# asbschmidt/CUDASW4

Measured on AMD Instinct MI355X. Metric: GCUPS, higher is better.
Workload: dtype f16x2; 1 GPU; peak: allqueries.fasta (20 queries, 41752 residues) vs pseudo DB 1000000 x 512, half2 kernel configuration, blosum62, gop -11 gex -1, top 10, C++ host driver; db_subjects=1000000, db_residues=512000000, queries=20, kernel=half2, queries_in_flight=1, tail_overlaps=10, numa_node_rank0=0, numa_bound=True, resident=True, residency=resident, cached_chars=512000000, parallelism=db-shard x1 (one DB sharded), one top-K gather per step + host merge

## Files before the change

cudasw4_amd/csrc/sw_api.hip:

```cpp
#include <hip/hip_runtime.h>
#include <hipcub/hipcub.hpp>

#include <algorithm>
#include <cstdio>
#include <cmath>
#include <cstdlib>
#include <cstring>
#include <ctime>
#include <string>
#include <vector>

#include "../../include/cudasw4_amd.h"
#include "../../include/cudasw4_amd_engine.h"
#include "sw_internal.hpp"
#include "sw_launch.hpp"
#include "sw_rows_pipeline.hpp"

namespace {

thread_local std::string g_last_error = "";

int fail(int code, const std::string& msg) {
    g_last_error = msg;
    return code;
}

#define SW_HIP(expr)                                                                              \
    do {                                                                                          \
        hipError_t e__ = (expr);                                                                  \
        if (e__ != hipSuccess)                                                                    \
            return fail(SW_ERR_HIP, std::string(#expr) + ": " + hipGetErrorString(e__));          \
    } while (0)

const swk::KindLaunch* kind_launch(int kind) {
    switch (kind) {
        case SW_KIND_F16X2: return &swk::launch_f16x2();
        case SW_KIND_I16X2: return &swk::launch_i16x2();
        case SW_KIND_I32: return &swk::launch_i32();
        case SW_KIND_F32: return &swk::launch_f32();
    }
    return nullptr;
}

bool kind_packed(int kind) { return kind == SW_KIND_F16X2 || kind == SW_KIND_I16X2; }

struct QueryPlan {
    int rows = 0;
    int nstripes = 0;
    int lanes = 16;
};

QueryPlan plan_query(int kind, int32_t qlen, int lanes) {
    const swk::KindLaunch* kl = kind_launch(kind);
    QueryPlan pl;
    pl.lanes = lanes;
    if (!kl || qlen <= 0) return pl;
    const int maxrows = swk::max_rows(kind, lanes);
    const int maxrows_multi = (kind == SW_KIND_F32 && lanes <= 16) ? std::min(maxrows, swk::kMaxRowsScalarMulti) : maxrows;
    double two_wave_penalty = 1.05;
    if (const char* e = getenv("CUDASW4_AMD_TWO_WAVE_PENALTY")) two_wave_penalty = std::max(1.0, atof(e));
    const bool has_three_wave_multi = kl->packed && lanes <= 16 && swk::kWaves3MaxRowsPackedMulti > maxrows / 2;
    double best = 1e300;
    auto consider = [&](int ns) {
        const int64_t per_lane = (qlen + (int64_t)lanes * ns - 1) / ((int64_t)lanes * ns);
        int r = (int)((per_lane + swk::kRowsGranule - 1) / swk::kRowsGranule * swk::kRowsGranule);
        r = std::max(r, swk::kRowsGranule);
        if (r > (ns > 1 ? maxrows_multi : maxrows)) return;
        if (ns > 1 && 2 * r <= maxrows) return;
        double cost = ns * (r + (ns > 1 ? 3.0 : 1.2));
        if (has_three_wave_multi && ns > 1 && r > swk::kWaves3MaxRowsPackedMulti) cost *= two_wave_penalty;
        if (cost < best - 1e-9) { best = cost; pl.rows = r; pl.nstripes = ns; }
    };
    if (qlen <= (int64_t)lanes * maxrows) consider(1);
    const int64_t stripe_multi = (int64_t)lanes * maxrows_multi;
    const int ns_m = std::max<int>(2, (int)((qlen + stripe_multi - 1) / stripe_multi));
    int ns_hi = ns_m + 2;
    if (has_three_wave_multi) {
        const int64_t stripe3 = (int64_t)lanes * swk::kWaves3MaxRowsPackedMulti;
        ns_hi = std::max<int>(ns_hi, (int)((qlen + stripe3 - 1) / stripe3) + 1);
    }
    for (int ns = ns_m; ns <= ns_hi; ns++) consider(ns);
    return pl;
}

struct Profile {
    unsigned char* dev = nullptr;
    size_t capacity = 0;
    bool valid = false;
    QueryPlan plan;
    int shift = 0;
    hipEvent_t ready = nullptr;
};

}

constexpr uint32_t kWorkSlots = 4096;
#ifndef SW_LANES8_MAX_QUERY_PACKED
#define SW_LANES8_MAX_QUERY_PACKED 256
#endif
#ifndef SW_LANES4_MAX_QUERY_PACKED
#define SW_LANES4_MAX_QUERY_PACKED 96
#endif
#ifndef SW_LANES4_MAX_QUERY_SCALAR
#define SW_LANES4_MAX_QUERY_SCALAR 128
#endif
#ifndef SW_LANES4_MAX_SUBJECT
#define SW_LANES4_MAX_SUBJECT 1280
#endif
#ifndef SW_LANES4_MIN_BATCHES_PER_CU
#define SW_LANES4_MIN_BATCHES_PER_CU 12
#endif
#ifndef SW_LANES8_MAX_SUBJECT
#define SW_LANES8_MAX_SUBJECT 192
#endif
#ifndef SW_LANES8_MAX_QUERY_SCALAR
#define SW_LANES8_MAX_QUERY_SCALAR 256
#endif

struct sw_ctx {
    int device = 0;
    int num_cus = 0;
    int8_t* d_matrix = nullptr;
    int dim = swk::kLetters;
    uint32_t* d_zeros = nullptr;
    uint32_t* d_work = nullptr;
    uint32_t work_next = 0;
    uint32_t work_zeroed = 0;
    uint32_t* start_signal = nullptr;
    uint32_t* dry_signal = nullptr;
    int32_t* dirty_counter = nullptr;
    uint32_t dry_value = 0;
    int grid_reserve = 0;
    int grid_mult = 4;
    int grid_cap = 0;
    bool have_matrix = false;
    int8_t* d_query = nullptr;
    size_t query_capacity = 0;
    static constexpr int kQuerySlots = 4;
    int8_t* h_query[kQuerySlots] = {};
    size_t h_query_capacity[kQuerySlots] = {};
    hipEvent_t query_copied[kQuerySlots] = {};
    bool query_slot_used[kQuerySlots] = {};
    int query_next = 0;
    int32_t qlen = 0;
    bool have_query = false;
    Profile profiles[4][4][2];
    bool use_offs = true;
    int64_t long16_min = -1;
    int64_t long16_min_default = -1;
    int matrix_max = 1;
    bool i32_native = false;
    int32_t lanes4_max_subject = -1;
    int32_t lanes4_max_q = -1;
    int32_t lanes8_max_q = -1;
    bool check_bounds = false;
    uint32_t pipe_spin_limit = 1u << 20;
    int32_t pipe_drop_stage = -1;
    int32_t pipe_cpl = 0;
    int32_t stream_slots = 4;
    int32_t stream_jump = 0;
    int32_t stream_cols_max = 4096;
    int32_t stream_multi_cols_max = 1536;
    int32_t stream_multi_max_subject = -1;
    int32_t pipe_quorum = 0;
    int32_t pipe_slot = 0;
};

namespace {

int max_grid(const sw_ctx* ctx) {
    const int g = std::max(1, ctx->num_cus) * ctx->grid_mult;
    return ctx->grid_cap > 0 ? std::min(g, ctx->grid_cap) : g;
}

int rescore_lanes(int32_t max_subject_len) { return max_subject_len > 1280 ? 64 : 16; }

int shape_index(int lanes) { return lanes == 64 ? 1 : lanes == 8 ? 2 : lanes == 4 ? 3 : 0; }

int effective_kind_of(const sw_ctx* ctx, int kind, int32_t max_subject_len) {
    if (kind != SW_KIND_I32 || ctx->i32_native || !ctx->have_query) return kind;
    const int64_t bound = (int64_t)std::min(ctx->qlen, max_subject_len) * std::max(1, ctx->matrix_max) + ((int64_t)1 << 22) + 4096;
    return bound < ((int64_t)1 << 24) ? SW_KIND_F32 : SW_KIND_I32;
}

int lanes_for_partition_any(const sw_ctx* ctx, int kind, int part_id, int32_t n, int32_t max_subject_len);
int lanes_for_partition(const sw_ctx* ctx, int kind, int part_id, int32_t n, int32_t max_subject_len) {
    const int lanes = lanes_for_partition_any(ctx, kind, part_id, n, max_subject_len);
    return (lanes == 16 && kind_packed(kind) && max_subject_len >= 0xffff) ? 64 : lanes;
}
int lanes_for_partition_any(const sw_ctx* ctx, int kind, int part_id, int32_t n, int32_t max_subject_len) {
    if (part_id < SW_NUM_LENGTH_PARTITIONS - 2) {
        if (!ctx->have_query) return 16;
        const int32_t limit4 = ctx->lanes4_max_q >= 0 ? ctx->lanes4_max_q : kind_packed(kind) ? SW_LANES4_MAX_QUERY_PACKED : SW_LANES4_MAX_QUERY_SCALAR;
        const int64_t batches4 = (int64_t)n / (64 * (kind_packed(kind) ? 2 : 1));
        const bool enough4 = ctx->lanes4_max_q >= 0 || batches4 >= (int64_t)SW_LANES4_MIN_BATCHES_PER_CU * std::max(1, ctx->num_cus);
        const int32_t lmax4 = ctx->lanes4_max_subject >= 0 ? ctx->lanes4_max_subject : SW_LANES4_MAX_SUBJECT;
        if (ctx->qlen <= 4 * swk::max_rows(kind, 4) && ctx->qlen <= limit4 && enough4 && max_subject_len <= lmax4) return 4;
        const bool fits8 = ctx->qlen <= 8 * swk::max_rows(kind, 8);
        const int32_t limit = ctx->lanes8_max_q >= 0 ? ctx->lanes8_max_q : kind_packed(kind) ? SW_LANES8_MAX_QUERY_PACKED : SW_LANES8_MAX_QUERY_SCALAR;
        if (fits8 && ctx->qlen <= limit) return 8;
        return 16;
    }
    const int64_t fills_gpu_twice = (int64_t)2 * std::max(1, ctx->num_cus) * 4 * 32;
    if (part_id == SW_NUM_LENGTH_PARTITIONS - 2) return n >= (ctx->long16_min >= 0 ? ctx->long16_min : 512) ? 16 : 64;
    return n >= fills_gpu_twice ? 16 : 64;
}


int ensure_profile(sw_ctx* ctx, int kind, int lanes, bool offs, int shift, hipStream_t stream) {
    Profile& pr = ctx->profiles[kind][shape_index(lanes)][offs];
    if (pr.valid && pr.shift != shift) pr.valid = false;
    if (pr.valid) {
        SW_HIP(hipStreamWaitEvent(stream, pr.ready, 0));
        return SW_OK;
    }
    const swk::KindLaunch* kl = kind_launch(kind);
    const QueryPlan pl = plan_query(kind, ctx->qlen, lanes);
    const size_t bytes = kl->tile_bytes(pl.rows, lanes) * (size_t)pl.nstripes;
    if (bytes == 0) return fail(SW_ERR_INVALID, "no kernel compiled for this query plan");
    if (bytes > pr.capacity) {
        const size_t cap = std::max<size_t>(std::max(bytes, 2 * pr.capacity), size_t(2) << 20);
        if (pr.dev) SW_HIP(hipFree(pr.dev));
        pr.dev = nullptr;
        pr.capacity = 0;
        SW_HIP(hipMalloc(&pr.dev, cap));
        pr.capacity = cap;
    }
    SW_HIP(kl->profile(pl.rows, lanes, ctx->d_query, ctx->qlen, ctx->d_matrix, ctx->dim, pl.nstripes, pr.dev, shift, stream));
    pr.shift = shift;
    if (!pr.ready) SW_HIP(hipEventCreateWithFlags(&pr.ready, hipEventDisableTiming));
    SW_HIP(hipEventRecord(pr.ready, stream));
    pr.plan = pl;
    pr.valid = true;
    return SW_OK;
}

int32_t border_capacity(int32_t max_len, int lanes) {
    const int64_t steps = ((int64_t)max_len + lanes - 1 + 3) / 4 * 4;
    return (int32_t)((steps + 15) / 16 * 16 + 16);
}
size_t border_bytes_per_wg(int32_t lcap, int lanes) {
    if (lanes == 4) return 0;
    const size_t region = lanes == 16 ? swk::border_region_words<16>(lcap) : lanes == 8 ? swk::border_region_words<8>(lcap) : swk::border_region_words<64>(lcap);
    return (size_t)(swk::kThreads / lanes) * region * sizeof(uint32_t);
}

__global__ void max_length_kernel(const int32_t* lengths, const int32_t* positions, const int32_t* count_ptr, int32_t first_pos,
                                  int32_t n, int32_t* out) {
    const int32_t cnt = count_ptr ? min(*count_ptr, n) : n;
    int32_t m = 0;
    for (int32_t i = blockIdx.x * blockDim.x + threadIdx.x; i < cnt; i += gridDim.x * blockDim.x)
        m = max(m, lengths[positions ? positions[i] : first_pos + i]);
    if (m > 0) atomicMax(out, m);
}

struct StreamPlan { int slots = 0, cols = 0, room = 0, base = 0, jump = 0; };
StreamPlan stream_plan(const sw_ctx* ctx, int kind, int lanes, int a, const QueryPlan& pl, int32_t max_subject_len) {
    StreamPlan sp;
    if (!kind_packed(kind) || lanes != 16 || a < 0) return sp;
    const bool multi = pl.nstripes > 1;
    const int P = swk::frame_classes(true, pl.rows, lanes, multi);
    sp.base = kind == SW_KIND_F16X2 ? -2016 : 0;
    const int top = kind == SW_KIND_F16X2 ? 1024 : 12400;
    sp.jump = ctx->stream_jump > 0 ? ctx->stream_jump : (kind == SW_KIND_F16X2 ? 512 : 2048);
    sp.room = top - sp.base - a * (2 * lanes + 4 + P);
    sp.cols = a > 0 ? std::min(sp.room / a, ctx->stream_cols_max) : ctx->stream_cols_max;
    sp.slots = std::max(1, std::min(ctx->stream_slots, swk::kStreamMaxSlots));
    if (sp.room < 4 * lanes * a || sp.cols < 4 * lanes) sp.slots = 1;
    if (multi) {
        const int32_t limit = ctx->stream_multi_max_subject >= 0 ? ctx->stream_multi_max_subject : (kind == SW_KIND_F16X2 ? 320 : 192);
        if (max_subject_len > limit) sp.slots = 1;
        sp.cols = std::min(sp.cols, ctx->stream_multi_cols_max);
    }
    return sp;
}

bool offs_possible(const sw_ctx* ctx, int kind, int lanes, int32_t max_subject_len, int gop, int gex, int ovf_check, int64_t* K_out) {
    const int a = -gex;
    const int64_t room = kind == SW_KIND_F16X2 ? 1536 : kind == SW_KIND_I16X2 ? 12500 : (int64_t)1 << 22;
    int64_t K = 1 << 21;
    while (K >= 4 * lanes && (int64_t)a * (K + 3 * lanes + 16) > room) K >>= 1;
    if (kind == SW_KIND_I16X2) K = std::min<int64_t>(K, std::max<int64_t>(2048, 4 * lanes));
    if (!kind_packed(kind) && max_subject_len + 3 * lanes + 16 > K) K = 0;
    if (K_out) *K_out = K;
    return ctx->use_offs && K >= 4 * lanes && (!kind_packed(kind) || (ovf_check && a >= 0)) && gop - gex >= -1000;
}
int packed_fallback_kind(int kind) { return kind == SW_KIND_F16X2 ? SW_KIND_F32 : SW_KIND_I32; }

constexpr uint32_t kWorkZeroBlock = 64;
hipError_t take_work_slot(sw_ctx* ctx, hipStream_t stream, uint32_t** out) {
    uint32_t* w = ctx->d_work + 2 * (ctx->work_next++ % kWorkSlots);
    *out = w;
    if (ctx->work_zeroed > 0) { ctx->work_zeroed--; return hipSuccess; }
    return hipMemsetAsync(w, 0, 2 * sizeof(uint32_t), stream);
}

struct ListMode {
    int32_t* claim = nullptr;
    int service_workgroups = 0;
    const uint32_t* done_flag = nullptr;
    uint32_t done_value = 0;
};

int scan_common(sw_ctx* ctx, int kind, int lanes, const int8_t* chars, const uint64_t* offsets, const int32_t* lengths,
                const int32_t* positions, const int32_t* count_ptr, int32_t first_pos, int32_t n,
                int32_t max_subject_len, int gop, int gex, float* scores, int32_t* ids, int64_t id_offset,
                int32_t* ovf_pos, int32_t* ovf_count, int ovf_check, void* temp, size_t temp_bytes,
                hipStream_t stream, int32_t* stat_count = nullptr, int32_t stat_limit = 0, const ListMode& list = ListMode()) {
    if (!ctx) return fail(SW_ERR_INVALID, "null context");
    uint32_t* const start_signal = ctx->start_signal;
    ctx->start_signal = nullptr;
    uint32_t* const dry_signal = ctx->dry_signal;
    ctx->dry_signal = nullptr;
    const swk::KindLaunch* kl = kind_launch(kind);
    if (!kl) return fail(SW_ERR_INVALID, "unknown kind");
    if (n < 0 || max_subject_len < 0) return fail(SW_ERR_INVALID, "negative count or length");
    if (max_subject_len > SW_MAX_SUBJECT_LEN)
        return fail(SW_ERR_INVALID, "max_subject_len " + std::to_string(max_subject_len) + ": pass the longest subject of the range (lengths[last]), not the partition's nominal boundary");
    if (gop > 0 || gex > 0) return fail(SW_ERR_INVALID, "gap scores must be <= 0");
    if (kind_packed(kind) && (gop < -1000 || gex < -1000)) return fail(SW_ERR_INVALID, "gap score out of range for a 16-bit kind");
    if (!ctx->have_matrix) return fail(SW_ERR_NO_MATRIX, "sw_set_matrix has not been called");
    if (!ctx->have_query) return fail(SW_ERR_NO_QUERY, "sw_set_query has not been called");
    if (n == 0) return SW_OK;
    if (!chars || !offsets || !lengths || !scores || !ids) return fail(SW_ERR_INVALID, "null buffer");
    if (ovf_check && kind_packed(kind) && (!ovf_pos || !ovf_count)) return fail(SW_ERR_INVALID, "overflow check without overflow buffers");
    SW_HIP(hipSetDevice(ctx->device));
    if (ctx->check_bounds) {
        int32_t* slot = reinterpret_cast<int32_t*>(ctx->d_zeros + 64);
        int32_t longest = 0;
        SW_HIP(hipMemsetAsync(slot, 0, sizeof(int32_t), stream));
        hipLaunchKernelGGL(max_length_kernel, dim3(std::min(1024, (n + 255) / 256)), dim3(256), 0, stream, lengths, positions, count_ptr, first_pos, n, slot);
        SW_HIP(hipGetLastError());
        SW_HIP(hipMemcpyAsync(&longest, slot, sizeof(int32_t), hipMemcpyDeviceToHost, stream));
        SW_HIP(hipStreamSynchronize(stream));
        if (longest > max_subject_len)
            return fail(SW_ERR_INVALID, "max_subject_len " + std::to_string(max_subject_len) + " under-reports: a subject of the range has " +
                                            std::to_string(longest) + " residues");
    }
    const int a = -gex;
    int64_t K = 0;
    const bool offs = offs_possible(ctx, kind, lanes, max_subject_len, gop, gex, ovf_check, &K);
    if (kind_packed(kind) && !offs) return fail(SW_ERR_INVALID, "internal: a packed launch without the column-offset recurrence (packed_fallback_kind)");
    int rc = ensure_profile(ctx, kind, lanes, offs, offs ? a : 0, stream);
    if (rc != SW_OK) return rc;
    const Profile& prof = ctx->profiles[kind][shape_index(lanes)][offs];
    const QueryPlan pl = prof.plan;
    const bool multi = pl.nstripes > 1;

    const int subj_per_batch = (swk::kThreads / lanes) * (kind_packed(kind) ? 2 : 1);
    const int nbatches = (n + subj_per_batch - 1) / subj_per_batch;
    int grid = std::min(nbatches, max_grid(ctx));
    if (list.service_workgroups > 0) grid = std::min(grid, list.service_workgroups);

    swk::ScanParams p{};
    p.claim = list.claim;
    p.service = list.service_workgroups > 0 ? 1 : 0;
    p.done_flag = list.done_flag;
    p.done_value = list.done_value;
    p.chars = chars; p.offsets = offsets; p.lengths = lengths;
    p.positions = positions; p.count_ptr = count_ptr;
    p.first_pos = first_pos; p.n = n;
    p.profile = prof.dev; p.nstripes = pl.nstripes;
    switch (kind) {
        case SW_KIND_F16X2: p.gop = swk::Arith<swk::F16X2>::encode_gap(gop); p.gex = swk::Arith<swk::F16X2>::encode_gap(gex); break;
        case SW_KIND_I16X2: p.gop = swk::Arith<swk::I16X2>::encode_gap(gop); p.gex = swk::Arith<swk::I16X2>::encode_gap(gex); break;
        case SW_KIND_I32: p.gop = swk::Arith<swk::I32>::encode_gap(gop); p.gex = swk::Arith<swk::I32>::encode_gap(gex); break;
        default: p.gop = swk::Arith<swk::F32>::encode_gap(gop); p.gex = swk::Arith<swk::F32>::encode_gap(gex); break;
    }
    if (offs) {
        const int g = gop - gex;
        switch (kind) {
            case SW_KIND_F16X2: p.gop = swk::Arith<swk::F16X2>::encode_gap(g); break;
            case SW_KIND_I16X2: p.gop = swk::Arith<swk::I16X2>::encode_gap(g); break;
            case SW_KIND_I32: p.gop = swk::Arith<swk::I32>::encode_gap(g); break;
            default: p.gop = swk::Arith<swk::F32>::encode_gap(g); break;
        }
        p.gex_mag = a;
        {
            const int P = swk::frame_classes(kl->packed, pl.rows, lanes, multi);
            const int wrap = -a * P, wrap_last = -a * ((pl.rows - 1) % P + 1);
            switch (kind) {
                case SW_KIND_F16X2: p.wrap_class = swk::Arith<swk::F16X2>::encode_gap(wrap); p.wrap_last = swk::Arith<swk::F16X2>::encode_gap(wrap_last); break;
                case SW_KIND_I16X2: p.wrap_class = swk::Arith<swk::I16X2>::encode_gap(wrap); p.wrap_last = swk::Arith<swk::I16X2>::encode_gap(wrap_last); break;
                case SW_KIND_I32: p.wrap_class = swk::Arith<swk::I32>::encode_gap(wrap); p.wrap_last = swk::Arith<swk::I32>::encode_gap(wrap_last); break;
                default: p.wrap_class = swk::Arith<swk::F32>::encode_gap(wrap); p.wrap_last = swk::Arith<swk::F32>::encode_gap(wrap_last); break;
            }
        }
        p.renorm_quads = (int32_t)(K / 4);
        const int lower = -(int)((int64_t)a * K);
        switch (kind) {
            case SW_KIND_F16X2: p.renorm_word = swk::Arith<swk::F16X2>::encode_gap(lower); break;
            case SW_KIND_I16X2: p.renorm_word = swk::Arith<swk::I16X2>::encode_gap(lower); break;
            case SW_KIND_I32: p.renorm_word = swk::Arith<swk::I32>::encode_gap(lower); break;
            default: p.renorm_word = swk::Arith<swk::F32>::encode_gap(lower); break;
        }
    }
    const StreamPlan sp = stream_plan(ctx, kind, lanes, a, pl, max_subject_len);
    if (sp.slots >= 1) {
        p.stream_slots = sp.slots; p.stream_cols = sp.cols; p.stream_room = sp.room; p.level_base = sp.base;
        p.jump = sp.jump; p.jump_limit = sp.jump - 4;
        p.jump_word = kind == SW_KIND_F16X2 ? swk::Arith<swk::F16X2>::pos_word(sp.jump) : swk::Arith<swk::I16X2>::pos_word(sp.jump);
    }
    p.scores = scores; p.ids = ids; p.id_offset = id_offset;
    p.ovf_pos = ovf_pos; p.ovf_count = ovf_count; p.ovf_check = (ovf_check && kind_packed(kind)) ? 1 : 0;
    p.scratch = nullptr; p.lcap = 0; p.zeros = ctx->d_zeros + kind * 16;
    p.stat_count = stat_count; p.stat_limit = stat_limit;
    if (multi) {
        p.lcap = border_capacity(max_subject_len, lanes);
        if (p.stream_slots > 1) {
            int cols = p.stream_cols;
            while (cols > max_subject_len && (size_t)grid * border_bytes_per_wg(border_capacity(cols, lanes), lanes) > temp_bytes) cols = cols * 3 / 4;
            p.stream_cols = cols;
            p.lcap = border_capacity(std::max(max_subject_len, cols), lanes);
        }
        const size_t per_wg = border_bytes_per_wg(p.lcap, lanes);
        if (!temp || temp_bytes < per_wg) return fail(SW_ERR_TEMP, "temp buffer too small for a multi-stripe query");
        grid = (int)std::min<size_t>((size_t)grid, temp_bytes / per_wg);
        p.scratch = static_cast<uint32_t*>(temp);
    }
    SW_HIP(take_work_slot(ctx, stream, &p.work_counter));
    p.start_signal = start_signal;
    p.start_quorum = (uint32_t)std::min(grid, 64);
    p.dry_signal = dry_signal;
    if (!stat_count && !positions && p.stream_slots > 1 && lanes == 16 && kind_packed(kind)) { p.stat_count = ctx->dirty_counter; p.stat_limit = INT32_MAX; }
    p.dry_value = ctx->dry_value;
    const int reserve = (list.service_workgroups > 0 || list.claim) ? 0 : ctx->grid_reserve;
    SW_HIP(kl->scan(pl.rows, lanes, multi, offs, grid, reserve, stream, p));
    return SW_OK;
}

}

namespace {
#define SW_REP8(OP) OP(0) OP(1) OP(2) OP(3) OP(4) OP(5) OP(6) OP(7)
#define SW_OP_PK_MAX3(i) asm volatile("v_pk_maximum3_f16 %0, %0, %1, %2" : "+v"(a[i]) : "v"(b), "v"(c));
#define SW_OP_ADD_F32(i) asm volatile("v_add_f32 %0, %0, %1" : "+v"(a[i]) : "v"(b));
#define SW_OP_MAX3_F32(i) asm volatile("v_max3_f32 %0, %0, %1, %2" : "+v"(a[i]) : "v"(b), "v"(c));
#define SW_OP_ADD_U32(i) asm volatile("v_add_u32 %0, %0, %1" : "+v"(a[i]) : "v"(b));
#define SW_OP_MAX3_I32(i) asm volatile("v_max3_i32 %0, %0, %1, %2" : "+v"(a[i]) : "v"(b), "v"(c));
#define SW_OP_PK_FMA(i) asm volatile("v_pk_fma_f16 %0, %1, %2, %0 op_sel:[0,1,0] op_sel_hi:[1,0,1]" : "+v"(a[i]) : "v"(b), "v"(c));
#define SW_OP_PK_ADD(i) asm volatile("v_pk_add_f16 %0, %0, %1" : "+v"(a[i]) : "v"(b));
#define SW_OP_DPP(i) asm volatile("v_mov_b32_dpp %0, %1 row_shr:1 row_mask:0xf bank_mask:0xf" : "+v"(a[i]) : "v"(b));
#define SW_OP_PERM(i) asm volatile("v_perm_b32 %0, %0, %1, %2" : "+v"(a[i]) : "v"(b), "v"(c));
template <int MIX>
__global__ void __launch_bounds__(256) valu_rate_kernel(unsigned* out, unsigned long long* clocks, unsigned seed, int iters) {
    unsigned a[8];
    unsigned b = seed + threadIdx.x, c = seed * 3u + 1u;
    for (int i = 0; i < 8; i++) a[i] = seed + i + threadIdx.x;
    if constexpr (MIX == 4) {
        asm volatile("v_mov_b32 v0, %0\nv_mov_b32 v1, %0\nv_mov_b32 v2, %0\nv_mov_b32 v3, %0\nv_mov_b32 v4, %0\nv_mov_b32 v5, %0\nv_mov_b32 v6, %0\nv_mov_b32 v7, %0\n"
                     "v_mov_b32 v8, %1\nv_mov_b32 v9, %1\nv_mov_b32 v10, %1\nv_mov_b32 v11, %1\nv_mov_b32 v12, %2\nv_mov_b32 v13, %2\nv_mov_b32 v14, %2\nv_mov_b32 v15, %2\n"
                     :: "v"(a[0]), "v"(b), "v"(c) : "v0", "v1", "v2", "v3", "v4", "v5", "v6", "v7", "v8", "v9", "v10", "v11", "v12", "v13", "v14", "v15");
    }
    const unsigned long long t0 = clock64(), w0 = wall_clock64();
    for (int it = 0; it < iters; it++) {
        if constexpr (MIX == 0) { SW_REP8(SW_OP_PK_MAX3) SW_REP8(SW_OP_PK_MAX3) SW_REP8(SW_OP_PK_MAX3) SW_REP8(SW_OP_PK_MAX3) }
        if constexpr (MIX == 1) { SW_REP8(SW_OP_ADD_F32) SW_REP8(SW_OP_MAX3_F32) SW_REP8(SW_OP_ADD_F32) SW_OP_MAX3_F32(0) SW_OP_MAX3_F32(1) SW_OP_MAX3_F32(2) SW_OP_MAX3_F32(3) SW_OP_MAX3_F32(4) SW_OP_MAX3_F32(5) SW_OP_ADD_F32(6) SW_OP_ADD_F32(7) }
        if constexpr (MIX == 3) {
            SW_REP8(SW_OP_PK_MAX3) SW_OP_PK_FMA(0) SW_OP_PK_FMA(1) SW_OP_PK_ADD(2) SW_OP_PK_ADD(3) SW_OP_DPP(4) SW_OP_PK_FMA(5) SW_OP_PK_ADD(6) SW_OP_ADD_U32(7)
            SW_REP8(SW_OP_PK_MAX3) SW_OP_PK_FMA(0) SW_OP_PK_FMA(1) SW_OP_PK_ADD(2) SW_OP_PK_ADD(3) SW_OP_DPP(4) SW_OP_PK_FMA(5) SW_OP_PK_ADD(6) SW_OP_PERM(7)
            SW_REP8(SW_OP_PK_MAX3) SW_OP_PK_FMA(0) SW_OP_PK_FMA(1) SW_OP_PK_ADD(2) SW_OP_PK_ADD(3) SW_OP_DPP(4) SW_OP_PK_ADD(5) SW_OP_PK_ADD(6) SW_OP_ADD_U32(7)
            SW_REP8(SW_OP_PK_MAX3) SW_OP_PK_FMA(0) SW_OP_PK_FMA(1) SW_OP_PK_ADD(2) SW_OP_PK_ADD(3) SW_OP_PK_MAX3(4) SW_OP_PK_MAX3(5) SW_OP_PK_MAX3(6) SW_OP_PK_ADD(7)
        }
        if constexpr (MIX == 4) {
#define SW_B4_MAX3(i, j, k) "v_pk_maximum3_f16 v" #i ", v" #i ", v" #j ", v" #k "\n"
#define SW_B4_FMA(i, j, k) "v_pk_fma_f16 v" #i ", v" #j ", v" #k ", v" #i " op_sel:[0,1,0] op_sel_hi:[1,0,1]\n"
#define SW_B4_ADD(i, j) "v_pk_add_f16 v" #i ", v" #i ", v" #j "\n"
#define SW_B4_DPP(i, j) "v_mov_b32_dpp v" #i ", v" #j " row_shr:1 row_mask:0xf bank_mask:0xf\n"
#define SW_B4_ADDU(i, j) "v_add_u32 v" #i ", v" #i ", v" #j "\n"
#define SW_B4_ROW8 SW_B4_MAX3(0, 9, 14) SW_B4_MAX3(1, 10, 15) SW_B4_MAX3(2, 11, 12) SW_B4_MAX3(3, 8, 13) SW_B4_MAX3(4, 9, 14) SW_B4_MAX3(5, 10, 15) SW_B4_MAX3(6, 11, 12) SW_B4_MAX3(7, 8, 13)
            asm volatile(
                SW_B4_ROW8 SW_B4_FMA(0, 9, 14) SW_B4_FMA(1, 10, 15) SW_B4_ADD(2, 11) SW_B4_ADD(3, 8) SW_B4_DPP(4, 9) SW_B4_FMA(5, 10, 15) SW_B4_ADD(6, 11) SW_B4_ADDU(7, 8)
                SW_B4_ROW8 SW_B4_FMA(0, 9, 14) SW_B4_FMA(1, 10, 15) SW_B4_ADD(2, 11) SW_B4_ADD(3, 8) SW_B4_DPP(4, 9) SW_B4_FMA(5, 10, 15) SW_B4_ADD(6, 11) SW_B4_MAX3(7, 8, 13)
                SW_B4_ROW8 SW_B4_FMA(0, 9, 14) SW_B4_FMA(1, 10, 15) SW_B4_ADD(2, 11) SW_B4_ADD(3, 8) SW_B4_DPP(4, 9) SW_B4_ADD(5, 10) SW_B4_ADD(6, 11) SW_B4_ADDU(7, 8)
                SW_B4_ROW8 SW_B4_FMA(0, 9, 14) SW_B4_FMA(1, 10, 15) SW_B4_ADD(2, 11) SW_B4_ADD(3, 8) SW_B4_MAX3(4, 9, 14) SW_B4_MAX3(5, 10, 15) SW_B4_MAX3(6, 11, 12) SW_B4_ADD(7, 8)
                ::: "v0", "v1", "v2", "v3", "v4", "v5", "v6", "v7", "v8", "v9", "v10", "v11", "v12", "v13", "v14", "v15");
        }
        if constexpr (MIX == 2) { SW_REP8(SW_OP_MAX3_I32) SW_REP8(SW_OP_ADD_U32) SW_REP8(SW_OP_MAX3_I32) SW_OP_ADD_U32(0) SW_OP_ADD_U32(1) SW_OP_ADD_U32(2) SW_OP_ADD_U32(3) SW_OP_MAX3_I32(4) SW_OP_MAX3_I32(5) SW_OP_MAX3_I32(6) SW_OP_MAX3_I32(7) }
    }
    const unsigned long long t1 = clock64(), w1 = wall_clock64();
    if constexpr (MIX == 4) asm volatile("v_mov_b32 %0, v0\nv_xor_b32 %0, %0, v7" : "=v"(a[0]) :: "v0", "v7");
    unsigned r = 0;
    for (int i = 0; i < 8; i++) r ^= a[i];
    out[blockIdx.x * blockDim.x + threadIdx.x] = r;
    if (threadIdx.x == 0) { clocks[2 * blockIdx.x] = t1 - t0; clocks[2 * blockIdx.x + 1] = w1 - w0; }
}
}

namespace swi {
int fail(int code, const std::string& msg) { return ::fail(code, msg); }
int32_t query_length(const sw_ctx* ctx) { return ctx && ctx->have_query ? ctx->qlen : 0; }
int device_of(const sw_ctx* ctx) { return ctx ? ctx->device : -1; }
int num_cus(const sw_ctx* ctx) { return ctx ? ctx->num_cus : 0; }
const int8_t* matrix(const sw_ctx* ctx, int* dim) {
    if (!ctx || !ctx->have_matrix) return nullptr;
    *dim = ctx->dim;
    return ctx->d_matrix;
}
}

extern "C" {

const char* sw_version(void) { return "cudasw4_amd 0.2 (gfx950)"; }

const char* sw_last_error(void) { return g_last_error.c_str(); }

int sw_device_count(void) {
    int n = 0;
    if (hipGetDeviceCount(&n) != hipSuccess) return 0;
    return n;
}

int sw_ctx_create(int device, sw_ctx** out) {
    if (!out) return fail(SW_ERR_INVALID, "null out pointer");
    *out = nullptr;
    int n = 0;
    if (hipGetDeviceCount(&n) != hipSuccess || n <= 0) return fail(SW_ERR_NO_DEVICE, "no HIP device available (this library has no CPU path)");
    if (device < 0 || device >= n) return fail(SW_ERR_INVALID, "device index out of range");
    SW_HIP(hipSetDevice(device));
    hipDeviceProp_t prop;
    SW_HIP(hipGetDeviceProperties(&prop, device));
    sw_ctx* ctx = new sw_ctx;
    ctx->device = device;
    ctx->num_cus = prop.multiProcessorCount;
    if (const char* e = getenv("CUDASW4_AMD_GRID_CAP")) ctx->grid_cap = std::max(0, atoi(e));
    if (const char* e = getenv("CUDASW4_AMD_NO_OFFS")) ctx->use_offs = !(e[0] == '1');
    if (const char* e = getenv("CUDASW4_AMD_I32_NATIVE")) ctx->i32_native = e[0] == '1';
    if (const char* e = getenv("CUDASW4_AMD_LANES8_MAX_Q")) ctx->lanes8_max_q = atoi(e);
    if (const char* e = getenv("CUDASW4_AMD_LANES4_MAX_Q")) ctx->lanes4_max_q = atoi(e);
    if (const char* e = getenv("CUDASW4_AMD_LANES4_MAX_SUBJECT")) ctx->lanes4_max_subject = atoi(e);
    if (const char* e = getenv("CUDASW4_AMD_CHECK_BOUNDS")) ctx->check_bounds = e[0] == '1';
    if (const char* e = getenv("CUDASW4_AMD_PIPE_SPIN_LIMIT")) ctx->pipe_spin_limit = (uint32_t)std::max(1ll, atoll(e));
    if (const char* e = getenv("CUDASW4_AMD_PIPE_TEST_DROP_STAGE")) ctx->pipe_drop_stage = atoi(e);
    if (const char* e = getenv("CUDASW4_AMD_PIPE_CPL")) ctx->pipe_cpl = atoi(e);
    if (const char* e = getenv("CUDASW4_AMD_STREAM")) ctx->stream_slots = std::max(0, std::min(swk::kStreamMaxSlots, atoi(e)));
    hipError_t e = hipMalloc(&ctx->d_matrix, 26 * swk::kLetters);
    if (e == hipSuccess) e = hipMalloc(&ctx->d_zeros, 256 + 64);
    if (e == hipSuccess) e = hipMalloc(&ctx->d_work, 2 * kWorkSlots * sizeof(uint32_t));
    if (e == hipSuccess) {
        uint32_t z[64] = {};
        for (int i = 0; i < 16; i++) z[SW_KIND_I16X2 * 16 + i] = swk::Arith<swk::I16X2>::kZero;
        e = hipMemcpy(ctx->d_zeros, z, sizeof(z), hipMemcpyHostToDevice);
    }
    for (int kind = 0; kind < 4 && e == hipSuccess; kind++) e = kind_launch(kind)->warm(nullptr);
    if (e == hipSuccess) e = hipStreamSynchronize(nullptr);
    if (e != hipSuccess) { delete ctx; return fail(SW_ERR_HIP, std::string("context set-up: ") + hipGetErrorString(e)); }
    *out = ctx;
    return SW_OK;
}

int sw_ctx_destroy(sw_ctx* ctx) {
    if (!ctx) return SW_OK;
    (void)hipSetDevice(ctx->device);
    if (ctx->d_matrix) (void)hipFree(ctx->d_matrix);
    if (ctx->d_zeros) (void)hipFree(ctx->d_zeros);
    if (ctx->d_work) (void)hipFree(ctx->d_work);
    if (ctx->d_query) (void)hipFree(ctx->d_query);
    for (int i = 0; i < sw_ctx::kQuerySlots; i++) {
        if (ctx->h_query[i]) (void)hipHostFree(ctx->h_query[i]);
        if (ctx->query_copied[i]) (void)hipEventDestroy(ctx->query_copied[i]);
    }
    for (auto& row : ctx->profiles)
        for (auto& shape : row)
            for (auto& pr : shape) {
                if (pr.dev) (void)hipFree(pr.dev);
                if (pr.ready) (void)hipEventDestroy(pr.ready);
            }
    delete ctx;
    return SW_OK;
}

int sw_set_matrix(sw_ctx* ctx, const int8_t* matrix_host, int dim) {
    if (!ctx || !matrix_host) return fail(SW_ERR_INVALID, "null argument");
    if (dim != 21 && dim != 25) return fail(SW_ERR_INVALID, "substitution matrices are 21 x 21 (20 amino acids + other) or 25 x 25 (types.hpp:205-396)");
    constexpr int kX = 23;
    int8_t m[26 * swk::kLetters];
    auto subject_col = [&](int j) { return (dim == 25 && j == swk::kPadLetter) ? kX : j; };
    for (int i = 0; i <= dim; i++) {
        const int qi = i < dim ? i : (dim == 25 ? kX : swk::kPadLetter);
        for (int j = 0; j < swk::kLetters; j++) m[i * swk::kLetters + j] = matrix_host[qi * dim + subject_col(j)];
    }
    for (int i = 0; i <= dim; i++)
        if (m[i * swk::kLetters + swk::kPadLetter] >= 0) return fail(SW_ERR_INVALID, "scores against the padding letter must be negative");
    for (int j = 0; j < swk::kLetters; j++)
        if (m[dim * swk::kLetters + j] >= 0) return fail(SW_ERR_INVALID, "scores against the padding letter must be negative");
    SW_HIP(hipSetDevice(ctx->device));
    SW_HIP(hipMemcpy(ctx->d_matrix, m, (size_t)(dim + 1) * swk::kLetters, hipMemcpyHostToDevice));
    ctx->matrix_max = 1;
    for (int i = 0; i < dim * dim; i++) ctx->matrix_max = std::max(ctx->matrix_max, (int)matrix_host[i]);
    if (ctx->have_query && dim < ctx->dim) ctx->have_query = false;
    ctx->dim = dim;
    ctx->have_matrix = true;
    for (auto& row : ctx->profiles)
        for (auto& shape : row)
            for (auto& pr : shape) pr.valid = false;
    return SW_OK;
}

int sw_set_query(sw_ctx* ctx, const int8_t* query_codes_host, int32_t qlen, void* stream) {
    if (!ctx || !query_codes_host) return fail(SW_ERR_INVALID, "null argument");
    if (qlen <= 0) return fail(SW_ERR_INVALID, "query length must be positive");
    for (int32_t i = 0; i < qlen; i++)
        if (query_codes_host[i] < 0 || query_codes_host[i] >= ctx->dim) return fail(SW_ERR_INVALID, "query code out of range for the installed matrix");
    SW_HIP(hipSetDevice(ctx->device));
    if ((size_t)qlen > ctx->query_capacity) {
        if (ctx->d_query) SW_HIP(hipFree(ctx->d_query));
        ctx->d_query = nullptr;
        ctx->query_capacity = 0;
        const size_t cap = std::max<size_t>(((size_t)qlen + 4095) / 4096 * 4096 * 2, size_t(1) << 16);
        SW_HIP(hipMalloc(&ctx->d_query, cap));
        ctx->query_capacity = cap;
    }
    hipStream_t s = static_cast<hipStream_t>(stream);
    const int slot = ctx->query_next;
    ctx->query_next = (ctx->query_next + 1) % sw_ctx::kQuerySlots;
    if (ctx->query_slot_used[slot]) SW_HIP(hipEventSynchronize(ctx->query_copied[slot]));
    if ((size_t)qlen > ctx->h_query_capacity[slot]) {
        if (ctx->h_query[slot]) SW_HIP(hipHostFree(ctx->h_query[slot]));
        ctx->h_query[slot] = nullptr;
        ctx->h_query_capacity[slot] = 0;
        const size_t cap = std::max<size_t>(((size_t)qlen + 4095) / 4096 * 4096 * 2, size_t(1) << 16);
        SW_HIP(hipHostMalloc(&ctx->h_query[slot], cap));
        ctx->h_query_capacity[slot] = cap;
    }
    if (!ctx->query_copied[slot]) SW_HIP(hipEventCreateWithFlags(&ctx->query_copied[slot], hipEventDisableTiming));
    memcpy(ctx->h_query[slot], query_codes_host, (size_t)qlen);
    SW_HIP(hipMemcpyAsync(ctx->d_query, ctx->h_query[slot], qlen, hipMemcpyHostToDevice, s));
    ctx->work_next = (ctx->work_next + kWorkZeroBlock - 1) / kWorkZeroBlock * kWorkZeroBlock;
    SW_HIP(hipMemsetAsync(ctx->d_work + 2 * (ctx->work_next % kWorkSlots), 0, 2 * kWorkZeroBlock * sizeof(uint32_t), s));
    ctx->work_zeroed = kWorkZeroBlock;
    SW_HIP(hipEventRecord(ctx->query_copied[slot], s));
    ctx->query_slot_used[slot] = true;
    ctx->qlen = qlen;
    ctx->have_query = true;
    for (auto& row : ctx->profiles)
        for (auto& shape : row)
            for (auto& pr : shape) pr.valid = false;
    return SW_OK;
}

namespace {
__global__ void __launch_bounds__(256) check_codes_kernel(const int8_t* __restrict__ chars, size_t n, int32_t* bad) {
    const size_t stride = (size_t)gridDim.x * blockDim.x * 16;
    unsigned m = 0;
    const size_t head = (16 - ((size_t)chars & 15)) & 15;
    const size_t tid = (size_t)blockIdx.x * blockDim.x + threadIdx.x;
    if (tid < head && tid < n) m |= (unsigned char)chars[tid] > 20 ? 1u : 0u;
    const size_t body = n > head ? (n - head) / 16 * 16 : 0;
    for (size_t i = tid * 16; i < body; i += stride) {
        const uint4 v = *reinterpret_cast<const uint4*>(chars + head + i);
        const unsigned w[4] = {v.x, v.y, v.z, v.w};
#pragma unroll
        for (int k = 0; k < 4; k++) {
            m |= w[k] & 0xE0E0E0E0u;
            m |= ((w[k] & 0x1F1F1F1Fu) + 0x0B0B0B0Bu) & 0x20202020u;
        }
    }
    const size_t tail0 = head + body;
    if (tail0 + tid < n && tid < 16) m |= (unsigned char)chars[tail0 + tid] > 20 ? 1u : 0u;
    if (m) atomicOr(bad, 1);
}
}

int sw_check_letter_codes(sw_ctx* ctx, const int8_t* chars, size_t n, int32_t* bad_flag, void* stream) {
    if (!ctx || !bad_flag) return fail(SW_ERR_INVALID, "null argument");
    if (n == 0) return SW_OK;
    if (!chars) return fail(SW_ERR_INVALID, "null buffer");
    SW_HIP(hipSetDevice(ctx->device));
    const size_t want = (n / 16 + 255) / 256 + 1;
    const int grid = (int)std::min<size_t>(want, (size_t)std::max(1, ctx->num_cus) * 16);
    hipLaunchKernelGGL(check_codes_kernel, dim3(grid), dim3(256), 0, static_cast<hipStream_t>(stream), chars, n, bad_flag);
    SW_HIP(hipGetLastError());
    return SW_OK;
}

int sw_set_start_signal(sw_ctx* ctx, uint32_t* signal) {
    if (!ctx) return fail(SW_ERR_INVALID, "null context");
    ctx->start_signal = signal;
    return SW_OK;
}


namespace {
int rows_common_checks(sw_ctx* ctx, const int8_t* chars, const uint64_t* offsets, const int32_t* lengths, int32_t first_pos, int32_t n,
                       int32_t max_subject_len, int gop, int gex, float* scores, int32_t* ids, bool dry_armed, hipStream_t stream,
                       const char* who) {
    if (dry_armed) return fail(SW_ERR_INVALID, std::string(who) + " never runs dry: sw_set_dry_signal applies to sw_scan_partition launches (the armed signal was cancelled)");
    if (n < 0 || max_subject_len < 0) return fail(SW_ERR_INVALID, "negative count or length");
    if (gop > 0 || gex > 0) return fail(SW_ERR_INVALID, "gap scores must be <= 0");
    if (gop > gex) return fail(SW_ERR_INVALID, std::string(who) + " needs gop <= gex (the prefix form of the horizontal gap)");
    if (gex < -10000 || gop < -100000) return fail(SW_ERR_INVALID, std::string("gap score out of range for ") + who);
    if (!ctx->have_matrix) return fail(SW_ERR_NO_MATRIX, "sw_set_matrix has not been called");
    if (!ctx->have_query) return fail(SW_ERR_NO_QUERY, "sw_set_query has not been called");
    if (n == 0) return SW_OK;
    if (!chars || !offsets || !lengths || !scores || !ids) return fail(SW_ERR_INVALID, "null buffer");
    SW_HIP(hipSetDevice(ctx->device));
    if (ctx->check_bounds) {
        int32_t* slot = reinterpret_cast<int32_t*>(ctx->d_zeros + 64);
        int32_t longest = 0;
        SW_HIP(hipMemsetAsync(slot, 0, sizeof(int32_t), stream));
        hipLaunchKernelGGL(max_length_kernel, dim3(std::min(1024, (n + 255) / 256)), dim3(256), 0, stream, lengths, nullptr, nullptr, first_pos, n, slot);
        SW_HIP(hipGetLastError());
        SW_HIP(hipMemcpyAsync(&longest, slot, sizeof(int32_t), hipMemcpyDeviceToHost, stream));
        SW_HIP(hipStreamSynchronize(stream));
        if (longest > max_subject_len)
            return fail(SW_ERR_INVALID, "max_subject_len " + std::to_string(max_subject_len) + " under-reports: a subject of the range has " +
                                            std::to_string(longest) + " residues");
    }
    return SW_OK;
}

int pipeline_cpl(const sw_ctx* ctx, int32_t n, int32_t max_subject_len) {
    if (ctx->pipe_cpl == 4 || ctx->pipe_cpl == 8 || ctx->pipe_cpl == 16) return ctx->pipe_cpl;
    static const double kRowUs16[3] = {0.27, 0.38, 0.57}, kHopUs16[3] = {3.6, 5.0, 8.0}, kRowUs8[3] = {0.32, 0.42, 0.61}, kHopUs8[3] = {2.4, 3.4, 5.3};
    const bool shortBatch = ctx->qlen <= swk::kPipeShortBatchMaxQuery;
    const double* kRowUs = shortBatch ? kRowUs8 : kRowUs16;
    const double* kHopUs = shortBatch ? kHopUs8 : kHopUs16;
    int best = 16;
    double bestT = 1e300;
    for (int k = 0; k < 3; k++) {
        const int cpl = 4 << k;
        const double stages = std::max(1.0, std::ceil((double)max_subject_len / (64.0 * cpl)));
        if (cpl < 16 && (double)std::max(n, 1) * stages > 768.0) continue;
        const double t = (double)std::max(ctx->qlen, 1) * kRowUs[k] + stages * kHopUs[k];
        if (t < bestT) { bestT = t; best = cpl; }
    }
    return best;
}
constexpr size_t kPipeCtrlBytes = 16;
int64_t pipeline_stages(int cpl, int32_t max_subject_len) { return std::max<int64_t>(1, ((int64_t)max_subject_len + 64 * cpl - 1) / (64 * cpl)); }
}


size_t sw_scan_rows_pipelined_temp_bytes(sw_ctx* ctx, int32_t n, int32_t max_subject_len) {
    if (!ctx || !ctx->have_query || n <= 0 || max_subject_len < 0) return 0;
    const int64_t tickets = (int64_t)n * pipeline_stages(pipeline_cpl(ctx, n, max_subject_len), max_subject_len);
    return kPipeCtrlBytes + (size_t)tickets * ((size_t)ctx->qlen + 1) * sizeof(unsigned long long);
}

namespace {
int launch_pipeline(sw_ctx* ctx, swk::PipelineParams& p, int cpl, int64_t stages, int64_t tickets, uint32_t* start_signal, void* xfer,
                    hipStream_t stream) {
    const size_t need = kPipeCtrlBytes + (size_t)tickets * ((size_t)ctx->qlen + 1) * sizeof(unsigned long long);
    p.query = ctx->d_query; p.qlen = ctx->qlen; p.matrix = ctx->d_matrix; p.dim = ctx->dim;
    p.ctrl = static_cast<uint32_t*>(xfer);
    p.xfer = reinterpret_cast<unsigned long long*>(static_cast<char*>(xfer) + kPipeCtrlBytes);
    p.start_signal = start_signal;
    const int slot_regs = ctx->pipe_slot > 0 ? ctx->pipe_slot : 128;
    const int64_t resident = (int64_t)std::max(1, ctx->num_cus) * 4 * std::max(1, std::min(8, 512 / slot_regs)) / 2;
    p.start_quorum = (uint32_t)std::max<int64_t>(1, std::min(tickets, ctx->pipe_quorum > 0 ? (int64_t)ctx->pipe_quorum : resident));
    p.max_stages = (int32_t)stages;
    p.spin_limit = ctx->pipe_spin_limit;
    p.test_drop_stage = ctx->pipe_drop_stage;
    SW_HIP(hipMemsetAsync(xfer, 0xFF, need, stream));
    const dim3 grid((unsigned)tickets), block(64);
    const int slot = ctx->pipe_slot;
#define SW_PIPE_LAUNCH_B(CPL, B)                                                                                            \
    do {                                                                                                                    \
        if (slot == 128) hipLaunchKernelGGL((swk::sw_rows_pipeline_kernel<CPL, 128, B>), grid, block, 0, stream, p);        \
        else if (slot == 168) hipLaunchKernelGGL((swk::sw_rows_pipeline_kernel<CPL, 168, B>), grid, block, 0, stream, p);   \
        else if (slot == 256) hipLaunchKernelGGL((swk::sw_rows_pipeline_kernel<CPL, 256, B>), grid, block, 0, stream, p);   \
        else hipLaunchKernelGGL((swk::sw_rows_pipeline_kernel<CPL, 0, B>), grid, block, 0, stream, p);                      \
    } while (0)
#define SW_PIPE_LAUNCH(CPL)                                                                                              \
    do {                                                                                                                 \
        if (ctx->qlen <= swk::kPipeShortBatchMaxQuery) SW_PIPE_LAUNCH_B(CPL, 8);                                         \
        else SW_PIPE_LAUNCH_B(CPL, 16);                                                                                  \
    } while (0)
    if (cpl == 4) SW_PIPE_LAUNCH(4);
    else if (cpl == 8) SW_PIPE_LAUNCH(8);
    else SW_PIPE_LAUNCH(16);
#undef SW_PIPE_LAUNCH_B
#undef SW_PIPE_LAUNCH
    SW_HIP(hipGetLastError());
    return SW_OK;
}

__global__ void __launch_bounds__(256) pipeline_pick_kernel(int32_t* list, const int32_t* count_ptr, int32_t max_count, const int32_t* lengths,
                                                            int32_t min_len, int32_t cap, int32_t* out_pos, int32_t* out_count) {
    __shared__ int k;
    if (threadIdx.x == 0) k = 0;
    __syncthreads();
    const int32_t cnt = min(*count_ptr, max_count);
    for (int32_t i = threadIdx.x; i < cnt; i += blockDim.x) {
        const int32_t v = __hip_atomic_load(list + i, __ATOMIC_RELAXED, __HIP_MEMORY_SCOPE_AGENT);
        if (v < 0 || lengths[v] < min_len) continue;
        const int slot = atomicAdd(&k, 1);
        if (slot >= cap) continue;
        if (atomicCAS(list + i, v, swk::kListTaken) == v) out_pos[slot] = v;
        else out_pos[slot] = -1;
    }
    __syncthreads();
    if (threadIdx.x == 0) *out_count = min(k, cap);
}
constexpr int32_t kPipeRescoreCap = 64;
size_t pipe_rescore_header_bytes() { return 256 + (size_t)kPipeRescoreCap * sizeof(int32_t); }
}

int sw_scan_rows_pipelined(sw_ctx* ctx, const int8_t* chars, const uint64_t* offsets, const int32_t* lengths, int32_t first_pos,
                           int32_t n, int32_t max_subject_len, int gop, int gex, float* scores, int32_t* ids, int64_t id_offset,
                           int32_t* fail_count, int32_t* over_limit_count, int32_t* over_limit_count2, int32_t packed_limit,
                           void* temp, size_t temp_bytes, void* stream_) {
    if (!ctx) return fail(SW_ERR_INVALID, "null context");
    uint32_t* const start_signal = ctx->start_signal;
    ctx->start_signal = nullptr;
    const bool dry_armed = ctx->dry_signal != nullptr;
    ctx->dry_signal = nullptr;
    hipStream_t stream = static_cast<hipStream_t>(stream_);
    if ((int64_t)max_subject_len * (int64_t)(-gex) >= ((int64_t)1 << 28)) return fail(SW_ERR_INVALID, "subject length x gap extension out of range for sw_scan_rows_pipelined");
    const int rc = rows_common_checks(ctx, chars, offsets, lengths, first_pos, n, max_subject_len, gop, gex, scores, ids, dry_armed, stream, "sw_scan_rows_pipelined");
    if (rc != SW_OK || n == 0) return rc;
    const int cpl = pipeline_cpl(ctx, n, max_subject_len);
    const int64_t stages = pipeline_stages(cpl, max_subject_len);
    const int64_t tickets = (int64_t)n * stages;
    if (tickets > (int64_t)1 << 24) return fail(SW_ERR_INVALID, "too many pipeline stages for one sw_scan_rows_pipelined launch");
    const size_t need = kPipeCtrlBytes + (size_t)tickets * ((size_t)ctx->qlen + 1) * sizeof(unsigned long long);
    if (!temp || temp_bytes < need) return fail(SW_ERR_TEMP, "temp buffer too small for sw_scan_rows_pipelined (sw_scan_rows_pipelined_temp_bytes)");
    swk::PipelineParams p{};
    p.chars = chars; p.offsets = offsets; p.lengths = lengths; p.first_pos = first_pos; p.n = n;
    p.gop = gop; p.gex = gex; p.scores = scores; p.ids = ids; p.id_offset = id_offset;
    p.fail_count = fail_count;
    p.stat_count = over_limit_count; p.stat_count2 = over_limit_count2; p.stat_limit = packed_limit;
    return launch_pipeline(ctx, p, cpl, stages, tickets, start_signal, temp, stream);
}

size_t sw_rescore_overflow_pipelined_temp_bytes(sw_ctx* ctx, int32_t max_subject_len) {
    if (!ctx || !ctx->have_query || max_subject_len < 0) return 0;
    const int64_t tickets = (int64_t)kPipeRescoreCap * pipeline_stages(pipeline_cpl(ctx, kPipeRescoreCap, max_subject_len), max_subject_len);
    return pipe_rescore_header_bytes() + kPipeCtrlBytes + (size_t)tickets * ((size_t)ctx->qlen + 1) * sizeof(unsigned long long);
}

int sw_rescore_overflow_pipelined(sw_ctx* ctx, int32_t* ovf_pos, const int32_t* ovf_count, int32_t max_count, const int8_t* chars,
                                  const uint64_t* offsets, const int32_t* lengths, int32_t max_subject_len, int32_t min_subject_len,
                                  int gop, int gex, float* scores, int32_t* ids, int64_t id_offset, int32_t* fail_count,
                                  int32_t packed_limit, int32_t* true_overflow_count, void* temp, size_t temp_bytes, void* stream_) {
    if (!ctx) return fail(SW_ERR_INVALID, "null context");
    ctx->start_signal = nullptr;
    const bool dry_armed = ctx->dry_signal != nullptr;
    ctx->dry_signal = nullptr;
    hipStream_t stream = static_cast<hipStream_t>(stream_);
    if (!ovf_pos || !ovf_count) return fail(SW_ERR_INVALID, "null overflow buffers");
    if (max_count <= 0) return SW_OK;
    if ((int64_t)max_subject_len * (int64_t)(-gex) >= ((int64_t)1 << 28)) return fail(SW_ERR_INVALID, "subject length x gap extension out of range for sw_rescore_overflow_pipelined");
    const int rc = rows_common_checks(ctx, chars, offsets, lengths, 0, 1, max_subject_len, gop, gex, scores, ids, dry_armed, stream, "sw_rescore_overflow_pipelined");
    if (rc != SW_OK) return rc;
    const int cpl = pipeline_cpl(ctx, kPipeRescoreCap, max_subject_len);
    const int64_t stages = pipeline_stages(cpl, max_subject_len);
    const int64_t tickets = (int64_t)kPipeRescoreCap * stages;
    const size_t need = sw_rescore_overflow_pipelined_temp_bytes(ctx, max_subject_len);
    if (!temp || temp_bytes < need) return fail(SW_ERR_TEMP, "temp buffer too small for sw_rescore_overflow_pipelined");
    int32_t* out_count = static_cast<int32_t*>(temp);
    int32_t* out_pos = reinterpret_cast<int32_t*>(static_cast<char*>(temp) + 256);
    hipLaunchKernelGGL(pipeline_pick_kernel, dim3(1), dim3(256), 0, stream, ovf_pos, ovf_count, max_count, lengths, std::max(min_subject_len, 1),
                       kPipeRescoreCap, out_pos, out_count);
    SW_HIP(hipGetLastError());
    swk::PipelineParams p{};
    p.chars = chars; p.offsets = offsets; p.lengths = lengths; p.first_pos = 0; p.n = kPipeRescoreCap;
    p.positions = out_pos; p.count_ptr = out_count;
    p.gop = gop; p.gex = gex; p.scores = scores; p.ids = ids; p.id_offset = id_offset;
    p.fail_count = fail_count;
    p.stat_count = true_overflow_count; p.stat_count2 = nullptr; p.stat_limit = packed_limit;
    return launch_pipeline(ctx, p, cpl, stages, tickets, nullptr, static_cast<char*>(temp) + pipe_rescore_header_bytes(), stream);
}

int sw_set_dirty_counter(sw_ctx* ctx, int32_t* counter) {
    if (!ctx) return fail(SW_ERR_INVALID, "null context");
    ctx->dirty_counter = counter;
    return SW_OK;
}

int sw_set_dry_signal(sw_ctx* ctx, uint32_t* signal, uint32_t value) {
    if (!ctx) return fail(SW_ERR_INVALID, "null context");
    ctx->dry_signal = signal;
    ctx->dry_value = value;
    return SW_OK;
}

int sw_set_long16_min(sw_ctx* ctx, int32_t subjects) {
    if (!ctx) return fail(SW_ERR_INVALID, "null context");
    ctx->long16_min = subjects < 0 ? ctx->long16_min_default : subjects;
    return SW_OK;
}

int sw_set_grid_reserve(sw_ctx* ctx, int32_t workgroups) {
    if (!ctx) return fail(SW_ERR_INVALID, "null context");
    if (workgroups < 0) return fail(SW_ERR_INVALID, "negative reserve");
    ctx->grid_reserve = workgroups;
    return SW_OK;
}

namespace {
__global__ void reduce_windows_kernel(const float* __restrict__ win_scores, const int32_t* __restrict__ win_first,
                                      const int32_t* __restrict__ real_pos, int32_t n_real, float* __restrict__ scores,
                                      int32_t* __restrict__ ids, int64_t id_offset) {
    const int32_t i = blockIdx.x * blockDim.x + threadIdx.x;
    if (i >= n_real) return;
    float m = -1.0f;
    for (int32_t w = win_first[i]; w < win_first[i + 1]; w++) m = fmaxf(m, win_scores[w]);
    const int32_t pos = real_pos[i];
    scores[pos] = m;
    ids[pos] = (int32_t)(id_offset + pos);
}
}

namespace {
__global__ void probe_wait_kernel(unsigned* flag, unsigned* saw, unsigned long long max_ticks) {
    const unsigned long long t0 = wall_clock64();
    unsigned v = 0;
    while ((v = __hip_atomic_load(flag, __ATOMIC_RELAXED, __HIP_MEMORY_SCOPE_AGENT)) == 0 && wall_clock64() - t0 < max_ticks)
        __builtin_amdgcn_s_sleep(8);
    *saw = v;
}
__global__ void probe_set_kernel(unsigned* flag) { __hip_atomic_store(flag, 1u, __ATOMIC_RELAXED, __HIP_MEMORY_SCOPE_AGENT); }
__global__ void probe_side_kernel(unsigned* signal, unsigned* flag, unsigned* saw, unsigned long long max_ticks) {
    __hip_atomic_fetch_add(signal, 1u, __ATOMIC_RELEASE, __HIP_MEMORY_SCOPE_SYSTEM);
    const unsigned long long t0 = wall_clock64();
    unsigned v = 0;
    while ((v = __hip_atomic_load(flag, __ATOMIC_RELAXED, __HIP_MEMORY_SCOPE_AGENT)) == 0 && wall_clock64() - t0 < max_ticks)
        __builtin_amdgcn_s_sleep(8);
    *saw = v;
}
}

int sw_probe_handshake(sw_ctx* ctx, void* side_stream, void* gated_stream, uint32_t* signal) {
    if (!ctx || !signal) return fail(SW_ERR_INVALID, "null argument");
    SW_HIP(hipSetDevice(ctx->device));
    hipStream_t side = static_cast<hipStream_t>(side_stream), gated = static_cast<hipStream_t>(gated_stream);
    unsigned* words = reinterpret_cast<unsigned*>(ctx->d_zeros + 72);
    SW_HIP(hipStreamSynchronize(side));
    SW_HIP(hipStreamSynchronize(gated));
    SW_HIP(hipMemsetAsync(words, 0, 2 * sizeof(unsigned), side));
    SW_HIP(hipStreamSynchronize(side));
    const uint32_t base = *reinterpret_cast<volatile uint32_t*>(signal);
    SW_HIP(hipStreamWaitValue32(gated, signal, base + 1u, hipStreamWaitValueGte, 0xffffffffu));
    hipLaunchKernelGGL(probe_set_kernel, dim3(1), dim3(1), 0, gated, words);
    hipLaunchKernelGGL(probe_side_kernel, dim3(1), dim3(1), 0, side, signal, words, words + 1, 1000000ull);
    SW_HIP(hipGetLastError());
    bool released = true;
    for (int i = 0;; i++) {
        const hipError_t q = hipStreamQuery(gated);
        if (q == hipSuccess) break;
        if (q != hipErrorNotReady) return fail(SW_ERR_HIP, std::string("hipStreamQuery: ") + hipGetErrorString(q));
        if (i >= 2000) {
            *reinterpret_cast<volatile uint32_t*>(signal) = base + 1u;
            released = false;
            break;
        }
        struct timespec ts = {0, 1000000};
        nanosleep(&ts, nullptr);
    }
    SW_HIP(hipStreamSynchronize(side));
    SW_HIP(hipStreamSynchronize(gated));
    unsigned saw = 0;
    SW_HIP(hipMemcpy(&saw, words + 1, sizeof(unsigned), hipMemcpyDeviceToHost));
    *reinterpret_cast<volatile uint32_t*>(signal) = base;
    return released && saw ? 1 : 0;
}

int sw_streams_run_concurrently(sw_ctx* ctx, void* stream_a, void* stream_b) {
    if (!ctx) return fail(SW_ERR_INVALID, "null context");
    SW_HIP(hipSetDevice(ctx->device));
    unsigned* words = reinterpret_cast<unsigned*>(ctx->d_zeros + 72);
    SW_HIP(hipMemsetAsync(words, 0, 2 * sizeof(unsigned), static_cast<hipStream_t>(stream_a)));
    SW_HIP(hipStreamSynchronize(static_cast<hipStream_t>(stream_a)));
    hipLaunchKernelGGL(probe_wait_kernel, dim3(1), dim3(1), 0, static_cast<hipStream_t>(stream_a), words, words + 1, 500000ull);
    hipLaunchKernelGGL(probe_set_kernel, dim3(1), dim3(1), 0, static_cast<hipStream_t>(stream_b), words);
    SW_HIP(hipGetLastError());
    unsigned saw = 0;
    SW_HIP(hipStreamSynchronize(static_cast<hipStream_t>(stream_b)));
    SW_HIP(hipMemcpyAsync(&saw, words + 1, sizeof(unsigned), hipMemcpyDeviceToHost, static_cast<hipStream_t>(stream_a)));
    SW_HIP(hipStreamSynchronize(static_cast<hipStream_t>(stream_a)));
    return saw ? 1 : 0;
}

int sw_measure_valu_rate(sw_ctx* ctx, int mix, int millis, double* lane_instr_per_s, double* shader_hz) {
    if (!ctx || mix < 0 || mix > 4) return fail(SW_ERR_INVALID, "null context or unknown instruction mix");
    SW_HIP(hipSetDevice(ctx->device));
    const int grid = std::max(1, ctx->num_cus) * 4;
    unsigned* out = nullptr;
    unsigned long long* clocks = nullptr;
    SW_HIP(hipMalloc(&out, (size_t)grid * 256 * sizeof(unsigned)));
    if (hipMalloc(&clocks, (size_t)grid * 2 * sizeof(unsigned long long)) != hipSuccess) { (void)hipFree(out); return fail(SW_ERR_HIP, "hipMalloc"); }
    hipEvent_t e0 = nullptr, e1 = nullptr;
    hipError_t err = hipEventCreate(&e0);
    if (err == hipSuccess) err = hipEventCreate(&e1);
    auto run = [&](int iters, float* ms) -> hipError_t {
        hipError_t e = hipEventRecord(e0, nullptr);
        if (e != hipSuccess) return e;
        if (mix == 0) hipLaunchKernelGGL(valu_rate_kernel<0>, dim3(grid), dim3(256), 0, nullptr, out, clocks, 7u, iters);
        else if (mix == 1) hipLaunchKernelGGL(valu_rate_kernel<1>, dim3(grid), dim3(256), 0, nullptr, out, clocks, 7u, iters);
        else if (mix == 2) hipLaunchKernelGGL(valu_rate_kernel<2>, dim3(grid), dim3(256), 0, nullptr, out, clocks, 7u, iters);
        else if (mix == 3) hipLaunchKernelGGL(valu_rate_kernel<3>, dim3(grid), dim3(256), 0, nullptr, out, clocks, 7u, iters);
        else hipLaunchKernelGGL(valu_rate_kernel<4>, dim3(grid), dim3(256), 0, nullptr, out, clocks, 7u, iters);
        e = hipGetLastError();
        if (e == hipSuccess) e = hipEventRecord(e1, nullptr);
        if (e == hipSuccess) e = hipEventSynchronize(e1);
        if (e == hipSuccess) e = hipEventElapsedTime(ms, e0, e1);
        return e;
    };
    float ms = 0.0f;
    int iters = 4096;
    if (err == hipSuccess) err = run(iters, &ms);
    if (err == hipSuccess && ms > 0.0f) {
        iters = (int)std::min(1.0e7, std::max(1024.0, iters * (double)std::max(millis, 1) / ms));
        err = run(iters, &ms);
    }
    double hz = 0.0;
    if (err == hipSuccess) {
        std::vector<unsigned long long> h((size_t)grid * 2);
        err = hipMemcpy(h.data(), clocks, h.size() * sizeof(unsigned long long), hipMemcpyDeviceToHost);
        double ticks = 0.0, wall = 0.0;
        for (int i = 0; i < grid; i++) { ticks += (double)h[2 * i]; wall += (double)h[2 * i + 1]; }
        if (wall > 0.0) hz = ticks / wall * 100.0e6;
    }
    if (e0) (void)hipEventDestroy(e0);
    if (e1) (void)hipEventDestroy(e1);
    (void)hipFree(out);
    (void)hipFree(clocks);
    if (err != hipSuccess) return fail(SW_ERR_HIP, std::string("sw_measure_valu_rate: ") + hipGetErrorString(err));
    if (lane_instr_per_s) *lane_instr_per_s = ms > 0.0f ? (double)grid * 256.0 * (mix >= 3 ? 64.0 : 32.0) * (double)iters / (ms * 1e-3) : 0.0;
    if (shader_hz) *shader_hz = hz;
    return SW_OK;
}

int32_t sw_window_overlap(sw_ctx* ctx, int gop, int gex) {
    if (!ctx || !ctx->have_query || !ctx->have_matrix) return -1;
    const int cost = std::min(-gop, -gex);
    if (cost <= 0) return -1;
    const int64_t span = (int64_t)ctx->qlen + (int64_t)ctx->qlen * std::max(1, ctx->matrix_max) / cost + 1;
    return span > 0x3fffffff ? -1 : (int32_t)span;
}

int sw_reduce_windows(sw_ctx* ctx, const float* win_scores, const int32_t* win_first, const int32_t* real_pos, int32_t n_real,
                      float* scores, int32_t* ids, int64_t id_offset, void* stream) {
    if (!ctx) return fail(SW_ERR_INVALID, "null context");
    if (n_real <= 0) return SW_OK;
    if (!win_scores || !win_first || !real_pos || !scores || !ids) return fail(SW_ERR_INVALID, "null buffer");
    SW_HIP(hipSetDevice(ctx->device));
    hipLaunchKernelGGL(reduce_windows_kernel, dim3((n_real + 255) / 256), dim3(256), 0, static_cast<hipStream_t>(stream), win_scores,
                       win_first, real_pos, n_real, scores, ids, id_offset);
    SW_HIP(hipGetLastError());
    return SW_OK;
}

int sw_plan_query(int kind, int32_t qlen, int32_t* rows_per_lane, int32_t* nstripes) {
    if (!kind_launch(kind) || qlen <= 0) return fail(SW_ERR_INVALID, "bad kind or query length");
    const QueryPlan pl = plan_query(kind, qlen, 16);
    if (rows_per_lane) *rows_per_lane = pl.rows;
    if (nstripes) *nstripes = pl.nstripes;
    return SW_OK;
}

int sw_plan_launch(sw_ctx* ctx, int kind, int part_id, int32_t n, int32_t max_subject_len, int32_t* effective_kind,
                   int32_t* rows_per_lane, int32_t* nstripes, int32_t* lanes) {
    if (!ctx || !kind_launch(kind)) return fail(SW_ERR_INVALID, "null context or unknown kind");
    if (!ctx->have_query) return fail(SW_ERR_NO_QUERY, "sw_set_query has not been called");
    if (part_id >= SW_NUM_LENGTH_PARTITIONS || max_subject_len < 0) return fail(SW_ERR_INVALID, "bad partition id or length");
    kind = effective_kind_of(ctx, kind, max_subject_len);
    const int ln = part_id < 0 ? rescore_lanes(max_subject_len) : lanes_for_partition(ctx, kind, part_id, n, max_subject_len);
    const QueryPlan pl = plan_query(kind, ctx->qlen, ln);
    if (effective_kind) *effective_kind = kind;
    if (rows_per_lane) *rows_per_lane = pl.rows;
    if (nstripes) *nstripes = pl.nstripes;
    if (lanes) *lanes = ln;
    return SW_OK;
}

int sw_launch_vgpr_slot(sw_ctx* ctx, int kind, int part_id, int32_t n, int32_t max_subject_len) {
    if (!ctx || !kind_launch(kind) || !ctx->have_query || part_id >= SW_NUM_LENGTH_PARTITIONS || max_subject_len < 0) return 0;
    kind = effective_kind_of(ctx, kind, max_subject_len);
    const int ln = part_id < 0 ? rescore_lanes(max_subject_len) : lanes_for_partition(ctx, kind, part_id, n, max_subject_len);
    const QueryPlan pl = plan_query(kind, ctx->qlen, ln);
    if (pl.rows <= 0) return 0;
    return swk::vgpr_slot_of(kind, pl.rows, ln, pl.nstripes > 1);
}

int sw_set_rows_pipeline_slot(sw_ctx* ctx, int vgprs) {
    if (!ctx) return fail(SW_ERR_INVALID, "null context");
    if (vgprs != 0 && vgprs != 128 && vgprs != 168 && vgprs != 256) return fail(SW_ERR_INVALID, "a register-file slot is 128, 168 or 256 VGPRs (0: as few as the stage needs)");
    ctx->pipe_slot = vgprs;
    return SW_OK;
}

static size_t scan_temp_bytes_of(sw_ctx* ctx, int kind, int part_id, int32_t n, int32_t max_subject_len);
size_t sw_scan_temp_bytes(sw_ctx* ctx, int kind, int part_id, int32_t n, int32_t max_subject_len) {
    if (!ctx || !ctx->have_query || !kind_launch(kind) || max_subject_len < 0 || n <= 0) return 0;
    if (kind_packed(kind) && part_id >= 0) {
        const int fb = packed_fallback_kind(kind);
        const size_t own = scan_temp_bytes_of(ctx, kind, part_id, n, max_subject_len);
        return std::max(own, scan_temp_bytes_of(ctx, effective_kind_of(ctx, fb, max_subject_len), part_id, n, max_subject_len));
    }
    return scan_temp_bytes_of(ctx, effective_kind_of(ctx, kind, max_subject_len), part_id, n, max_subject_len);
}

static size_t scan_temp_bytes_of(sw_ctx* ctx, int kind, int part_id, int32_t n, int32_t max_subject_len) {
    const int lanes = part_id < 0 ? rescore_lanes(max_subject_len) : lanes_for_partition(ctx, kind, part_id, n, max_subject_len);
    const QueryPlan pl = plan_query(kind, ctx->qlen, lanes);
    if (pl.nstripes <= 1) return 0;
    const int subj_per_batch = (swk::kThreads / lanes) * (kind_packed(kind) ? 2 : 1);
    const int64_t nbatches = ((int64_t)n + subj_per_batch - 1) / subj_per_batch;
    const int64_t grid = std::min<int64_t>(nbatches, max_grid(ctx));
    const StreamPlan sp = stream_plan(ctx, kind, lanes, 1, pl, max_subject_len);
    const int32_t cols = sp.slots > 1 ? std::max(max_subject_len, sp.cols) : max_subject_len;
    return (size_t)grid * border_bytes_per_wg(border_capacity(cols, lanes), lanes);
}

int sw_scan_partition(sw_ctx* ctx, int kind, int part_id, const int8_t* chars, const uint64_t* offsets,
                      const int32_t* lengths, int32_t first_pos, int32_t n, int32_t max_subject_len, int gop, int gex,
                      float* scores, int32_t* ids, int64_t id_offset, int32_t* ovf_pos, int32_t* ovf_count,
                      int ovf_check, void* temp, size_t temp_bytes, void* stream) {
    if (!ctx) return fail(SW_ERR_INVALID, "null context");
    if (part_id < 0 || part_id >= SW_NUM_LENGTH_PARTITIONS || !kind_launch(kind)) {
        ctx->start_signal = nullptr;
        ctx->dry_signal = nullptr;
        return fail(SW_ERR_INVALID, part_id < 0 || part_id >= SW_NUM_LENGTH_PARTITIONS ? "partition id out of range" : "unknown kind");
    }
    kind = effective_kind_of(ctx, kind, max_subject_len);
    int lanes = lanes_for_partition(ctx, kind, part_id, n, max_subject_len);
    if (kind_packed(kind) && !offs_possible(ctx, kind, lanes, max_subject_len, gop, gex, ovf_check, nullptr)) {
        kind = effective_kind_of(ctx, packed_fallback_kind(kind), max_subject_len);
        lanes = lanes_for_partition(ctx, kind, part_id, n, max_subject_len);
        ovf_pos = nullptr; ovf_count = nullptr; ovf_check = 0;
    }
    return scan_common(ctx, kind, lanes, chars, offsets, lengths, nullptr, nullptr, first_pos, n, max_subject_len, gop, gex,
                       scores, ids, id_offset, ovf_pos, ovf_count, ovf_check, temp, temp_bytes,
                       static_cast<hipStream_t>(stream));
}

int sw_rescore_overflow(sw_ctx* ctx, int kind, const int32_t* ovf_pos, const int32_t* ovf_count, int32_t max_count,
                        const int8_t* chars, const uint64_t* offsets, const int32_t* lengths, int32_t max_subject_len,
                        int gop, int gex, float* scores, int32_t* ids, int64_t id_offset, void* temp,
                        size_t temp_bytes, void* stream) {
    return sw_rescore_overflow_stat(ctx, kind, ovf_pos, ovf_count, max_count, chars, offsets, lengths, max_subject_len, gop, gex,
                                    scores, ids, id_offset, temp, temp_bytes, 0, nullptr, stream);
}

int sw_rescore_overflow_stat(sw_ctx* ctx, int kind, const int32_t* ovf_pos, const int32_t* ovf_count, int32_t max_count,
                             const int8_t* chars, const uint64_t* offsets, const int32_t* lengths, int32_t max_subject_len,
                             int gop, int gex, float* scores, int32_t* ids, int64_t id_offset, void* temp,
                             size_t temp_bytes, int32_t packed_limit, int32_t* true_overflow_count, void* stream) {
    if (!ctx) return fail(SW_ERR_INVALID, "null context");
    uint32_t* const start_signal = ctx->start_signal;
    uint32_t* const dry_signal = ctx->dry_signal;
    ctx->start_signal = nullptr;
    ctx->dry_signal = nullptr;
    if (kind != SW_KIND_I32 && kind != SW_KIND_F32) return fail(SW_ERR_INVALID, "overflow re-score needs a 32-bit kind");
    if (!ovf_pos || !ovf_count) return fail(SW_ERR_INVALID, "null overflow buffers");
    if (max_count <= 0) return SW_OK;
    ctx->start_signal = start_signal;
    ctx->dry_signal = dry_signal;
    kind = effective_kind_of(ctx, kind, max_subject_len);
    const int lanes = rescore_lanes(max_subject_len);
    return scan_common(ctx, kind, lanes, chars, offsets, lengths, ovf_pos, ovf_count, 0, max_count, max_subject_len, gop, gex,
                       scores, ids, id_offset, nullptr, nullptr, 0, temp, temp_bytes, static_cast<hipStream_t>(stream),
                       true_overflow_count, packed_limit);
}

size_t sw_rescore_service_temp_bytes(sw_ctx* ctx, int kind, int32_t max_subject_len, int workgroups) {
    if (!ctx || !ctx->have_query || !kind_launch(kind) || max_subject_len < 0 || workgroups <= 0) return 0;
    kind = effective_kind_of(ctx, kind, max_subject_len);
    const int lanes = rescore_lanes(max_subject_len);
    const QueryPlan pl = plan_query(kind, ctx->qlen, lanes);
    if (pl.nstripes <= 1) return 0;
    return (size_t)workgroups * border_bytes_per_wg(border_capacity(max_subject_len, lanes), lanes);
}

int sw_rescore_service(sw_ctx* ctx, int kind, int32_t* ovf_pos, const int32_t* ovf_count, int32_t max_count,
                       const int8_t* chars, const uint64_t* offsets, const int32_t* lengths, int32_t max_subject_len,
                       int gop, int gex, float* scores, int32_t* ids, int64_t id_offset, void* temp, size_t temp_bytes,
                       int32_t packed_limit, int32_t* true_overflow_count, const uint32_t* done_flag, uint32_t done_value,
                       int workgroups, void* stream) {
    if (!ctx) return fail(SW_ERR_INVALID, "null context");
    uint32_t* const start_signal = ctx->start_signal;
    uint32_t* const dry_signal = ctx->dry_signal;
    ctx->start_signal = nullptr;
    ctx->dry_signal = nullptr;
    if (kind != SW_KIND_I32 && kind != SW_KIND_F32) return fail(SW_ERR_INVALID, "overflow re-score needs a 32-bit kind");
    if (!ovf_pos || !ovf_count || !done_flag) return fail(SW_ERR_INVALID, "null overflow buffers or flag");
    if (max_count <= 0 || workgroups <= 0) return SW_OK;
    ctx->start_signal = start_signal;
    ctx->dry_signal = dry_signal;
    kind = effective_kind_of(ctx, kind, max_subject_len);
    ListMode lm;
    lm.claim = ovf_pos;
    lm.service_workgroups = workgroups;
    lm.done_flag = done_flag;
    lm.done_value = done_value;
    return scan_common(ctx, kind, rescore_lanes(max_subject_len), chars, offsets, lengths, ovf_pos, ovf_count, 0, max_count, max_subject_len,
                       gop, gex, scores, ids, id_offset, nullptr, nullptr, 0, temp, temp_bytes, static_cast<hipStream_t>(stream),
                       true_overflow_count, packed_limit, lm);
}

int sw_rescore_overflow_claim(sw_ctx* ctx, int kind, int32_t* ovf_pos, const int32_t* ovf_count, int32_t max_count,
                              const int8_t* chars, const uint64_t* offsets, const int32_t* lengths, int32_t max_subject_len,
                              int gop, int gex, float* scores, int32_t* ids, int64_t id_offset, void* temp, size_t temp_bytes,
                              int32_t packed_limit, int32_t* true_overflow_count, void* stream) {
    if (!ctx) return fail(SW_ERR_INVALID, "null context");
    uint32_t* const start_signal = ctx->start_signal;
    uint32_t* const dry_signal = ctx->dry_signal;
    ctx->start_signal = nullptr;
    ctx->dry_signal = nullptr;
    if (kind != SW_KIND_I32 && kind != SW_KIND_F32) return fail(SW_ERR_INVALID, "overflow re-score needs a 32-bit kind");
    if (!ovf_pos || !ovf_count) return fail(SW_ERR_INVALID, "null overflow buffers");
    if (max_count <= 0) return SW_OK;
    ctx->start_signal = start_signal;
    ctx->dry_signal = dry_signal;
    kind = effective_kind_of(ctx, kind, max_subject_len);
    ListMode lm;
    lm.claim = ovf_pos;
    return scan_common(ctx, kind, rescore_lanes(max_subject_len), chars, offsets, lengths, ovf_pos, ovf_count, 0, max_count, max_subject_len,
                       gop, gex, scores, ids, id_offset, nullptr, nullptr, 0, temp, temp_bytes, static_cast<hipStream_t>(stream),
                       true_overflow_count, packed_limit, lm);
}


namespace {
struct TopkLayout {
    size_t keys_off, vals_off, cub_off, total, cub_bytes;
};
TopkLayout topk_layout(int64_t n) {
    TopkLayout L{};
    size_t cub = 0;
    (void)hipcub::DeviceRadixSort::SortPairsDescending(nullptr, cub, (const float*)nullptr, (float*)nullptr,
                                                       (const int32_t*)nullptr, (int32_t*)nullptr, (int)std::max<int64_t>(n, 1));
    auto al = [](size_t x) { return (x + 255) / 256 * 256; };
    L.keys_off = 0;
    L.vals_off = al((size_t)n * sizeof(float));
    L.cub_off = L.vals_off + al((size_t)n * sizeof(int32_t));
    L.cub_bytes = cub;
    L.total = L.cub_off + al(cub);
    return L;
}
__global__ void topk_copy_kernel(const float* keys, const int32_t* vals, int64_t n, int k, float* out_s, int32_t* out_i) {
    const int i = blockIdx.x * blockDim.x + threadIdx.x;
    if (i < k) {
        out_s[i] = i < n ? keys[i] : -1.0f;
        out_i[i] = i < n ? vals[i] : -1;
    }
}

constexpr int kSelBins = 2048;
constexpr int kSelPasses = 6;
__constant__ const int kSelShift[kSelPasses] = {53, 42, 32, 21, 10, 0};
__constant__ const int kSelBits[kSelPasses] = {11, 11, 10, 11, 11, 10};

struct TopkState {
    unsigned long long prefix;
    unsigned long long decided;
    unsigned long long remaining;
    unsigned int skip_rest;
    unsigned int out_count;
    unsigned int blocks_done;
    unsigned int hist[kSelBins];
};

__device__ __forceinline__ unsigned long long topk_key(float score, unsigned int pos) {
    unsigned int u = __float_as_uint(score);
    u ^= (u >> 31) ? 0xffffffffu : 0x80000000u;
    return ((unsigned long long)u << 32) | (unsigned long long)(~pos);
}

__global__ void topk_init_kernel(TopkState* st, int k) {
    for (int i = threadIdx.x; i < kSelBins; i += blockDim.x) st->hist[i] = 0;
    if (threadIdx.x == 0) { st->prefix = 0; st->decided = 0; st->remaining = (unsigned long long)k; st->skip_rest = 0; st->out_count = 0; st->blocks_done = 0; }
}

__device__ void topk_pick(TopkState* st, int pass, unsigned int* h, unsigned long long* part) {
    const int nb = 1 << kSelBits[pass];
    for (int i = threadIdx.x; i < kSelBins; i += blockDim.x) { h[i] = i < nb ? __hip_atomic_load(&st->hist[i], __ATOMIC_RELAXED, __HIP_MEMORY_SCOPE_AGENT) : 0u; }
    __syncthreads();
    constexpr int per = kSelBins / 256;
    unsigned long long mine = 0;
    for (int j = 0; j < per; j++) { const int b = kSelBins - 1 - (threadIdx.x * per + j); mine += h[b]; }
    part[threadIdx.x] = mine;
    __syncthreads();
    if (threadIdx.x == 0) {
        unsigned long long need = st->remaining, above = 0;
        int t = 0;
        while (t < 255 && above + part[t] < need) { above += part[t]; t++; }
        int b = kSelBins - 1 - t * per;
        for (int j = 0; j < per - 1 && above + h[b] < need; j++) { above += h[b]; b--; }
        const int shift = kSelShift[pass];
        st->prefix |= (unsigned long long)b << shift;
        st->decided |= (unsigned long long)((1u << kSelBits[pass]) - 1u) << shift;
        st->remaining = need - above;
        if (st->remaining == h[b]) st->skip_rest = 1;
    }
    __syncthreads();
    for (int i = threadIdx.x; i < kSelBins; i += blockDim.x) st->hist[i] = 0;
}

__global__ void __launch_bounds__(256) topk_hist_kernel(const float* __restrict__ scores, int64_t n, TopkState* st, int pass) {
    if (st->skip_rest) return;
    __shared__ unsigned int h[kSelBins];
    for (int i = threadIdx.x; i < kSelBins; i += blockDim.x) h[i] = 0;
    __syncthreads();
    const unsigned long long prefix = st->prefix, decided = st->decided;
    const int shift = kSelShift[pass];
    const unsigned int mask = (1u << kSelBits[pass]) - 1u;
    const int wlane = threadIdx.x & 63;
    for (int64_t i0 = (int64_t)blockIdx.x * blockDim.x; i0 < n; i0 += (int64_t)gridDim.x * blockDim.x) {
        const int64_t i = i0 + threadIdx.x;
        bool act = false;
        unsigned int bin = 0;
        if (i < n) {
            const unsigned long long key = topk_key(scores[i], (unsigned int)i);
            act = (key & decided) == prefix;
            bin = (unsigned int)(key >> shift) & mask;
        }
        const unsigned long long m = __ballot(act);
        if (m == 0) continue;
        const unsigned int lb = (unsigned int)__shfl((int)bin, __ffsll((long long)m) - 1);
        const unsigned long long same = __ballot(act && bin == lb);
        if (act) {
            if (bin != lb) atomicAdd(&h[bin], 1u);
            else if (wlane == __ffsll((long long)same) - 1) atomicAdd(&h[lb], (unsigned int)__popcll(same));
        }
    }
    __syncthreads();
    for (int i = threadIdx.x; i < kSelBins; i += blockDim.x)
        if (h[i]) atomicAdd(&st->hist[i], h[i]);
    __shared__ unsigned long long part[256];
    __shared__ bool last;
    __threadfence();
    __syncthreads();
    if (threadIdx.x == 0) last = atomicAdd(&st->blocks_done, 1u) + 1u == gridDim.x;
    __syncthreads();
    if (!last) return;
    __threadfence();
    topk_pick(st, pass, h, part);
    if (threadIdx.x == 0) st->blocks_done = 0;
}

__global__ void __launch_bounds__(256) topk_compact_kernel(const float* __restrict__ scores, const int32_t* __restrict__ ids, int64_t n,
                                                           TopkState* st, int k, unsigned long long* out_keys, int32_t* out_ids) {
    const unsigned long long prefix = st->prefix, decided = st->decided;
    for (int64_t i = (int64_t)blockIdx.x * blockDim.x + threadIdx.x; i < n; i += (int64_t)gridDim.x * blockDim.x) {
        const unsigned long long key = topk_key(scores[i], (unsigned int)i);
        if ((key & decided) >= prefix) {
            const unsigned int slot = atomicAdd(&st->out_count, 1u);
            if (slot < (unsigned int)k) { out_keys[slot] = key; out_ids[slot] = ids[i]; }
        }
    }
}

__global__ void topk_emit_kernel(const unsigned long long* keys, const int32_t* vals, int k, float* out_s, int32_t* out_i) {
    const int i = blockIdx.x * blockDim.x + threadIdx.x;
    if (i < k) {
        unsigned int u = (unsigned int)(keys[i] >> 32);
        u ^= (u >> 31) ? 0x80000000u : 0xffffffffu;
        out_s[i] = __uint_as_float(u);
        out_i[i] = vals[i];
    }
}

__global__ void __launch_bounds__(256) topk_rank_emit_kernel(const unsigned long long* keys, const int32_t* vals, int k, float* out_s, int32_t* out_i) {
    __shared__ unsigned long long sk[1024];
    for (int i = threadIdx.x; i < k; i += blockDim.x) sk[i] = keys[i];
    __syncthreads();
    for (int i = threadIdx.x; i < k; i += blockDim.x) {
        const unsigned long long mine = sk[i];
        int rank = 0;
        for (int j = 0; j < k; j++) rank += sk[j] > mine ? 1 : 0;
        unsigned int u = (unsigned int)(mine >> 32);
        u ^= (u >> 31) ? 0x80000000u : 0xffffffffu;
        out_s[rank] = __uint_as_float(u);
        out_i[rank] = vals[i];
    }
}

constexpr int kSmallK = 32;
constexpr int kSmallChunk = 2048;
constexpr int kSmallMaxGrid = 1024;

__device__ __forceinline__ unsigned long long block_max_u64(unsigned long long v, unsigned long long* wmax) {
#pragma unroll
    for (int d = 32; d >= 1; d >>= 1) {
        const unsigned long long o = __shfl_xor(v, d);
        v = o > v ? o : v;
    }
    __syncthreads();
    if ((threadIdx.x & 63) == 0) wmax[threadIdx.x >> 6] = v;
    __syncthreads();
    unsigned long long m = wmax[0];
#pragma unroll
    for (int w = 1; w < 4; w++) m = wmax[w] > m ? wmax[w] : m;
    return m;
}

__device__ __forceinline__ void small_merge(unsigned long long (&key)[8], unsigned long long* best, unsigned long long* wmax, int k) {
    unsigned long long mine = 0;
#pragma unroll
    for (int e = 0; e < 8; e++) mine = key[e] > mine ? key[e] : mine;
    for (int round = 0; round < k; round++) {
        const unsigned long long m = block_max_u64(mine, wmax);
        if (m <= best[k - 1]) break;
        if (mine == m) {
            mine = 0;
#pragma unroll
            for (int e = 0; e < 8; e++) {
                if (key[e] == m) key[e] = 0;
                mine = key[e] > mine ? key[e] : mine;
            }
        }
        if (threadIdx.x == 0) {
            int i = k - 1;
            while (i > 0 && best[i - 1] < m) { best[i] = best[i - 1]; i--; }
            best[i] = m;
        }
        __syncthreads();
    }
}

__global__ void __launch_bounds__(256) topk_small_partial_kernel(const float* __restrict__ scores, int64_t n, int k, unsigned long long* out) {
    __shared__ unsigned long long best[kSmallK];
    __shared__ unsigned long long wmax[4];
    if (threadIdx.x < kSmallK) best[threadIdx.x] = 0;
    __syncthreads();
    const int64_t nchunks = (n + kSmallChunk - 1) / kSmallChunk;
    for (int64_t c = blockIdx.x; c < nchunks; c += gridDim.x) {
        unsigned long long key[8];
        const unsigned long long thr = best[k - 1];
        bool above = false;
#pragma unroll
        for (int e = 0; e < 8; e++) {
            const int64_t i = c * kSmallChunk + e * 256 + threadIdx.x;
            key[e] = i < n ? topk_key(scores[i], (unsigned int)i) : 0ull;
            above = above || key[e] > thr;
        }
        if (!__syncthreads_or(above)) continue;
        small_merge(key, best, wmax, k);
    }
    __syncthreads();
    if (threadIdx.x < k) out[(size_t)blockIdx.x * k + threadIdx.x] = best[threadIdx.x];
}

__global__ void __launch_bounds__(256) topk_small_final_kernel(const unsigned long long* __restrict__ cand, int ncand, const int32_t* __restrict__ ids,
                                                               int k, float* out_s, int32_t* out_i) {
    __shared__ unsigned long long best[kSmallK];
    __shared__ unsigned long long wmax[4];
    if (threadIdx.x < kSmallK) best[threadIdx.x] = 0;
    __syncthreads();
    for (int c0 = 0; c0 < ncand; c0 += kSmallChunk) {
        unsigned long long key[8];
#pragma unroll
        for (int e = 0; e < 8; e++) {
            const int i = c0 + e * 256 + threadIdx.x;
            key[e] = i < ncand ? cand[i] : 0ull;
        }
        small_merge(key, best, wmax, k);
    }
    __syncthreads();
    if (threadIdx.x < k) {
        const unsigned long long key = best[threadIdx.x];
        unsigned int u = (unsigned int)(key >> 32);
        u ^= (u >> 31) ? 0x80000000u : 0xffffffffu;
        out_s[threadIdx.x] = __uint_as_float(u);
        out_i[threadIdx.x] = ids[~(unsigned int)key];
    }
}

int small_grid(const sw_ctx* ctx, int64_t n) {
    const int64_t nchunks = (n + kSmallChunk - 1) / kSmallChunk;
    return (int)std::max<int64_t>(1, std::min<int64_t>(nchunks, std::min<int64_t>(kSmallMaxGrid, (int64_t)std::max(1, ctx->num_cus) * 4)));
}

struct SelectLayout {
    size_t state_off, keys_a, keys_b, vals_a, vals_b, cub_off, cub_bytes, total;
};
SelectLayout select_layout(int k) {
    SelectLayout L{};
    size_t cub = 0;
    (void)hipcub::DeviceRadixSort::SortPairsDescending(nullptr, cub, (const unsigned long long*)nullptr, (unsigned long long*)nullptr,
                                                       (const int32_t*)nullptr, (int32_t*)nullptr, std::max(k, 1));
    auto al = [](size_t x) { return (x + 255) / 256 * 256; };
    L.state_off = 0;
    L.keys_a = al(sizeof(TopkState));
    L.keys_b = L.keys_a + al((size_t)k * 8);
    L.vals_a = L.keys_b + al((size_t)k * 8);
    L.vals_b = L.vals_a + al((size_t)k * 4);
    L.cub_off = L.vals_b + al((size_t)k * 4);
    L.cub_bytes = cub;
    L.total = L.cub_off + al(cub);
    return L;
}

bool use_select(int64_t n, int k) {
    const char* force = getenv("CUDASW4_AMD_TOPK");
    if (k >= n) return false;
    if (force && force[0] == 's' && force[1] == 'o') return false;
    if (force && force[0] == 's' && force[1] == 'e') return true;
    return n >= (int64_t(1) << 17) && (int64_t)k * 8 <= n;
}
}

size_t sw_topk_temp_bytes(int64_t n, int k) {
    if (n <= 0 || k <= 0) return 0;
    return std::max(std::max(topk_layout(n).total, k < n ? select_layout(k).total : size_t(0)), (size_t)kSmallMaxGrid * kSmallK * sizeof(unsigned long long));
}

int sw_topk(sw_ctx* ctx, const float* scores, const int32_t* ids, int64_t n, int k, float* out_scores,
            int32_t* out_ids, void* temp, size_t temp_bytes, void* stream) {
    if (!ctx) return fail(SW_ERR_INVALID, "null context");
    if (k <= 0) return SW_OK;
    if (n < 0 || n > 0x7fffffffLL) return fail(SW_ERR_INVALID, "bad result count");
    if (!out_scores || !out_ids) return fail(SW_ERR_INVALID, "null output");
    SW_HIP(hipSetDevice(ctx->device));
    hipStream_t s = static_cast<hipStream_t>(stream);
    if (n > 0 && (!scores || !ids)) return fail(SW_ERR_INVALID, "null input");
    const char* force = getenv("CUDASW4_AMD_TOPK");
    if (n > k && k <= kSmallK && (!force || (force[0] == 's' && force[1] == 'm'))) {
        const int grid = small_grid(ctx, n);
        if (!temp || temp_bytes < (size_t)grid * k * sizeof(unsigned long long)) return fail(SW_ERR_TEMP, "temp buffer too small for top-K");
        unsigned long long* cand = static_cast<unsigned long long*>(temp);
        hipLaunchKernelGGL(topk_small_partial_kernel, dim3(grid), dim3(256), 0, s, scores, n, k, cand);
        hipLaunchKernelGGL(topk_small_final_kernel, dim3(1), dim3(256), 0, s, cand, grid * k, ids, k, out_scores, out_ids);
        SW_HIP(hipGetLastError());
        return SW_OK;
    }
    if (n > 0 && use_select(n, k)) {
        const SelectLayout L = select_layout(k);
        if (!temp || temp_bytes < L.total) return fail(SW_ERR_TEMP, "temp buffer too small for top-K");
        char* base = static_cast<char*>(temp);
        TopkState* st = reinterpret_cast<TopkState*>(base + L.state_off);
        auto* keys_a = reinterpret_cast<unsigned long long*>(base + L.keys_a);
        auto* keys_b = reinterpret_cast<unsigned long long*>(base + L.keys_b);
        auto* vals_a = reinterpret_cast<int32_t*>(base + L.vals_a);
        auto* vals_b = reinterpret_cast<int32_t*>(base + L.vals_b);
        const int grid = (int)std::min<int64_t>((n + 256 * 16 - 1) / (256 * 16), (int64_t)std::max(1, ctx->num_cus) * 8);
        hipLaunchKernelGGL(topk_init_kernel, dim3(1), dim3(256), 0, s, st, k);
        for (int pass = 0; pass < kSelPasses; pass++) {
            hipLaunchKernelGGL(topk_hist_kernel, dim3(grid), dim3(256), 0, s, scores, n, st, pass);
        }
        hipLaunchKernelGGL(topk_compact_kernel, dim3(grid), dim3(256), 0, s, scores, ids, n, st, k, keys_a, vals_a);
        SW_HIP(hipGetLastError());
        if (k <= 1024) {
            hipLaunchKernelGGL(topk_rank_emit_kernel, dim3(1), dim3(256), 0, s, keys_a, vals_a, k, out_scores, out_ids);
        } else {
            size_t cub = L.cub_bytes;
            SW_HIP(hipcub::DeviceRadixSort::SortPairsDescending(base + L.cub_off, cub, keys_a, keys_b, vals_a, vals_b, k, 0, 64, s));
            hipLaunchKernelGGL(topk_emit_kernel, dim3((k + 255) / 256), dim3(256), 0, s, keys_b, vals_b, k, out_scores, out_ids);
        }
        SW_HIP(hipGetLastError());
        return SW_OK;
    }
    float* keys = nullptr;
    int32_t* vals = nullptr;
    if (n > 0) {
        const TopkLayout L = topk_layout(n);
        if (!temp || temp_bytes < L.total) return fail(SW_ERR_TEMP, "temp buffer too small for top-K");
        char* base = static_cast<char*>(temp);
        keys = reinterpret_cast<float*>(base + L.keys_off);
        vals = reinterpret_cast<int32_t*>(base + L.vals_off);
        size_t cub = L.cub_bytes;
        SW_HIP(hipcub::DeviceRadixSort::SortPairsDescending(base + L.cub_off, cub, scores, keys, ids, vals, (int)n, 0, 32, s));
    }
    hipLaunchKernelGGL(topk_copy_kernel, dim3((k + 255) / 256), dim3(256), 0, s, keys, vals, n, k, out_scores, out_ids);
    SW_HIP(hipGetLastError());
    return SW_OK;
}

}
```

cudasw4_amd/csrc/sw_dp_kernel.hpp:

```cpp
#pragma once

#include <hip/hip_runtime.h>
#include <stdint.h>

#include <type_traits>

namespace swk {

typedef uint32_t u32;
typedef short s16x2 __attribute__((ext_vector_type(2)));
typedef unsigned short u16x2 __attribute__((ext_vector_type(2)));
typedef _Float16 f16x2 __attribute__((ext_vector_type(2)));

constexpr int kGroup = 16;
constexpr int kThreads = 256;
constexpr int kPadLetter = 20;
constexpr int kLetters = 21;

enum { F16X2 = 0, I16X2 = 1, I32 = 2, F32 = 3 };

constexpr int DPP_ROW_SHL1 = 0x101;
constexpr int DPP_ROW_SHR1 = 0x111;
constexpr int DPP_ROW_ROR1 = 0x121;
constexpr int DPP_QUAD_SHR1 = 0x90;
constexpr int DPP_WAVE_SHL1 = 0x130;
constexpr int DPP_WAVE_SHR1 = 0x138;

template <int LANES>
struct Shift {
    static_assert(LANES == 4 || LANES == 8 || LANES == 16 || LANES == 64, "group = a DPP quad, half a DPP row, a DPP row or the whole wave");
    static constexpr int kShr1 = LANES <= 16 ? DPP_ROW_SHR1 : DPP_WAVE_SHR1;
    static constexpr int kShl1 = LANES <= 16 ? DPP_ROW_SHL1 : DPP_WAVE_SHL1;
};

template <int CTRL, bool ZERO_FILL>
__device__ __forceinline__ u32 dpp(u32 old, u32 src) {
    return (u32)__builtin_amdgcn_update_dpp((int)old, (int)src, CTRL, 0xf, 0xf, ZERO_FILL);
}

template <int LANES, bool ZERO_FILL>
__device__ __forceinline__ u32 prev_lane(u32 headval, u32 src, bool head) {
    if constexpr (LANES == 8) {
        const u32 v = dpp<DPP_ROW_SHR1, false>(headval, src);
        return head ? headval : v;
    } else if constexpr (LANES == 4) {
        const u32 v = dpp<DPP_QUAD_SHR1, false>(headval, src);
        return head ? headval : v;
    } else {
        (void)head;
        return dpp<Shift<LANES>::kShr1, ZERO_FILL>(headval, src);
    }
}

#ifndef SWK_F32_WINDOW
#define SWK_F32_WINDOW 0
#endif
template <int KIND>
struct Arith;

template <>
struct Arith<I16X2> {
    static constexpr bool kPacked = true;
    static constexpr int kSubjects = 2;
    static constexpr int kLimit = 25000;
    static constexpr bool kWindow = true;
    static constexpr int kBias = 1024;
    static constexpr u32 kZero = (u32)kBias | ((u32)kBias << 16);
    static __host__ __device__ u32 encode_gap(int g) { u32 m = (u32)(-g) & 0xffffu; return m | (m << 16); }
    static __host__ __device__ u32 encode_score(int s) { return (u32)(uint16_t)(int16_t)s; }
    static __device__ __forceinline__ u32 add(u32 a, u32 b) {
        return __builtin_bit_cast(u32, (u16x2)(__builtin_bit_cast(u16x2, a) + __builtin_bit_cast(u16x2, b)));
    }
    static __device__ __forceinline__ u32 max3(u32 a, u32 b, u32 c) {
        return __builtin_bit_cast(u32, __builtin_elementwise_maximum(
            __builtin_elementwise_maximum(__builtin_bit_cast(f16x2, a), __builtin_bit_cast(f16x2, b)),
            __builtin_bit_cast(f16x2, c)));
    }
    static __device__ __forceinline__ u32 max2(u32 a, u32 b) {
        return __builtin_bit_cast(u32, __builtin_elementwise_maximum(__builtin_bit_cast(f16x2, a), __builtin_bit_cast(f16x2, b)));
    }
    static __device__ __forceinline__ u32 cell_h(u32 t, u32 e, u32 f) { return max3(t, e, f); }
    static __device__ __forceinline__ u32 gap(u32 a, u32 g) {
        return __builtin_bit_cast(u32, (u16x2)(__builtin_bit_cast(u16x2, a) - __builtin_bit_cast(u16x2, g)));
    }
    static __device__ __forceinline__ u32 gap_state(u32 ext, u32 open) { return max3(ext, open, kZero); }
    static __device__ __forceinline__ u32 fold2(u32 m, u32 a, u32 b) { return max3(m, a, b); }
    static __device__ __forceinline__ int score_lo(u32 v) { return (int)(v & 0xffffu) - kBias; }
    static __device__ __forceinline__ int score_hi(u32 v) { return (int)(v >> 16) - kBias; }
    static __host__ __device__ u32 zero_at(int a, int k) { u32 z = (u32)(kBias + a * k) & 0xffffu; return z | (z << 16); }
    static __host__ __device__ u32 pos_word(int a) { u32 m = (u32)a & 0xffffu; return m | (m << 16); }
    static __device__ __forceinline__ u32 level_word(int v) { const u32 z = (u32)(kBias + v) & 0xffffu; return z | (z << 16); }
    static __device__ __forceinline__ u32 true_of(u32 m, u32 z) { return gap(m, z); }
    static __device__ __forceinline__ u32 true_max(u32 a, u32 b) {
        return __builtin_bit_cast(u32, __builtin_elementwise_max(__builtin_bit_cast(u16x2, a), __builtin_bit_cast(u16x2, b)));
    }
    static __device__ __forceinline__ int true_lo(u32 v) { return (int)(v & 0xffffu); }
    static __device__ __forceinline__ int true_hi(u32 v) { return (int)(v >> 16); }
    static constexpr u32 kOne = 1u;
    static __device__ __forceinline__ u32 add_pair(u32 wa, u32 wb, u32 c) {
        u32 d;
        asm("v_pk_mad_u16 %0, %1, %2, %3 op_sel:[0,1,0] op_sel_hi:[1,0,1]" : "=v"(d) : "v"(wa), "v"(wb), "v"(c));
        return d;
    }
};

template <>
struct Arith<F16X2> {
    static constexpr bool kPacked = true;
    static constexpr int kSubjects = 2;
    static constexpr int kLimit = 2048;
    static constexpr bool kWindow = true;
    static constexpr u32 kZero = 0u;
    static __host__ __device__ u32 half_bits(int v) {
        if (v == 0) return 0;
        u32 sign = v < 0 ? 0x8000u : 0u;
        u32 a = (u32)(v < 0 ? -v : v);
        int e = 0;
        while ((a >> (e + 1)) != 0) e++;
        u32 mant = (a << (10 - e)) & 0x3ffu;
        return sign | ((u32)(e + 15) << 10) | mant;
    }
    static __host__ __device__ u32 encode_gap(int g) { u32 h = half_bits(g); return h | (h << 16); }
    static __host__ __device__ u32 encode_score(int s) { return half_bits(s); }
    static __device__ __forceinline__ u32 add(u32 a, u32 b) {
        return __builtin_bit_cast(u32, (f16x2)(__builtin_bit_cast(f16x2, a) + __builtin_bit_cast(f16x2, b)));
    }
    static __device__ __forceinline__ u32 max3(u32 a, u32 b, u32 c) {
        return __builtin_bit_cast(u32, __builtin_elementwise_maximum(
            __builtin_elementwise_maximum(__builtin_bit_cast(f16x2, a), __builtin_bit_cast(f16x2, b)),
            __builtin_bit_cast(f16x2, c)));
    }
    static __device__ __forceinline__ u32 max2(u32 a, u32 b) {
        return __builtin_bit_cast(u32, __builtin_elementwise_maximum(__builtin_bit_cast(f16x2, a), __builtin_bit_cast(f16x2, b)));
    }
    static __device__ __forceinline__ u32 cell_h(u32 t, u32 e, u32 f) { return max3(t, e, f); }
    static __device__ __forceinline__ u32 gap(u32 a, u32 g) { return add(a, g); }
    static __device__ __forceinline__ u32 gap_state(u32 ext, u32 open) { return max3(ext, open, 0u); }
    static __device__ __forceinline__ u32 fold2(u32 m, u32 a, u32 b) { return max3(m, a, b); }
    static __device__ __forceinline__ int score_lo(u32 v) { return (int)(float)__builtin_bit_cast(f16x2, v).x; }
    static __device__ __forceinline__ int score_hi(u32 v) { return (int)(float)__builtin_bit_cast(f16x2, v).y; }
    static __host__ __device__ u32 zero_at(int a, int k) { u32 h = half_bits(a * k); return h | (h << 16); }
    static __host__ __device__ u32 pos_word(int a) { u32 h = half_bits(a); return h | (h << 16); }
    static __device__ __forceinline__ u32 level_word(int v) {
        const u32 h = (u32)__builtin_bit_cast(unsigned short, (_Float16)(float)v);
        return h | (h << 16);
    }
    static __device__ __forceinline__ u32 true_of(u32 m, u32 z) {
        return __builtin_bit_cast(u32, (f16x2)(__builtin_bit_cast(f16x2, m) - __builtin_bit_cast(f16x2, z)));
    }
    static __device__ __forceinline__ u32 true_max(u32 a, u32 b) { return max2(a, b); }
    static __device__ __forceinline__ int true_lo(u32 v) { return score_lo(v); }
    static __device__ __forceinline__ int true_hi(u32 v) { return score_hi(v); }
    static constexpr u32 kOne = 0x3c00u;
    static __device__ __forceinline__ u32 add_pair(u32 wa, u32 wb, u32 c) {
        u32 d;
        asm("v_pk_fma_f16 %0, %1, %2, %3 op_sel:[0,1,0] op_sel_hi:[1,0,1]" : "=v"(d) : "v"(wa), "v"(wb), "v"(c));
        return d;
    }
};

template <>
struct Arith<I32> {
    static constexpr bool kPacked = false;
    static constexpr int kSubjects = 1;
    static constexpr int kLimit = 0x7fffffff;
    static constexpr bool kWindow = true;
    static constexpr u32 kZero = 0u;
    static __host__ __device__ u32 encode_gap(int g) { return (u32)g; }
    static __host__ __device__ u32 encode_score(int s) { return (u32)s; }
    static __device__ __forceinline__ u32 max3(u32 a, u32 b, u32 c) {
        u32 d;
        asm("v_max3_i32 %0, %1, %2, %3" : "=v"(d) : "v"(a), "v"(b), "v"(c));
        return d;
    }
    static __device__ __forceinline__ u32 max3_zero(u32 a, u32 b) {
        u32 d;
        asm("v_max3_i32 %0, %1, %2, 0" : "=v"(d) : "v"(a), "v"(b));
        return d;
    }
    static __device__ __forceinline__ u32 add(u32 a, u32 b) { return a + b; }
    static __device__ __forceinline__ u32 max2(u32 a, u32 b) { return (u32)((int)a > (int)b ? (int)a : (int)b); }
    static __device__ __forceinline__ u32 cell_h(u32 t, u32 e, u32 f) { return max3(t, e, f); }
    static __device__ __forceinline__ u32 gap(u32 a, u32 g) { return a + g; }
    static __device__ __forceinline__ u32 gap_state(u32 ext, u32 open) { return max3_zero(ext, open); }
    static __device__ __forceinline__ u32 fold2(u32 m, u32 a, u32 b) { return max3(m, a, b); }
    static __device__ __forceinline__ int score_lo(u32 v) { return (int)v; }
    static __device__ __forceinline__ int score_hi(u32) { return 0; }
    static __host__ __device__ u32 zero_at(int a, int k) { return (u32)(a * k); }
    static __host__ __device__ u32 pos_word(int a) { return (u32)a; }
    static __device__ __forceinline__ u32 true_of(u32 m, u32 z) { return m - z; }
    static __device__ __forceinline__ u32 true_max(u32 a, u32 b) { return max2(a, b); }
    static __device__ __forceinline__ int true_lo(u32 v) { return (int)v; }
    static __device__ __forceinline__ int true_hi(u32) { return 0; }
};

template <>
struct Arith<F32> {
    static constexpr bool kPacked = false;
    static constexpr int kSubjects = 1;
    static constexpr int kLimit = 0x7fffffff;
    static constexpr bool kWindow = SWK_F32_WINDOW != 0;
    static constexpr u32 kZero = 0u;
    static __host__ __device__ u32 encode_gap(int g) { return __builtin_bit_cast(u32, (float)g); }
    static __host__ __device__ u32 encode_score(int s) { return __builtin_bit_cast(u32, (float)s); }
    static __device__ __forceinline__ float f(u32 v) { return __builtin_bit_cast(float, v); }
    static __device__ __forceinline__ u32 u(float v) { return __builtin_bit_cast(u32, v); }
    static __device__ __forceinline__ u32 add(u32 a, u32 b) { return u(f(a) + f(b)); }
    static __device__ __forceinline__ u32 max2(u32 a, u32 b) { return u(__builtin_fmaxf(f(a), f(b))); }
    static __device__ __forceinline__ u32 max3(u32 a, u32 b, u32 c) { return u(__builtin_fmaxf(__builtin_fmaxf(f(a), f(b)), f(c))); }
    static __device__ __forceinline__ u32 cell_h(u32 t, u32 e, u32 ff) { return u(__builtin_fmaxf(__builtin_fmaxf(f(t), f(e)), f(ff))); }
    static __device__ __forceinline__ u32 gap(u32 a, u32 g) { return u(f(a) + f(g)); }
    static __device__ __forceinline__ u32 gap_state(u32 ext, u32 open) { return u(__builtin_fmaxf(__builtin_fmaxf(f(ext), f(open)), 0.0f)); }
    static __device__ __forceinline__ u32 fold2(u32 m, u32 a, u32 b) { return u(__builtin_fmaxf(__builtin_fmaxf(f(m), f(a)), f(b))); }
    static __device__ __forceinline__ int score_lo(u32 v) { return (int)f(v); }
    static __device__ __forceinline__ int score_hi(u32) { return 0; }
    static __host__ __device__ u32 zero_at(int a, int k) { return __builtin_bit_cast(u32, (float)(a * k)); }
    static __host__ __device__ u32 pos_word(int a) { return __builtin_bit_cast(u32, (float)a); }
    static __device__ __forceinline__ u32 true_of(u32 m, u32 z) { return u(f(m) - f(z)); }
    static __device__ __forceinline__ u32 true_max(u32 a, u32 b) { return max2(a, b); }
    static __device__ __forceinline__ int true_lo(u32 v) { return (int)f(v); }
    static __device__ __forceinline__ int true_hi(u32) { return 0; }
};

template <int NW>
struct Chunks {
    static constexpr int kRem = NW % 4;
    static constexpr int kWant3 = (4 - kRem) % 4;
    static constexpr bool kSplit = NW >= 3 * kWant3;
    static constexpr int kN3 = kSplit ? kWant3 : 1;
    static constexpr int kN4 = kSplit ? (NW - 3 * kWant3) / 4 : NW / 4;
    static constexpr int kCount = kN4 + kN3;
    static constexpr int first(int c) { return c < kN4 ? 4 * c : 4 * kN4 + 3 * (c - kN4); }
    static constexpr int words(int c) { return c < kN4 ? 4 : (kSplit ? 3 : kRem); }
    static constexpr int chunk_of(int w) { return w < 4 * kN4 ? w / 4 : kN4 + (w - 4 * kN4) / 3; }
    static constexpr bool starts_chunk(int w) { return first(chunk_of(w)) == w; }
    static constexpr bool lead_ok(int lead, int ahead, int slack) {
        for (int r = 0; r < NW; r++) {
            const int need = chunk_of(r + ahead < NW ? r + ahead : NW - 1);
            if (need >= lead && first(need - lead) + slack > r) return false;
        }
        return true;
    }
    static constexpr int lead_for(int ahead, int slack) {
        int lead = 1;
        while (lead < kCount && !lead_ok(lead, ahead, slack)) lead++;
        return lead;
    }
};

template <int KIND, int R, int LANES = kGroup>
struct Geometry {
    static constexpr bool kPacked = Arith<KIND>::kPacked;
    static constexpr bool kWide = kPacked && LANES <= 16;
    static constexpr int NW = (kPacked && !kWide) ? (R + 1) / 2 : R;
    using C = Chunks<NW>;
    static constexpr int NCH = C::kCount;
    static constexpr int kChunkRowBytes = (LANES <= 16 ? 16 : LANES) * 16;
    static constexpr int kRowBytes = NCH * kChunkRowBytes;
    static constexpr int kTileBytes = kLetters * kRowBytes;
    static constexpr int kStripeRows = LANES * R;
    static constexpr int kLetterShift = LANES <= 16 ? 8 : 10;
    static constexpr int kLetterUnits = kRowBytes >> kLetterShift;
    static_assert(kPadLetter * kLetterUnits < 256, "letter offset must fit a byte");
};

struct ScanParams {
    const int8_t* chars;
    const uint64_t* offsets;
    const int32_t* lengths;
    const int32_t* positions;
    const int32_t* count_ptr;
    int32_t first_pos;
    int32_t n;
    const unsigned char* profile;
    int32_t nstripes;
    u32 gop, gex;
    float* scores;
    int32_t* ids;
    int64_t id_offset;
    int32_t* ovf_pos;
    int32_t* ovf_count;
    int32_t ovf_check;
    u32* scratch;
    int32_t lcap;
    const u32* zeros;
    u32* work_counter;
    int32_t gex_mag;
    int32_t renorm_quads;
    u32 renorm_word;
    u32 wrap_class;
    u32 wrap_last;
    int32_t* stat_count;
    int32_t stat_limit;
    u32* start_signal;
    u32 start_quorum;
    int32_t* claim;
    int32_t service;
    const u32* done_flag;
    u32 done_value;
    u32* dry_signal;
    u32 dry_value;
    int32_t stream_slots;
    int32_t stream_cols;
    int32_t stream_room;
    int32_t level_base;
    int32_t jump;
    u32 jump_word;
    int32_t jump_limit;
};

constexpr int32_t kListEmpty = -1, kListTaken = -2;

typedef u32 u32x3 __attribute__((ext_vector_type(3)));

template <int NW, int CHUNK_ROW_BYTES>
__device__ __forceinline__ void lds_read_chunk(u32 (&dst)[NW], const unsigned char* p, int c) {
    using C = Chunks<NW>;
    const int w = C::first(c);
    if (c < C::kN4) {
        const uint4 v = *reinterpret_cast<const uint4*>(p + c * CHUNK_ROW_BYTES);
        dst[w + 0] = v.x; dst[w + 1] = v.y; dst[w + 2] = v.z; dst[w + 3] = v.w;
    } else if (c < C::kCount) {
        const u32x3 v = *reinterpret_cast<const u32x3*>(p + c * CHUNK_ROW_BYTES);
        if constexpr (C::kSplit) {
            dst[w + 0] = v.x; dst[w + 1] = v.y; dst[w + 2] = v.z;
        } else {
            u32 x = v.x;
            if constexpr (C::kRem == 1) asm("" : "+v"(x) : "v"(v.y), "v"(v.z));
            if constexpr (C::kRem == 2) asm("" : "+v"(x) : "v"(v.z));
            dst[w] = x;
            if constexpr (C::kRem == 2) dst[w + 1] = v.y;
        }
    }
}

template <int NW, int CHUNK_ROW_BYTES>
__device__ __forceinline__ void lds_read_words(u32 (&dst)[NW], const unsigned char* p) {
#pragma unroll
    for (int c = 0; c < Chunks<NW>::kCount; c++) lds_read_chunk<NW, CHUNK_ROW_BYTES>(dst, p, c);
}

#ifndef SWK_WAVES3_MAX_R
#define SWK_WAVES3_MAX_R 36
#endif
#ifndef SWK_WAVES3_MAX_R_MULTI
#define SWK_WAVES3_MAX_R_MULTI 32
#endif
#ifndef SWK_MULTI_SCALAR_LOOP
#define SWK_MULTI_SCALAR_LOOP 1
#endif
#ifndef SWK_WAVES4_MAX_R
#define SWK_WAVES4_MAX_R 22
#endif
#ifndef SWK_CLASSES_PACKED
#define SWK_CLASSES_PACKED 8
#endif
#ifndef SWK_CLASSES_PACKED_SMALL
#define SWK_CLASSES_PACKED_SMALL 4
#endif
#ifndef SWK_CLASSES_SCALAR
#define SWK_CLASSES_SCALAR 4
#endif
constexpr int frame_classes(bool packed, int R, int lanes, bool multi) {
    (void)lanes;
    const int want = packed ? ((R > SWK_WAVES3_MAX_R || (multi && R >= 25 && R > SWK_WAVES3_MAX_R_MULTI)) ? SWK_CLASSES_PACKED : SWK_CLASSES_PACKED_SMALL)
                            : SWK_CLASSES_SCALAR;
    int P = want;
    while (P > 1 && 2 * P > R) P--;
    return P;
}

template <int NW, int CHUNK_ROW_BYTES>
__device__ __forceinline__ void lds_read_chunk2(u32 (&da)[NW], u32 (&db)[NW], const unsigned char* pa, const unsigned char* pb, int c) {
    lds_read_chunk<NW, CHUNK_ROW_BYTES>(da, pa, c);
    lds_read_chunk<NW, CHUNK_ROW_BYTES>(db, pb, c);
    __builtin_amdgcn_sched_barrier(0);
}

template <int NW, int CHUNK_ROW_BYTES>
__device__ __forceinline__ void lds_read_words2(u32 (&da)[NW], u32 (&db)[NW], const unsigned char* pa, const unsigned char* pb) {
#pragma unroll
    for (int c = 0; c < Chunks<NW>::kCount; c++) lds_read_chunk2<NW, CHUNK_ROW_BYTES>(da, db, pa, pb, c);
}

template <int NW, int CHUNK_ROW_BYTES>
__device__ __forceinline__ void lds_read_chunk1(u32 (&da)[NW], const unsigned char* pa, int c) {
    lds_read_chunk<NW, CHUNK_ROW_BYTES>(da, pa, c);
    __builtin_amdgcn_sched_barrier(0);
}

template <int KIND, int R, int P = 1>
struct StripeState {
    u32 H[R];
    u32 E[R];
    u32 upH_prev;
    u32 Hlast;
    u32 Fout;
    u32 yA, yB;
    u32 maxv[P + 3];
    u32 Zc[P + 4];
};

template <int KIND, int R, int LANES, int BYTE, bool MULTI, bool OFFS = false, int P = 1, bool ZFILL = true>
__device__ __forceinline__ void dp_step(StripeState<KIND, R, P>& st, const unsigned char* tile,
                                        u32 lettersA, u32 lettersB, u32 gop, u32 gex, u32 inH, u32 inF,
                                        u32 apos = 0, bool first = false, u32 wrapP = 0, u32 wrapLast = 0, bool head = false,
                                        u32 laneStep = 0) {
    using A = Arith<KIND>;
    using G = Geometry<KIND, R, LANES>;
    const u32 step2 = LANES < 16 ? laneStep : 0x00100010u;
    const u32 step1 = LANES < 16 ? laneStep : 16u;
    constexpr u32 kSel = 0x0c0c000cu | ((u32)BYTE << 8);
    constexpr int kPostShift = G::kLetterShift - 8;

#ifndef SWK_PROG_SCALAR
#define SWK_PROG_SCALAR 1
#endif
    constexpr bool kProgScalar = SWK_PROG_SCALAR != 0;
    u32 wa[G::NW];
    u32 wb[G::NW];
    if constexpr (A::kPacked && LANES <= 16) {
        constexpr u32 kSel2 = ((u32)(4 + BYTE) << 24) | 0x000c000cu | ((u32)BYTE << 8);
        const u32 inj = __builtin_amdgcn_perm(lettersB, lettersA, kSel2);
        st.yA = prev_lane<LANES, false>(inj, st.yA, head) + step2;
        if constexpr (!OFFS) lds_read_words2<G::NW, G::kChunkRowBytes>(wa, wb, tile + (st.yA & 0xffffu), tile + (st.yA >> 16));
    } else {
        const u32 injA = __builtin_amdgcn_perm(0u, lettersA, kSel) << kPostShift;
        st.yA = prev_lane<LANES, false>(injA, st.yA, head) + step1;
        if constexpr (A::kPacked || !OFFS || !kProgScalar) lds_read_words<G::NW, G::kChunkRowBytes>(wa, tile + st.yA);
        if constexpr (A::kPacked) {
            const u32 injB = __builtin_amdgcn_perm(0u, lettersB, kSel) << kPostShift;
            st.yB = prev_lane<LANES, false>(injB, st.yB, head) + step1;
            lds_read_words<G::NW, G::kChunkRowBytes>(wb, tile + st.yB);
        }
    }

    if constexpr (OFFS) {
        constexpr int kLastClass = (R - 1) % P;
        constexpr int Q = A::kWindow ? BYTE : 0;
        u32 upH, F;
        if constexpr (MULTI) {
            (void)first;
            upH = prev_lane<LANES, false>(inH, st.Hlast, head);
            F = prev_lane<LANES, false>(inF, st.Fout, head);
        } else {
            const u32 bH = st.Zc[Q + kLastClass];
            upH = prev_lane<LANES, false>(bH, st.Hlast, head);
            if constexpr (ZFILL) F = prev_lane<LANES, true>(0u, st.Fout, head);
            else F = prev_lane<LANES, false>(st.Zc[Q], st.Fout, head);
        }
        u32 diag = st.upH_prev;
        st.upH_prev = upH;
        u32 m[P];
#pragma unroll
        for (int c = 0; c < P; c++) m[c] = A::kWindow ? st.maxv[Q + c] : A::add(st.maxv[c], apos);
        auto score = [&](int r) -> u32 {
            if constexpr (G::kWide) return 0u;
            else if constexpr (A::kPacked) return __builtin_amdgcn_perm(wb[r >> 1], wa[r >> 1], (r & 1) ? 0x07060302u : 0x05040100u);
            else return wa[r];
        };
        auto diag_term = [&](int, u32 d, u32 sc) -> u32 { return A::add(d, sc); };
#ifndef SWK_LOOKAHEAD
#define SWK_LOOKAHEAD 12
#endif
        constexpr int kAhead = G::kWide ? (SWK_LOOKAHEAD < R ? SWK_LOOKAHEAD : R) : 1;
        using CH = Chunks<G::NW>;
        constexpr int kChunksAll = CH::kCount;
        constexpr int kChunks0 = G::kWide ? CH::lead_for(kAhead, 4) : 1;
        static_assert(!G::kWide || kChunks0 >= kChunksAll || CH::lead_ok(kChunks0, kAhead, 4), "a score word would be used before its read is issued");
        const unsigned char* const pa = tile + (st.yA & 0xffffu);
        const unsigned char* const pb = tile + (st.yA >> 16);
        u32 tq[G::kWide ? R : 1];
        if constexpr (G::kWide) {
#pragma unroll
            for (int k = 0; k < kChunks0 && k < kChunksAll; k++) lds_read_chunk2<G::NW, G::kChunkRowBytes>(wa, wb, pa, pb, k);
#pragma unroll
            for (int r = 0; r < kAhead; r++) tq[r] = A::add_pair(wa[r], wb[r], r == 0 ? diag : st.H[r - 1]);
        }
        constexpr bool kProg1 = !A::kPacked && kProgScalar;
        constexpr int kChunks0S = kProg1 ? CH::lead_for(2, 6) : 1;
        if constexpr (kProg1) {
#pragma unroll
            for (int k = 0; k < kChunks0S && k < kChunksAll; k++) lds_read_chunk1<G::NW, G::kChunkRowBytes>(wa, tile + st.yA, k);
        }
        u32 s_next = score(0);
        u32 t_next = G::kWide ? 0u : diag_term(0, diag, s_next);
        s_next = R > 1 ? score(1) : 0u;
#pragma unroll
        for (int r = 0; r < R; r++) {
            const int c = r % P;
            const u32 zop = st.Zc[Q + c + 1];
            if constexpr (G::kWide) {
                if (r % 4 == 0) __builtin_amdgcn_sched_barrier(0);
                if (CH::starts_chunk(r) && CH::chunk_of(r) + kChunks0 < kChunksAll)
                    lds_read_chunk2<G::NW, G::kChunkRowBytes>(wa, wb, pa, pb, CH::chunk_of(r) + kChunks0);
                t_next = tq[r];
            }
            if constexpr (kProg1) {
                if (r % 4 == 0) __builtin_amdgcn_sched_barrier(0);
                if (CH::starts_chunk(r) && CH::chunk_of(r) + kChunks0S < kChunksAll)
                    lds_read_chunk1<G::NW, G::kChunkRowBytes>(wa, tile + st.yA, CH::chunk_of(r) + kChunks0S);
            }
            const u32 t = t_next;
            const u32 h = A::cell_h(t, st.E[r], F);
            const u32 s1 = s_next;
            if (r + 2 < R) s_next = score(r + 2);
            const u32 hg = A::gap(h, gop);
            if constexpr (G::kWide) {
                if (r + kAhead < R) tq[r + kAhead] = A::add_pair(wa[r + kAhead], wb[r + kAhead], st.H[r + kAhead - 1]);
            } else {
                if (r + 1 < R) t_next = diag_term(r + 1, st.H[r], s1);
            }
            const u32 fm = A::max3(F, hg, zop);
            st.E[r] = A::max3(st.E[r], hg, zop);
            if (c == P - 1) F = A::gap(fm, wrapP);
            else if (r == R - 1) F = A::gap(fm, wrapLast);
            else F = fm;
            if ((r / P) & 1) m[c] = A::fold2(m[c], st.H[r - P], h);
            else if (r + P >= R) m[c] = A::max2(m[c], h);
            st.H[r] = h;
        }
#pragma unroll
        for (int c = 0; c < P; c++) st.maxv[Q + c] = m[c];
        if constexpr (!A::kWindow) {
#pragma unroll
            for (int k = (kLastClass == 0 ? 0 : 1); k <= P; k++) st.Zc[k] = A::add(st.Zc[k], apos);
        }
        st.Hlast = st.H[R - 1];
        st.Fout = F;
        return;
    }

    u32 upH, F;
    if constexpr (MULTI) {
        upH = prev_lane<LANES, false>(inH, st.Hlast, head);
        F = prev_lane<LANES, false>(inF, st.Fout, head);
    } else if constexpr (A::kZero == 0u) {
        upH = prev_lane<LANES, true>(0u, st.Hlast, head);
        F = prev_lane<LANES, true>(0u, st.Fout, head);
    } else {
        upH = prev_lane<LANES, false>(A::kZero, st.Hlast, head);
        F = prev_lane<LANES, false>(A::kZero, st.Fout, head);
    }
    u32 diag = st.upH_prev;
    st.upH_prev = upH;

    u32 maxv = st.maxv[0];
#pragma unroll
    for (int r = 0; r < R; r++) {
        u32 t;
        if constexpr (G::kWide) {
            t = A::add_pair(wa[r], wb[r], diag);
        } else if constexpr (A::kPacked) {
            t = A::add(diag, __builtin_amdgcn_perm(wb[r >> 1], wa[r >> 1], (r & 1) ? 0x07060302u : 0x05040100u));
        } else {
            t = A::add(diag, wa[r]);
        }
        diag = st.H[r];
        const u32 h = A::cell_h(t, st.E[r], F);
        const u32 hg = A::gap(h, gop);
        st.E[r] = A::gap_state(A::gap(st.E[r], gex), hg);
        F = A::gap_state(A::gap(F, gex), hg);
        st.H[r] = h;
        if (r & 1) maxv = A::fold2(maxv, st.H[r - 1], h);
        else if (r == R - 1) maxv = A::max2(maxv, h);
    }
    st.maxv[0] = maxv;
    st.Hlast = st.H[R - 1];
    st.Fout = F;
}

template <int TILE_BYTES>
__device__ __forceinline__ void load_tile(unsigned char* lds, const unsigned char* gsrc) {
    static_assert(TILE_BYTES % 16 == 0, "tile must be 16-byte granular");
    const uint4* src = reinterpret_cast<const uint4*>(gsrc);
    uint4* dst = reinterpret_cast<uint4*>(lds + 16);
    for (int i = threadIdx.x; i < TILE_BYTES / 16; i += kThreads) dst[i] = src[i];
}

template <class MAX>
__device__ __forceinline__ u32 half_row_max(u32 v, MAX&& mx) {
    v = mx(v, dpp<0x141, false>(v, v));
    v = mx(v, dpp<0xB1, false>(v, v));
    v = mx(v, dpp<0x4E, false>(v, v));
    return v;
}

template <class MAX>
__device__ __forceinline__ u32 quad_max(u32 v, MAX&& mx) {
    v = mx(v, dpp<0xB1, false>(v, v));
    v = mx(v, dpp<0x4E, false>(v, v));
    return v;
}

template <int KIND, int LANES>
__device__ __forceinline__ u32 group_max(u32 v) {
    using A = Arith<KIND>;
    if constexpr (LANES == 8) return half_row_max(v, [](u32 a, u32 b) { return A::max2(a, b); });
    if constexpr (LANES == 4) return quad_max(v, [](u32 a, u32 b) { return A::max2(a, b); });
    v = A::max2(v, dpp<0x128, false>(v, v));
    v = A::max2(v, dpp<0x124, false>(v, v));
    v = A::max2(v, dpp<0x122, false>(v, v));
    v = A::max2(v, dpp<0x121, false>(v, v));
    if constexpr (LANES == 64) {
        v = A::max2(v, (u32)__shfl_xor((int)v, 16));
        v = A::max2(v, (u32)__shfl_xor((int)v, 32));
    }
    return v;
}

#ifndef SWK_BORDER_PEND
#define SWK_BORDER_PEND 1
#endif
template <int LANES>
struct Border {
    static constexpr int kBlockCols = 2 * LANES;
    static constexpr int kQuadsPerBlock = LANES / 2;
    static constexpr int kBlockBytes = 8 * kBlockCols;
    static constexpr int kBlockWords = 2 * kBlockCols;
    static constexpr int kInBytes = kBlockBytes, kOutBytes = kBlockBytes, kDummyBytes = 8 * (kThreads / LANES) + 32;
    static constexpr int kGroupBytes = kInBytes + kOutBytes + 16;
    static constexpr int ring_bytes(int groups) { return groups * kGroupBytes + kDummyBytes; }
    static_assert(kGroupBytes % 16 == 0, "rings are read and written 16 bytes at a time");
    static constexpr int blocks(int steps) { return (steps + kBlockCols - 1) / kBlockCols + 3; }
};
template <int LANES>
constexpr int border_region_words(int lcap) { return Border<LANES>::blocks(lcap) * Border<LANES>::kBlockWords; }

#ifndef SWK_MIN_WAVES_SCALAR
#define SWK_MIN_WAVES_SCALAR 0
#endif
#ifndef SWK_I32_WAVES3_MAX_R
#define SWK_I32_WAVES3_MAX_R 32
#endif
#ifndef SWK_I32_WAVES3_MAX_R_MULTI
#define SWK_I32_WAVES3_MAX_R_MULTI 32
#endif
#ifndef SWK_F32_WAVES3_MAX_R
#define SWK_F32_WAVES3_MAX_R 48
#endif
#ifndef SWK_F32_WAVES3_MAX_R_MULTI
#define SWK_F32_WAVES3_MAX_R_MULTI 48
#endif
constexpr int min_waves_of(int KIND, int R, int LANES, bool MULTI) {
    const bool packed = KIND == F16X2 || KIND == I16X2;
    if (packed && LANES <= 16 && MULTI && R <= SWK_WAVES3_MAX_R_MULTI) return 3;
    if (packed) return (LANES <= 16 && !MULTI && R <= SWK_WAVES4_MAX_R) ? 4 : (LANES <= 16 && !MULTI && R <= SWK_WAVES3_MAX_R) ? 3 : 2;
    if (SWK_MIN_WAVES_SCALAR > 0) return SWK_MIN_WAVES_SCALAR;
    if (KIND == I32 && LANES <= 16 && R > (MULTI ? SWK_I32_WAVES3_MAX_R_MULTI : SWK_I32_WAVES3_MAX_R)) return 2;
    if (KIND == F32 && LANES <= 16 && R > (MULTI ? SWK_F32_WAVES3_MAX_R_MULTI : SWK_F32_WAVES3_MAX_R)) return 2;
    return (R <= 16 && !MULTI && LANES <= 16) ? 4 : 3;
}
template <int KIND, int R, int LANES, bool MULTI>
constexpr int min_waves() { return min_waves_of(KIND, R, LANES, MULTI); }
constexpr int vgpr_slot_of(int KIND, int R, int LANES, bool MULTI) { return (512 / min_waves_of(KIND, R, LANES, MULTI)) & ~7; }

template <int KIND, int R, int LANES, bool MULTI, bool OFFS = false>
__global__ void __launch_bounds__(kThreads, (min_waves<KIND, R, LANES, MULTI>())) sw_scan_kernel(const ScanParams p) {
    using A = Arith<KIND>;
    using G = Geometry<KIND, R, LANES>;
    constexpr int kGroups = kThreads / LANES;
    using BD = Border<LANES>;
    constexpr int SHL1 = Shift<LANES>::kShl1;
    constexpr int kQuadsPerLetterBlock = LANES;
    constexpr int P = OFFS ? frame_classes(A::kPacked, R, LANES, MULTI) : 1;
    __shared__ __attribute__((aligned(16))) unsigned char lds[16 + G::kTileBytes];
    __shared__ __attribute__((aligned(16))) unsigned char rings[MULTI ? BD::ring_bytes(kGroups) : 16];

    const int tid = threadIdx.x;
    const int lane = tid & (LANES - 1);
    const int group = tid / LANES;
    const bool head = lane == 0;
    const int slot = LANES < 16 ? (tid & 15) : lane;
    const u32 laneStep = (A::kPacked ? 0x00100010u : 16u) * ((LANES < 16 && head) ? u32(slot + 1) : 1u);
    if (p.start_signal && tid == 0) {
        if (atomicAdd(p.work_counter + 1, 1u) + 1u == p.start_quorum)
            __hip_atomic_fetch_add(p.start_signal, 1u, __ATOMIC_RELEASE, __HIP_MEMORY_SCOPE_SYSTEM);
    }
    if (p.positions) __builtin_amdgcn_s_setprio(2);
    const bool service = p.service != 0;
    const int n = (p.count_ptr && !service) ? *p.count_ptr : p.n;
    constexpr int kSubjPerBatch = kGroups * A::kSubjects;
    const int nbatches = (n + kSubjPerBatch - 1) / kSubjPerBatch;
    if (!service && (int)blockIdx.x >= nbatches) return;

    if constexpr (!MULTI) {
        load_tile<G::kTileBytes>(lds, p.profile);
        __syncthreads();
    }

    unsigned char* const ringIn = rings + (MULTI ? group * BD::kGroupBytes : 0);
    unsigned char* const ringOut = ringIn + BD::kInBytes;
    u32* const gBorder = MULTI ? p.scratch + ((size_t)blockIdx.x * kGroups + group) * (size_t)border_region_words<LANES>(p.lcap) : nullptr;

    const u32 apos = OFFS ? A::pos_word(p.gex_mag) : 0u;
    const u32 apos4 = OFFS ? A::pos_word(4 * p.gex_mag) : 0u;
    constexpr bool kLowers = OFFS && A::kPacked;
    const int rq = kLowers ? p.renorm_quads : 0;
    const u32 zstart = OFFS ? A::zero_at(p.gex_mag, LANES - lane) : A::kZero;
    const u32 zbefore = OFFS ? A::zero_at(p.gex_mag, LANES - lane - 1) : A::kZero;

    __shared__ int next_batch, batch_avail;
    auto claim_entry = [&](int i) -> int {
        for (int spin = 0; spin < (1 << 20); spin++) {
            const int v = __hip_atomic_load(p.claim + i, __ATOMIC_RELAXED, __HIP_MEMORY_SCOPE_AGENT);
            if (v == kListTaken) return -1;
            if (v >= 0) return atomicCAS(p.claim + i, v, kListTaken) == v ? v : -1;
            __builtin_amdgcn_s_sleep(2);
        }
        return -1;
    };
    for (;;) {
        __syncthreads();
        if (tid == 0) {
            int b = (int)atomicAdd(p.work_counter, 1u), avail = n;
            if (service) {
                avail = 0;
                for (u32 spin = 0; b < nbatches; spin++) {
                    avail = __hip_atomic_load(p.count_ptr, __ATOMIC_RELAXED, __HIP_MEMORY_SCOPE_AGENT);
                    if (avail > b * kSubjPerBatch) break;
                    const u32 done = __hip_atomic_load(p.done_flag, __ATOMIC_RELAXED, __HIP_MEMORY_SCOPE_SYSTEM);
                    if ((int32_t)(done - p.done_value) >= 0 || spin > 600000u) { b = nbatches; break; }
                    __builtin_amdgcn_s_sleep(127);
                }
                avail = min(avail, n);
            }
            if (b == nbatches && p.dry_signal) __hip_atomic_store(p.dry_signal, p.dry_value, __ATOMIC_RELAXED, __HIP_MEMORY_SCOPE_SYSTEM);
            next_batch = b;
            batch_avail = avail;
        }
        __syncthreads();
        const int b = next_batch;
        if (b >= nbatches) break;
        const int navail = batch_avail;
        const int batch = service ? b : nbatches - 1 - b;
        const int i0 = batch * kSubjPerBatch + group * A::kSubjects;
        const int i1 = i0 + 1;
        bool valid0 = i0 < navail;
        bool valid1 = A::kPacked && (i1 < navail);
        int pos0 = 0, pos1 = 0, len0 = 0, len1 = 0;
        const int8_t* s0 = p.chars;
        const int8_t* s1 = p.chars;
        if (p.claim) {
            int v = -1;
            if (valid0 && lane == 0) v = claim_entry(i0);
            if constexpr (LANES == 64) v = __builtin_amdgcn_readfirstlane(v);
            else v = __shfl(v, (tid & 63) & ~(LANES - 1));
            valid0 = v >= 0;
            pos0 = valid0 ? v : 0;
            if (valid0) {
                len0 = p.lengths[pos0];
                s0 = p.chars + (p.offsets[pos0] - p.offsets[0]);
            }
            valid1 = false;
        } else {
            if (valid0) {
                pos0 = p.positions ? p.positions[i0] : p.first_pos + i0;
                len0 = p.lengths[pos0];
                s0 = p.chars + (p.offsets[pos0] - p.offsets[0]);
            }
            if (valid1) {
                pos1 = p.positions ? p.positions[i1] : p.first_pos + i1;
                len1 = p.lengths[pos1];
                s1 = p.chars + (p.offsets[pos1] - p.offsets[0]);
            }
        }
        int lmax = len0 > len1 ? len0 : len1;
        if constexpr (LANES <= 16) {
            if constexpr (LANES <= 4) lmax = max(lmax, __shfl_xor(lmax, 4));
            if constexpr (LANES <= 8) lmax = max(lmax, __shfl_xor(lmax, 8));
            lmax = max(lmax, __shfl_xor(lmax, 16));
            lmax = max(lmax, __shfl_xor(lmax, 32));
        }
        int nquads = (lmax + LANES - 1 + 3) >> 2;
        if constexpr (MULTI) nquads = min(nquads, (p.lcap - 4) >> 2);
        if constexpr (!MULTI || SWK_MULTI_SCALAR_LOOP) nquads = __builtin_amdgcn_readfirstlane(nquads);
        const int len0pad = (len0 + 3) & ~3, len1pad = (len1 + 3) & ~3;

        u32 maxv = OFFS ? 0u : A::kZero;
        for (int stripe = 0; stripe < p.nstripes; stripe++) {
            const bool first = stripe == 0;
            if constexpr (MULTI) {
                __syncthreads();
                load_tile<G::kTileBytes>(lds, p.profile + (size_t)stripe * G::kTileBytes);
                __syncthreads();
            }
            StripeState<KIND, R, P> st;
            {
                u32 zc[P + 5];
                zc[0] = zbefore; zc[1] = zstart;
#pragma unroll
                for (int k = 2; k < P + 5; k++) zc[k] = A::add(zc[k - 1], apos);
#pragma unroll
                for (int r = 0; r < R; r++) { st.H[r] = zc[r % P]; st.E[r] = zc[r % P + 1]; }
                st.upH_prev = zc[(R - 1) % P]; st.Hlast = zc[(R - 1) % P]; st.Fout = zbefore;
#pragma unroll
                for (int k = 0; k < P + 4; k++) st.Zc[k] = zc[k + 1];
#pragma unroll
                for (int d = 0; d < P + 3; d++) st.maxv[d] = OFFS ? A::add(maxv, zc[A::kWindow ? d + 1 : d]) : maxv;
            }
            st.yA = ((u32)(kPadLetter * G::kLetterUnits) << G::kLetterShift) + 16u * (u32)(slot + 1);
            st.yB = st.yA;
            if constexpr (A::kPacked && LANES <= 16) st.yA |= st.yA << 16;

            auto fetch = [&](const int8_t* s, int lenpad, int blk) -> u32 {
                const int j = blk * (4 * LANES) + lane * 4;
                u32 w = 0x14141414u;
                if (j < lenpad) w = *reinterpret_cast<const u32*>(s + j);
                return w * (u32)G::kLetterUnits;
            };
            u32 nextA = fetch(s0, len0pad, 0);
            u32 nextB = A::kPacked ? fetch(s1, len1pad, 0) : 0u;
            u32 lettersA = 0, lettersB = 0;

            const bool last = stripe + 1 == p.nstripes;
            const unsigned char* inPtr = ringIn;
            unsigned char* outPtr = (lane == LANES - 1) ? ringOut : rings + kGroups * BD::kGroupBytes + 8 * group;
            const u32 walkIn = 32u;
            const u32 walkOut = (lane == LANES - 1) ? 32u : 0u;
            uint4 pend = make_uint4(A::kZero, A::kZero, A::kZero, A::kZero);
            uint2 nxt = make_uint2(A::kZero, A::kZero);
            const u32* const gIn = MULTI ? gBorder + 2 * (LANES - 1) + 4 * lane : nullptr;
            auto first_stripe_pairs = [&](int j) -> uint4 {
                if constexpr (OFFS) {
                    constexpr int kLastClass = (R - 1) % P;
                    const int K = 4 * rq;
                    const int j0 = K > 0 ? (j & (K - 1)) : j, j1 = K > 0 ? ((j + 1) & (K - 1)) : j + 1;
                    return make_uint4(A::zero_at(p.gex_mag, j0 + LANES + kLastClass), A::kZero, A::zero_at(p.gex_mag, j1 + LANES + kLastClass), A::kZero);
                } else {
                    return make_uint4(A::kZero, A::kZero, A::kZero, A::kZero);
                }
            };
            if constexpr (MULTI) {
                __builtin_amdgcn_fence(__ATOMIC_ACQUIRE, "workgroup");
                if (!first) {
                    const uint4 b0 = *reinterpret_cast<const uint4*>(gIn);
#if SWK_BORDER_PEND
                    pend = *reinterpret_cast<const uint4*>(gIn + BD::kBlockWords);
#endif
                    *reinterpret_cast<uint4*>(ringIn + 16 * lane) = b0;
                } else {
                    *reinterpret_cast<uint4*>(ringIn + 16 * lane) = first_stripe_pairs(2 * lane);
                }
                __builtin_amdgcn_fence(__ATOMIC_RELEASE, "wavefront");
                nxt = *reinterpret_cast<const uint2*>(inPtr);
            }
            auto block_end = [&](int blk) {
                int t = tid;
                asm volatile("" : "+v"(t));
                const int ln = t & (LANES - 1), grp = t / LANES;
                unsigned char* const rIn = rings + grp * BD::kGroupBytes + 16 * ln;
                u32* const gb = p.scratch + ((size_t)blockIdx.x * kGroups + grp) * (size_t)border_region_words<LANES>(p.lcap) + 4 * ln;
                __builtin_amdgcn_fence(__ATOMIC_ACQ_REL, "wavefront");
                if (!last) {
                    const uint4 v = *reinterpret_cast<const uint4*>(rIn + BD::kInBytes);
                    *reinterpret_cast<uint4*>(gb + (size_t)blk * BD::kBlockWords) = v;
                }
                outPtr -= walkOut * BD::kQuadsPerBlock;
                inPtr -= walkIn * BD::kQuadsPerBlock;
                if (first) {
                    *reinterpret_cast<uint4*>(rIn) = first_stripe_pairs((blk + 1) * BD::kBlockCols + 2 * ln);
                } else {
#if SWK_BORDER_PEND
                    *reinterpret_cast<uint4*>(rIn) = pend;
                    pend = *reinterpret_cast<const uint4*>(gb + 2 * (LANES - 1) + (size_t)(blk + 2) * BD::kBlockWords);
#else
                    *reinterpret_cast<uint4*>(rIn) = *reinterpret_cast<const uint4*>(gb + 2 * (LANES - 1) + (size_t)(blk + 1) * BD::kBlockWords);
#endif
                }
                __builtin_amdgcn_fence(__ATOMIC_ACQ_REL, "wavefront");
                nxt = *reinterpret_cast<const uint2*>(inPtr);
            };

            auto quad = [&](int q, auto lower_tag) {
                constexpr bool LOWER = decltype(lower_tag)::value;
                if ((q & (kQuadsPerLetterBlock - 1)) == 0) {
                    lettersA = nextA; lettersB = nextB;
                    nextA = fetch(s0, len0pad, q / kQuadsPerLetterBlock + 1);
                    if constexpr (A::kPacked) nextB = fetch(s1, len1pad, q / kQuadsPerLetterBlock + 1);
                }
                const int lower_lane = 4 * (q & (rq - 1));
                auto lower_frame = [&](int k) {
                    const u32 gw = lane == k ? p.renorm_word : 0u;
#pragma unroll
                    for (int r = 0; r < R; r++) { st.H[r] = A::gap(st.H[r], gw); st.E[r] = A::gap(st.E[r], gw); }
                    st.upH_prev = A::gap(st.upH_prev, gw);
#pragma unroll
                    for (int k = 0; k < P + 4; k++) st.Zc[k] = A::gap(st.Zc[k], gw);
#pragma unroll
                    for (int d = 0; d < P + 3; d++) st.maxv[d] = A::gap(st.maxv[d], gw);
                };
                auto border_step = [&](auto byte_tag) {
                    constexpr int BYTE = decltype(byte_tag)::value;
                    const uint2 in = nxt;
                    if constexpr (MULTI) {
                        if constexpr (BYTE == 3) {
                            inPtr += walkIn;
                            nxt = *reinterpret_cast<const uint2*>(inPtr);
                        } else {
                            nxt = *reinterpret_cast<const uint2*>(inPtr + 8 * (BYTE + 1));
                        }
                    }
                    dp_step<KIND, R, LANES, BYTE, MULTI, OFFS, P>(st, lds, lettersA, lettersB, p.gop, p.gex, in.x, in.y, apos, first, p.wrap_class, p.wrap_last, head, laneStep);
                    if constexpr (MULTI) *reinterpret_cast<uint2*>(outPtr + 8 * BYTE) = make_uint2(st.Hlast, st.Fout);
                };
                if constexpr (LOWER) lower_frame(lower_lane + 0);
                border_step(std::integral_constant<int, 0>{});
                if constexpr (LOWER) lower_frame(lower_lane + 1);
                border_step(std::integral_constant<int, 1>{});
                if constexpr (LOWER) lower_frame(lower_lane + 2);
                border_step(std::integral_constant<int, 2>{});
                if constexpr (LOWER) lower_frame(lower_lane + 3);
                border_step(std::integral_constant<int, 3>{});
                if constexpr (MULTI) outPtr += walkOut;
                lettersA = dpp<SHL1, true>(0u, lettersA);
                if constexpr (A::kPacked) lettersB = dpp<SHL1, true>(0u, lettersB);
                if constexpr (OFFS && A::kWindow) {
#pragma unroll
                    for (int k = 0; k < P + 4; k++) st.Zc[k] = A::add(st.Zc[k], apos4);
#pragma unroll
                    for (int d = 0; d < P + 3; d++) st.maxv[d] = A::add(st.maxv[d], apos4);
                }
            };
            if constexpr (!MULTI) {
                const int seg = (kLowers && rq > 0) ? rq : nquads;
                for (int q0 = 0; q0 < nquads; q0 += seg) {
                    const int qend = min(nquads, q0 + seg);
                    int q = q0;
                    if constexpr (kLowers) {
                        if (q0 > 0) {
                            const int qlow = min(qend, q0 + LANES / 4);
                            for (; q < qlow; q++) quad(q, std::true_type{});
                        }
                    }
                    for (; q < qend; q++) quad(q, std::false_type{});
                }
            } else {
                static_assert(BD::kQuadsPerBlock >= LANES / 4, "the lowering quads of a period must lie in one block");
                for (int q0 = 0; q0 < nquads; q0 += BD::kQuadsPerBlock) {
                    const int qend = min(nquads, q0 + BD::kQuadsPerBlock);
                    int q = q0;
                    if constexpr (kLowers) {
                        if (rq > 0 && q0 > 0 && (q0 & (rq - 1)) == 0) {
                            const int qlow = min(qend, q0 + LANES / 4);
                            for (; q < qlow; q++) quad(q, std::true_type{});
                        }
                    }
                    for (; q < qend; q++) quad(q, std::false_type{});
                    if (qend == q0 + BD::kQuadsPerBlock) block_end(q0 / BD::kQuadsPerBlock);
                }
            }
            if constexpr (MULTI) {
                if (!last) {
                    const int done = nquads & ~(BD::kQuadsPerBlock - 1);
                    const int slot = 4 * (nquads - done) + lane;
                    u32* const g = gBorder + (size_t)(done / BD::kQuadsPerBlock) * BD::kBlockWords;
                    __builtin_amdgcn_fence(__ATOMIC_ACQ_REL, "wavefront");
                    if (slot < BD::kBlockCols) *reinterpret_cast<uint2*>(ringOut + 8 * slot) = make_uint2(A::kZero, A::kZero);
                    else *reinterpret_cast<uint2*>(g + 2 * slot) = make_uint2(A::kZero, A::kZero);
                    __builtin_amdgcn_fence(__ATOMIC_ACQ_REL, "wavefront");
                    *reinterpret_cast<uint4*>(g + 4 * lane) = *reinterpret_cast<const uint4*>(ringOut + 16 * lane);
                }
            }
            if constexpr (OFFS) {
                if constexpr (A::kWindow) {
                    maxv = A::true_of(st.maxv[0], st.Zc[0]);
#pragma unroll
                    for (int d = 1; d < P + 3; d++) maxv = A::true_max(maxv, A::true_of(st.maxv[d], st.Zc[d]));
                } else {
                    maxv = A::true_of(st.maxv[0], A::gap(A::gap(st.Zc[1], p.gex), p.gex));
#pragma unroll
                    for (int c = 1; c < P; c++)
                        maxv = A::true_max(maxv, A::true_of(st.maxv[c], A::gap(A::gap(st.Zc[c + 1], p.gex), p.gex)));
                }
            } else {
                maxv = st.maxv[0];
            }
            if constexpr (MULTI) __builtin_amdgcn_fence(__ATOMIC_RELEASE, "workgroup");
        }

        int sc0, sc1, guard = 0;
        if constexpr (OFFS) {
            if constexpr (LANES == 8) {
                maxv = half_row_max(maxv, [](u32 a, u32 b) { return A::true_max(a, b); });
            } else if constexpr (LANES == 4) {
                maxv = quad_max(maxv, [](u32 a, u32 b) { return A::true_max(a, b); });
            } else {
                maxv = A::true_max(maxv, dpp<0x128, false>(maxv, maxv));
                maxv = A::true_max(maxv, dpp<0x124, false>(maxv, maxv));
                maxv = A::true_max(maxv, dpp<0x122, false>(maxv, maxv));
                maxv = A::true_max(maxv, dpp<0x121, false>(maxv, maxv));
            }
            if constexpr (LANES == 64) {
                maxv = A::true_max(maxv, (u32)__shfl_xor((int)maxv, 16));
                maxv = A::true_max(maxv, (u32)__shfl_xor((int)maxv, 32));
            }
            sc0 = A::true_lo(maxv);
            sc1 = A::true_hi(maxv);
            guard = p.gex_mag * ((rq > 0 && 4 * nquads > 4 * rq ? 4 * rq : 4 * nquads) + 2 * LANES + 4 + P);
        } else {
            maxv = group_max<KIND, LANES>(maxv);
            sc0 = A::score_lo(maxv);
            sc1 = A::score_hi(maxv);
        }
        if (lane == 0) {
            if (valid0) {
                if (A::kPacked && p.ovf_check && sc0 >= A::kLimit - guard) {
                    __hip_atomic_store(p.ovf_pos + atomicAdd(p.ovf_count, 1), pos0, __ATOMIC_RELAXED, __HIP_MEMORY_SCOPE_AGENT);
                } else {
                    p.scores[pos0] = (float)sc0;
                    if (p.stat_count && sc0 >= p.stat_limit) atomicAdd(p.stat_count, 1);
                }
                p.ids[pos0] = (int32_t)(p.id_offset + pos0);
            }
            if (valid1) {
                if (p.ovf_check && sc1 >= A::kLimit - guard) {
                    __hip_atomic_store(p.ovf_pos + atomicAdd(p.ovf_count, 1), pos1, __ATOMIC_RELAXED, __HIP_MEMORY_SCOPE_AGENT);
                } else {
                    p.scores[pos1] = (float)sc1;
                }
                p.ids[pos1] = (int32_t)(p.id_offset + pos1);
            }
        }
    }
}

template <int KIND, int R, int LANES>
__global__ void sw_build_profile_kernel(const int8_t* __restrict__ query, int32_t qlen,
                                        const int8_t* __restrict__ matrix21, int32_t pad_row, int32_t nstripes,
                                        unsigned char* __restrict__ profile, int32_t shift) {
    using A = Arith<KIND>;
    using G = Geometry<KIND, R, LANES>;
    constexpr int kWordsPerRow = G::kRowBytes / 4;
    constexpr int kWordsPerChunkRow = G::kChunkRowBytes / 4;
    const size_t total = (size_t)nstripes * kLetters * kWordsPerRow;
    u32* out = reinterpret_cast<u32*>(profile);
    for (size_t i = (size_t)blockIdx.x * blockDim.x + threadIdx.x; i < total; i += (size_t)gridDim.x * blockDim.x) {
        const int word = (int)(i % kWordsPerRow);
        const int letter = (int)((i / kWordsPerRow) % kLetters);
        const int stripe = (int)(i / ((size_t)kWordsPerRow * kLetters));
        const int chunk = word / kWordsPerChunkRow, lane = ((word % kWordsPerChunkRow) / 4) % LANES, sub = word % 4;
        const int w = G::C::first(chunk) + sub;
        u32 v = 0;
        if (sub < G::C::words(chunk) && w < G::NW) {
            auto entry = [&](int row_in_lane) -> u32 {
                if (row_in_lane >= R) return 0u;
                const int64_t row = (int64_t)stripe * G::kStripeRows + lane * R + row_in_lane;
                const int qc = row < qlen ? (int)query[row] : pad_row;
                const int P = frame_classes(A::kPacked, R, LANES, nstripes > 1);
                const int cls = row_in_lane % P, above = (row_in_lane == 0 ? R - 1 : row_in_lane - 1) % P;
                return A::encode_score((int)matrix21[qc * kLetters + letter] + shift * (1 + cls - above));
            };
            if constexpr (G::kWide) v = w < R ? (entry(w) | (A::kOne << 16)) : 0u;
            else if constexpr (A::kPacked) v = entry(2 * w) | (entry(2 * w + 1) << 16);
            else v = entry(w);
        }
        out[i] = v;
    }
}

}
```

cudasw4_amd/csrc/sw_kind_f16x2.hip:

```cpp
#include "sw_launch.hpp"

namespace swk {
#define SWK_CASE_SCAN16_F16X2(R) case R: return launch_scan_r<F16X2, R, 16>(multi, offs, grid, reserve, stream, p);
#define SWK_CASE_SCAN64_F16X2(R) case R: return launch_scan_r<F16X2, R, 64>(multi, offs, grid, reserve, stream, p);
#define SWK_CASE_PROF16_F16X2(R) case R: return launch_profile_r<F16X2, R, 16>(q, qlen, m, pr, ns, out, shift, s);
#define SWK_CASE_PROF64_F16X2(R) case R: return launch_profile_r<F16X2, R, 64>(q, qlen, m, pr, ns, out, shift, s);
#define SWK_CASE_TILE16_F16X2(R) case R: return tile_bytes_r<F16X2, R, 16>();
#define SWK_CASE_TILE64_F16X2(R) case R: return tile_bytes_r<F16X2, R, 64>();
#define SWK_CASE_SCAN8_F16X2(R) case R: return launch_scan_r<F16X2, R, 8>(multi, offs, grid, reserve, stream, p);
#define SWK_CASE_PROF8_F16X2(R) case R: return launch_profile_r<F16X2, R, 8>(q, qlen, m, pr, ns, out, shift, s);
#define SWK_CASE_TILE8_F16X2(R) case R: return tile_bytes_r<F16X2, R, 8>();
#define SWK_CASE_SCAN4_F16X2(R) case R: return launch_scan_r<F16X2, R, 4>(multi, offs, grid, reserve, stream, p);
#define SWK_CASE_PROF4_F16X2(R) case R: return launch_profile_r<F16X2, R, 4>(q, qlen, m, pr, ns, out, shift, s);
#define SWK_CASE_TILE4_F16X2(R) case R: return tile_bytes_r<F16X2, R, 4>();
SWK_DEFINE_KIND(launch_f16x2, F16X2, SWK_FOR_EACH_R_PACKED)
}
```

cudasw4_amd/csrc/sw_kind_f32.hip:

```cpp
#include "sw_launch.hpp"

namespace swk {
#define SWK_CASE_SCAN16_F32(R) case R: return launch_scan_r<F32, R, 16>(multi, offs, grid, reserve, stream, p);
#define SWK_CASE_SCAN64_F32(R) case R: return launch_scan_r<F32, R, 64>(multi, offs, grid, reserve, stream, p);
#define SWK_CASE_PROF16_F32(R) case R: return launch_profile_r<F32, R, 16>(q, qlen, m, pr, ns, out, shift, s);
#define SWK_CASE_PROF64_F32(R) case R: return launch_profile_r<F32, R, 64>(q, qlen, m, pr, ns, out, shift, s);
#define SWK_CASE_TILE16_F32(R) case R: return tile_bytes_r<F32, R, 16>();
#define SWK_CASE_TILE64_F32(R) case R: return tile_bytes_r<F32, R, 64>();
#define SWK_CASE_SCAN8_F32(R) case R: return launch_scan_r<F32, R, 8>(multi, offs, grid, reserve, stream, p);
#define SWK_CASE_PROF8_F32(R) case R: return launch_profile_r<F32, R, 8>(q, qlen, m, pr, ns, out, shift, s);
#define SWK_CASE_TILE8_F32(R) case R: return tile_bytes_r<F32, R, 8>();
#define SWK_CASE_SCAN4_F32(R) case R: return launch_scan_r<F32, R, 4>(multi, offs, grid, reserve, stream, p);
#define SWK_CASE_PROF4_F32(R) case R: return launch_profile_r<F32, R, 4>(q, qlen, m, pr, ns, out, shift, s);
#define SWK_CASE_TILE4_F32(R) case R: return tile_bytes_r<F32, R, 4>();
SWK_DEFINE_KIND(launch_f32, F32, SWK_FOR_EACH_R_I32)
}
```

cudasw4_amd/csrc/sw_kind_i16x2.hip:

```cpp
#include "sw_launch.hpp"

namespace swk {
#define SWK_CASE_SCAN16_I16X2(R) case R: return launch_scan_r<I16X2, R, 16>(multi, offs, grid, reserve, stream, p);
#define SWK_CASE_SCAN64_I16X2(R) case R: return launch_scan_r<I16X2, R, 64>(multi, offs, grid, reserve, stream, p);
#define SWK_CASE_PROF16_I16X2(R) case R: return launch_profile_r<I16X2, R, 16>(q, qlen, m, pr, ns, out, shift, s);
#define SWK_CASE_PROF64_I16X2(R) case R: return launch_profile_r<I16X2, R, 64>(q, qlen, m, pr, ns, out, shift, s);
#define SWK_CASE_TILE16_I16X2(R) case R: return tile_bytes_r<I16X2, R, 16>();
#define SWK_CASE_TILE64_I16X2(R) case R: return tile_bytes_r<I16X2, R, 64>();
#define SWK_CASE_SCAN8_I16X2(R) case R: return launch_scan_r<I16X2, R, 8>(multi, offs, grid, reserve, stream, p);
#define SWK_CASE_PROF8_I16X2(R) case R: return launch_profile_r<I16X2, R, 8>(q, qlen, m, pr, ns, out, shift, s);
#define SWK_CASE_TILE8_I16X2(R) case R: return tile_bytes_r<I16X2, R, 8>();
#define SWK_CASE_SCAN4_I16X2(R) case R: return launch_scan_r<I16X2, R, 4>(multi, offs, grid, reserve, stream, p);
#define SWK_CASE_PROF4_I16X2(R) case R: return launch_profile_r<I16X2, R, 4>(q, qlen, m, pr, ns, out, shift, s);
#define SWK_CASE_TILE4_I16X2(R) case R: return tile_bytes_r<I16X2, R, 4>();
SWK_DEFINE_KIND(launch_i16x2, I16X2, SWK_FOR_EACH_R_PACKED)
}
```

cudasw4_amd/csrc/sw_kind_i32.hip:

```cpp
#include "sw_launch.hpp"

namespace swk {
#define SWK_CASE_SCAN16_I32(R) case R: return launch_scan_r<I32, R, 16>(multi, offs, grid, reserve, stream, p);
#define SWK_CASE_SCAN64_I32(R) case R: return launch_scan_r<I32, R, 64>(multi, offs, grid, reserve, stream, p);
#define SWK_CASE_PROF16_I32(R) case R: return launch_profile_r<I32, R, 16>(q, qlen, m, pr, ns, out, shift, s);
#define SWK_CASE_PROF64_I32(R) case R: return launch_profile_r<I32, R, 64>(q, qlen, m, pr, ns, out, shift, s);
#define SWK_CASE_TILE16_I32(R) case R: return tile_bytes_r<I32, R, 16>();
#define SWK_CASE_TILE64_I32(R) case R: return tile_bytes_r<I32, R, 64>();
#define SWK_CASE_SCAN8_I32(R) case R: return launch_scan_r<I32, R, 8>(multi, offs, grid, reserve, stream, p);
#define SWK_CASE_PROF8_I32(R) case R: return launch_profile_r<I32, R, 8>(q, qlen, m, pr, ns, out, shift, s);
#define SWK_CASE_TILE8_I32(R) case R: return tile_bytes_r<I32, R, 8>();
#define SWK_CASE_SCAN4_I32(R) case R: return launch_scan_r<I32, R, 4>(multi, offs, grid, reserve, stream, p);
#define SWK_CASE_PROF4_I32(R) case R: return launch_profile_r<I32, R, 4>(q, qlen, m, pr, ns, out, shift, s);
#define SWK_CASE_TILE4_I32(R) case R: return tile_bytes_r<I32, R, 4>();
SWK_DEFINE_KIND(launch_i32, I32, SWK_FOR_EACH_R_I32)
}
```

cudasw4_amd/csrc/sw_launch.hpp:

```cpp
#pragma once
#include <hip/hip_runtime.h>

#include <algorithm>
#include <atomic>

#include "sw_dp_kernel.hpp"
#include "sw_stream_kernel.hpp"

namespace swk {

constexpr int kRowsGranule = 1;
#ifndef SWK_MAX_ROWS_PACKED
#define SWK_MAX_ROWS_PACKED 48
#endif
constexpr int kMaxRowsPacked = SWK_MAX_ROWS_PACKED;
#ifndef SWK_MAX_ROWS_SCALAR
#define SWK_MAX_ROWS_SCALAR 36
#endif
constexpr int kMaxRowsScalar = SWK_MAX_ROWS_SCALAR;
#ifndef SWK_MAX_ROWS_SCALAR_MULTI
#define SWK_MAX_ROWS_SCALAR_MULTI 32
#endif
constexpr int kMaxRowsScalarMulti = SWK_MAX_ROWS_SCALAR_MULTI;
#ifndef SWK_MAX_ROWS_I32
#define SWK_MAX_ROWS_I32 48
#endif
constexpr int kMaxRowsI32 = SWK_MAX_ROWS_I32;
constexpr int kWaves3MaxRowsPackedMulti = SWK_WAVES3_MAX_R_MULTI;
constexpr int kMaxRowsPackedLong = 16;
constexpr int kMaxRowsScalarLong = 8;
constexpr int kMaxRowsShortGroups = 32;
constexpr int max_rows(int kind, int lanes) {
    const bool packed = kind == F16X2 || kind == I16X2;
    if (lanes < 16) return kMaxRowsShortGroups;
    return lanes == 16 ? (packed ? kMaxRowsPacked : kind == I32 ? kMaxRowsI32 : kMaxRowsScalar) : (packed ? kMaxRowsPackedLong : kMaxRowsScalarLong);
}

struct KindLaunch {
    hipError_t (*scan)(int R, int lanes, bool multi, bool offs, int grid, int reserve, hipStream_t stream, const ScanParams& p);
    hipError_t (*profile)(int R, int lanes, const int8_t* query, int32_t qlen, const int8_t* matrix21, int32_t pad_row,
                          int32_t nstripes, unsigned char* out, int32_t shift, hipStream_t stream);
    size_t (*tile_bytes)(int R, int lanes);
    hipError_t (*warm)(hipStream_t stream);
    bool packed;
};

const KindLaunch& launch_f16x2();
const KindLaunch& launch_i16x2();
const KindLaunch& launch_i32();
const KindLaunch& launch_f32();

template <class K>
int resident_workgroups(K kernel) {
    static std::atomic<int> cached[64];
    int dev = 0;
    if (hipGetDevice(&dev) != hipSuccess || dev < 0 || dev >= 64) return 0;
    int v = cached[dev].load(std::memory_order_relaxed);
    if (v == 0) {
        int per_cu = 0, cus = 0;
        if (hipOccupancyMaxActiveBlocksPerMultiprocessor(&per_cu, kernel, kThreads, 0) != hipSuccess ||
            hipDeviceGetAttribute(&cus, hipDeviceAttributeMultiprocessorCount, dev) != hipSuccess || per_cu <= 0 || cus <= 0) {
            (void)hipGetLastError();
            v = -1;
        } else {
            v = per_cu * cus;
        }
        cached[dev].store(v, std::memory_order_relaxed);
    }
    return v > 0 ? v : 0;
}

template <class K>
hipError_t launch_scan_k(K kernel, int grid, int reserve, hipStream_t stream, const ScanParams& p) {
    if (reserve > 0) {
        const int resident = resident_workgroups(kernel);
        if (resident > 0 && grid > resident - reserve) {
            ScanParams q = p;
            grid = resident - reserve > 1 ? resident - reserve : 1;
            if (q.start_quorum > (u32)grid) q.start_quorum = (u32)grid;
            hipLaunchKernelGGL(kernel, dim3(grid), dim3(kThreads), 0, stream, q);
            return hipGetLastError();
        }
    }
    hipLaunchKernelGGL(kernel, dim3(grid), dim3(kThreads), 0, stream, p);
    return hipGetLastError();
}

template <int KIND, int R, int LANES, bool OFFS>
hipError_t launch_scan_ro(bool multi, int grid, int reserve, hipStream_t stream, const ScanParams& p) {
    constexpr int kMaxR = max_rows(KIND, LANES);
    constexpr bool kPacked = Arith<KIND>::kPacked;
    if constexpr (R > kMaxR || (kPacked && !OFFS)) {
        return hipErrorInvalidValue;
    } else if constexpr (kPacked && LANES == 16) {
        if (p.positions || p.claim || p.service || p.count_ptr || p.stream_slots < 1) return hipErrorInvalidValue;
        if (multi) {
            if constexpr (2 * R > kMaxR) {
                if (p.stream_slots > 1) return launch_scan_k(sw_scan_stream_kernel<KIND, R, LANES, true>, grid, reserve, stream, p);
                return launch_scan_k(sw_scan_kernel<KIND, R, LANES, true, OFFS>, grid, reserve, stream, p);
            } else {
                return hipErrorInvalidValue;
            }
        } else {
            return launch_scan_k(sw_scan_stream_kernel<KIND, R, LANES, false>, grid, reserve, stream, p);
        }
    } else {
        if (multi) {
            if constexpr (2 * R > kMaxR && LANES >= 16) {
                return launch_scan_k(sw_scan_kernel<KIND, R, LANES, true, OFFS>, grid, reserve, stream, p);
            } else {
                return hipErrorInvalidValue;
            }
        } else {
            return launch_scan_k(sw_scan_kernel<KIND, R, LANES, false, OFFS>, grid, reserve, stream, p);
        }
    }
}

template <int KIND, int R, int LANES>
hipError_t launch_scan_r(bool multi, bool offs, int grid, int reserve, hipStream_t stream, const ScanParams& p) {
    return offs ? launch_scan_ro<KIND, R, LANES, true>(multi, grid, reserve, stream, p)
                : launch_scan_ro<KIND, R, LANES, false>(multi, grid, reserve, stream, p);
}

template <int KIND, int R, int LANES>
hipError_t launch_profile_r(const int8_t* query, int32_t qlen, const int8_t* matrix21, int32_t pad_row, int32_t nstripes,
                            unsigned char* out, int32_t shift, hipStream_t stream) {
    if constexpr (R > max_rows(KIND, LANES)) {
        return hipErrorInvalidValue;
    } else {
        const size_t total = (size_t)nstripes * kLetters * (Geometry<KIND, R, LANES>::kRowBytes / 4);
        const int grid = (int)std::min<size_t>((total + 255) / 256, 65536);
        hipLaunchKernelGGL((sw_build_profile_kernel<KIND, R, LANES>), dim3(grid), dim3(256), 0, stream, query, qlen,
                           matrix21, pad_row, nstripes, out, shift);
        return hipGetLastError();
    }
}

template <int KIND, int R, int LANES>
constexpr size_t tile_bytes_r() {
    if constexpr (R > max_rows(KIND, LANES)) return 0;
    else return (size_t)Geometry<KIND, R, LANES>::kTileBytes;
}

#define SWK_FOR_EACH_R_PACKED(X) \
    X(1) X(2) X(3) X(4) X(5) X(6) X(7) X(8) X(9) X(10) X(11) X(12) X(13) X(14) X(15) X(16) X(17) X(18) X(19) X(20) X(21) X(22) X(23) X(24) X(25) X(26) X(27) X(28) X(29) X(30) X(31) X(32) X(33) X(34) X(35) X(36) X(37) X(38) X(39) X(40) X(41) X(42) X(43) X(44) X(45) X(46) X(47) X(48)
#define SWK_FOR_EACH_R_I32(X) SWK_FOR_EACH_R_PACKED(X)
#define SWK_FOR_EACH_R_SCALAR(X) \
    X(1) X(2) X(3) X(4) X(5) X(6) X(7) X(8) X(9) X(10) X(11) X(12) X(13) X(14) X(15) X(16) X(17) X(18) X(19) X(20) X(21) X(22) X(23) X(24) X(25) X(26) X(27) X(28) X(29) X(30) X(31) X(32)

#define SWK_DEFINE_KIND(FN, KIND, FOR_EACH_R)                                                                      \
    static hipError_t FN##_scan(int R, int lanes, bool multi, bool offs, int grid, int reserve, hipStream_t stream, \
                                const ScanParams& p) {                                                              \
        if (lanes == 16) { switch (R) { FOR_EACH_R(SWK_CASE_SCAN16_##KIND) } }                                      \
        else if (lanes == 64) { switch (R) { FOR_EACH_R(SWK_CASE_SCAN64_##KIND) } }                                 \
        else if (lanes == 8) { switch (R) { FOR_EACH_R(SWK_CASE_SCAN8_##KIND) } }                                   \
        else if (lanes == 4) { switch (R) { FOR_EACH_R(SWK_CASE_SCAN4_##KIND) } }                                   \
        return hipErrorInvalidValue;                                                                                \
    }                                                                                                               \
    static hipError_t FN##_profile(int R, int lanes, const int8_t* q, int32_t qlen, const int8_t* m, int32_t pr,    \
                                   int32_t ns, unsigned char* out, int32_t shift, hipStream_t s) {                  \
        if (lanes == 16) { switch (R) { FOR_EACH_R(SWK_CASE_PROF16_##KIND) } }                                      \
        else if (lanes == 64) { switch (R) { FOR_EACH_R(SWK_CASE_PROF64_##KIND) } }                                 \
        else if (lanes == 8) { switch (R) { FOR_EACH_R(SWK_CASE_PROF8_##KIND) } }                                   \
        else if (lanes == 4) { switch (R) { FOR_EACH_R(SWK_CASE_PROF4_##KIND) } }                                   \
        return hipErrorInvalidValue;                                                                                \
    }                                                                                                               \
    static size_t FN##_tile_bytes(int R, int lanes) {                                                               \
        if (lanes == 16) { switch (R) { FOR_EACH_R(SWK_CASE_TILE16_##KIND) } }                                      \
        else if (lanes == 64) { switch (R) { FOR_EACH_R(SWK_CASE_TILE64_##KIND) } }                                 \
        else if (lanes == 8) { switch (R) { FOR_EACH_R(SWK_CASE_TILE8_##KIND) } }                                   \
        else if (lanes == 4) { switch (R) { FOR_EACH_R(SWK_CASE_TILE4_##KIND) } }                                   \
        return 0;                                                                                                   \
    }                                                                                                               \
    static __global__ void FN##_warm_kernel() {}                                                                    \
    static hipError_t FN##_warm(hipStream_t s) {                                                                    \
        hipLaunchKernelGGL(FN##_warm_kernel, dim3(1), dim3(64), 0, s);                                              \
        return hipGetLastError();                                                                                   \
    }                                                                                                               \
    const KindLaunch& FN() {                                                                                        \
        static const KindLaunch k{FN##_scan, FN##_profile, FN##_tile_bytes, FN##_warm, Arith<KIND>::kPacked};       \
        return k;                                                                                                   \
    }

}
```

Measured before the change: 11650 GCUPS.

## Use a wave-uniform frame offset table for packed column-offset kernels

Packed kernels with the column-offset recurrence now read their frame baseline words from a per-launch table of level words in kernel params, loaded into scalar registers per quad. This replaces the per-lane Zc register arrays and their per-quad increments. Renormalization becomes one uniform lowering of all state every K columns instead of a lane-staggered lowering at each step. A third profile variant with an extra head offset is built to match. The aim is to cut VGPR pressure and vector ALU work in the inner loop, at the cost of larger kernel arguments, scalar loads each quad, and a cap on the renormalization period.

Measured after the change: 11930 GCUPS (median of 6 runs). 2.4% higher.

```diff
diff --git a/cudasw4_amd/csrc/sw_api.hip b/cudasw4_amd/csrc/sw_api.hip
--- a/cudasw4_amd/csrc/sw_api.hip
+++ b/cudasw4_amd/csrc/sw_api.hip
@@ -144,7 +144,7 @@
     int query_next = 0;
     int32_t qlen = 0;
     bool have_query = false;
-    Profile profiles[4][4][2];
+    Profile profiles[4][4][3];
     bool use_offs = true;
     int64_t long16_min = -1;
     int64_t long16_min_default = -1;
@@ -207,8 +207,8 @@
 }
 
 
-int ensure_profile(sw_ctx* ctx, int kind, int lanes, bool offs, int shift, hipStream_t stream) {
-    Profile& pr = ctx->profiles[kind][shape_index(lanes)][offs];
+int ensure_profile(sw_ctx* ctx, int kind, int lanes, int frame, int shift, hipStream_t stream) {
+    Profile& pr = ctx->profiles[kind][shape_index(lanes)][frame];
     if (pr.valid && pr.shift != shift) pr.valid = false;
     if (pr.valid) {
         SW_HIP(hipStreamWaitEvent(stream, pr.ready, 0));
@@ -226,7 +226,7 @@
         SW_HIP(hipMalloc(&pr.dev, cap));
         pr.capacity = cap;
     }
-    SW_HIP(kl->profile(pl.rows, lanes, ctx->d_query, ctx->qlen, ctx->d_matrix, ctx->dim, pl.nstripes, pr.dev, shift, stream));
+    SW_HIP(kl->profile(pl.rows, lanes, ctx->d_query, ctx->qlen, ctx->d_matrix, ctx->dim, pl.nstripes, pr.dev, shift, frame == 2 ? 1 : 0, stream));
     pr.shift = shift;
     if (!pr.ready) SW_HIP(hipEventCreateWithFlags(&pr.ready, hipEventDisableTiming));
     SW_HIP(hipEventRecord(pr.ready, stream));
@@ -341,9 +341,13 @@
     int64_t K = 0;
     const bool offs = offs_possible(ctx, kind, lanes, max_subject_len, gop, gex, ovf_check, &K);
     if (kind_packed(kind) && !offs) return fail(SW_ERR_INVALID, "internal: a packed launch without the column-offset recurrence (packed_fallback_kind)");
-    int rc = ensure_profile(ctx, kind, lanes, offs, offs ? a : 0, stream);
+    const QueryPlan plan0 = plan_query(kind, ctx->qlen, lanes);
+    const StreamPlan sp = stream_plan(ctx, kind, lanes, a, plan0, max_subject_len);
+    const bool uniform = swk::uniform_frame_launch(kl->packed, offs, lanes, plan0.nstripes > 1, sp.slots);
+    const int frame = offs ? (uniform ? 2 : 1) : 0;
+    int rc = ensure_profile(ctx, kind, lanes, frame, offs ? a : 0, stream);
     if (rc != SW_OK) return rc;
-    const Profile& prof = ctx->profiles[kind][shape_index(lanes)][offs];
+    const Profile& prof = ctx->profiles[kind][shape_index(lanes)][frame];
     const QueryPlan pl = prof.plan;
     const bool multi = pl.nstripes > 1;
 
@@ -377,8 +381,8 @@
         }
         p.gex_mag = a;
         {
-            const int P = swk::frame_classes(kl->packed, pl.rows, lanes, multi);
-            const int wrap = -a * P, wrap_last = -a * ((pl.rows - 1) % P + 1);
+            const int P = swk::frame_classes(kl->packed, pl.rows, lanes, multi, uniform);
+            const int wrap = -a * P, wrap_last = -a * ((pl.rows - 1) % P + (uniform ? 0 : 1));
             switch (kind) {
                 case SW_KIND_F16X2: p.wrap_class = swk::Arith<swk::F16X2>::encode_gap(wrap); p.wrap_last = swk::Arith<swk::F16X2>::encode_gap(wrap_last); break;
                 case SW_KIND_I16X2: p.wrap_class = swk::Arith<swk::I16X2>::encode_gap(wrap); p.wrap_last = swk::Arith<swk::I16X2>::encode_gap(wrap_last); break;
@@ -386,6 +390,8 @@
                 default: p.wrap_class = swk::Arith<swk::F32>::encode_gap(wrap); p.wrap_last = swk::Arith<swk::F32>::encode_gap(wrap_last); break;
             }
         }
+        p.flag_period = (int32_t)K;
+        if (uniform) K = std::min<int64_t>(K, swk::kUniformMaxPeriod);
         p.renorm_quads = (int32_t)(K / 4);
         const int lower = -(int)((int64_t)a * K);
         switch (kind) {
@@ -394,8 +400,13 @@
             case SW_KIND_I32: p.renorm_word = swk::Arith<swk::I32>::encode_gap(lower); break;
             default: p.renorm_word = swk::Arith<swk::F32>::encode_gap(lower); break;
         }
-    }
-    const StreamPlan sp = stream_plan(ctx, kind, lanes, a, pl, max_subject_len);
+        if (uniform) {
+            p.uniform_frame = 1;
+            for (int u = 0; u < swk::kLevelWords; u++)
+                p.levels[u] = kind == SW_KIND_F16X2 ? swk::Arith<swk::F16X2>::zero_at(a, std::min<int>(u, (int)K + 16))
+                                                    : swk::Arith<swk::I16X2>::zero_at(a, std::min<int>(u, (int)K + 16));
+        }
+    }
     if (sp.slots >= 1) {
         p.stream_slots = sp.slots; p.stream_cols = sp.cols; p.stream_room = sp.room; p.level_base = sp.base;
         p.jump = sp.jump; p.jump_limit = sp.jump - 4;
diff --git a/cudasw4_amd/csrc/sw_dp_kernel.hpp b/cudasw4_amd/csrc/sw_dp_kernel.hpp
--- a/cudasw4_amd/csrc/sw_dp_kernel.hpp
+++ b/cudasw4_amd/csrc/sw_dp_kernel.hpp
@@ -91,6 +91,9 @@
     static __host__ __device__ u32 pos_word(int a) { u32 m = (u32)a & 0xffffu; return m | (m << 16); }
     static __device__ __forceinline__ u32 level_word(int v) { const u32 z = (u32)(kBias + v) & 0xffffu; return z | (z << 16); }
     static __device__ __forceinline__ u32 true_of(u32 m, u32 z) { return gap(m, z); }
+    static __device__ __forceinline__ u32 lower(u32 a, u32 w) {
+        return __builtin_bit_cast(u32, __builtin_elementwise_sub_sat(__builtin_bit_cast(u16x2, a), __builtin_bit_cast(u16x2, w)));
+    }
     static __device__ __forceinline__ u32 true_max(u32 a, u32 b) {
         return __builtin_bit_cast(u32, __builtin_elementwise_max(__builtin_bit_cast(u16x2, a), __builtin_bit_cast(u16x2, b)));
     }
@@ -148,6 +151,7 @@
     static __device__ __forceinline__ u32 true_of(u32 m, u32 z) {
         return __builtin_bit_cast(u32, (f16x2)(__builtin_bit_cast(f16x2, m) - __builtin_bit_cast(f16x2, z)));
     }
+    static __device__ __forceinline__ u32 lower(u32 a, u32 w) { return add(a, w); }
     static __device__ __forceinline__ u32 true_max(u32 a, u32 b) { return max2(a, b); }
     static __device__ __forceinline__ int true_lo(u32 v) { return score_lo(v); }
     static __device__ __forceinline__ int true_hi(u32 v) { return score_hi(v); }
@@ -263,6 +267,9 @@
     static constexpr int kLetterUnits = kRowBytes >> kLetterShift;
     static_assert(kPadLetter * kLetterUnits < 256, "letter offset must fit a byte");
 };
+
+constexpr int kUniformMaxPeriod = 256;
+constexpr int kLevelWords = kUniformMaxPeriod + 16;
 
 struct ScanParams {
     const int8_t* chars;
@@ -307,6 +314,9 @@
     int32_t jump;
     u32 jump_word;
     int32_t jump_limit;
+    int32_t uniform_frame;
+    int32_t flag_period;
+    u32 levels[kLevelWords];
 };
 
 constexpr int32_t kListEmpty = -1, kListTaken = -2;
@@ -361,9 +371,9 @@
 #ifndef SWK_CLASSES_SCALAR
 #define SWK_CLASSES_SCALAR 4
 #endif
-constexpr int frame_classes(bool packed, int R, int lanes, bool multi) {
+constexpr int frame_classes(bool packed, int R, int lanes, bool multi, bool uniform = false) {
     (void)lanes;
-    const int want = packed ? ((R > SWK_WAVES3_MAX_R || (multi && R >= 25 && R > SWK_WAVES3_MAX_R_MULTI)) ? SWK_CLASSES_PACKED : SWK_CLASSES_PACKED_SMALL)
+    const int want = packed ? ((R > SWK_WAVES3_MAX_R || (multi && R >= 25 && (uniform || R > SWK_WAVES3_MAX_R_MULTI))) ? SWK_CLASSES_PACKED : SWK_CLASSES_PACKED_SMALL)
                             : SWK_CLASSES_SCALAR;
     int P = want;
     while (P > 1 && 2 * P > R) P--;
@@ -401,11 +411,11 @@
     u32 Zc[P + 4];
 };
 
-template <int KIND, int R, int LANES, int BYTE, bool MULTI, bool OFFS = false, int P = 1, bool ZFILL = true>
+template <int KIND, int R, int LANES, int BYTE, bool MULTI, bool OFFS = false, int P = 1, bool ZFILL = true, bool UNI = false>
 __device__ __forceinline__ void dp_step(StripeState<KIND, R, P>& st, const unsigned char* tile,
                                         u32 lettersA, u32 lettersB, u32 gop, u32 gex, u32 inH, u32 inF,
                                         u32 apos = 0, bool first = false, u32 wrapP = 0, u32 wrapLast = 0, bool head = false,
-                                        u32 laneStep = 0) {
+                                        u32 laneStep = 0, const u32* zw = nullptr) {
     using A = Arith<KIND>;
     using G = Geometry<KIND, R, LANES>;
     const u32 step2 = LANES < 16 ? laneStep : 0x00100010u;
@@ -444,7 +454,7 @@
             upH = prev_lane<LANES, false>(inH, st.Hlast, head);
             F = prev_lane<LANES, false>(inF, st.Fout, head);
         } else {
-            const u32 bH = st.Zc[Q + kLastClass];
+            const u32 bH = UNI ? zw[Q + kLastClass] : st.Zc[Q + kLastClass];
             upH = prev_lane<LANES, false>(bH, st.Hlast, head);
             if constexpr (ZFILL) F = prev_lane<LANES, true>(0u, st.Fout, head);
             else F = prev_lane<LANES, false>(st.Zc[Q], st.Fout, head);
@@ -489,7 +499,7 @@
 #pragma unroll
         for (int r = 0; r < R; r++) {
             const int c = r % P;
-            const u32 zop = st.Zc[Q + c + 1];
+            const u32 zop = UNI ? zw[Q + c + 2] : st.Zc[Q + c + 1];
             if constexpr (G::kWide) {
                 if (r % 4 == 0) __builtin_amdgcn_sched_barrier(0);
                 if (CH::starts_chunk(r) && CH::chunk_of(r) + kChunks0 < kChunksAll)
@@ -513,8 +523,8 @@
             }
             const u32 fm = A::max3(F, hg, zop);
             st.E[r] = A::max3(st.E[r], hg, zop);
-            if (c == P - 1) F = A::gap(fm, wrapP);
-            else if (r == R - 1) F = A::gap(fm, wrapLast);
+            if (r == R - 1) F = (UNI && kLastClass == 0) ? fm : A::gap(fm, wrapLast);
+            else if (c == P - 1) F = A::gap(fm, wrapP);
             else F = fm;
             if ((r / P) & 1) m[c] = A::fold2(m[c], st.H[r - P], h);
             else if (r + P >= R) m[c] = A::max2(m[c], h);
@@ -663,7 +673,7 @@
     using BD = Border<LANES>;
     constexpr int SHL1 = Shift<LANES>::kShl1;
     constexpr int kQuadsPerLetterBlock = LANES;
-    constexpr int P = OFFS ? frame_classes(A::kPacked, R, LANES, MULTI) : 1;
+    constexpr int P = OFFS ? frame_classes(A::kPacked, R, LANES, MULTI, OFFS && A::kPacked) : 1;
     __shared__ __attribute__((aligned(16))) unsigned char lds[16 + G::kTileBytes];
     __shared__ __attribute__((aligned(16))) unsigned char rings[MULTI ? BD::ring_bytes(kGroups) : 16];
 
@@ -693,12 +703,13 @@
     unsigned char* const ringOut = ringIn + BD::kInBytes;
     u32* const gBorder = MULTI ? p.scratch + ((size_t)blockIdx.x * kGroups + group) * (size_t)border_region_words<LANES>(p.lcap) : nullptr;
 
+    constexpr bool kUni = OFFS && A::kPacked;
     const u32 apos = OFFS ? A::pos_word(p.gex_mag) : 0u;
     const u32 apos4 = OFFS ? A::pos_word(4 * p.gex_mag) : 0u;
-    constexpr bool kLowers = OFFS && A::kPacked;
-    const int rq = kLowers ? p.renorm_quads : 0;
-    const u32 zstart = OFFS ? A::zero_at(p.gex_mag, LANES - lane) : A::kZero;
-    const u32 zbefore = OFFS ? A::zero_at(p.gex_mag, LANES - lane - 1) : A::kZero;
+    const int rq = kUni ? p.renorm_quads : 0;
+    const int kmask = 4 * rq - 1;
+    const u32 zstart = (OFFS && !kUni) ? A::zero_at(p.gex_mag, LANES - lane) : A::kZero;
+    const u32 zbefore = (OFFS && !kUni) ? A::zero_at(p.gex_mag, LANES - lane - 1) : A::kZero;
 
     __shared__ int next_batch, batch_avail;
     auto claim_entry = [&](int i) -> int {
@@ -786,7 +797,23 @@
                 __syncthreads();
             }
             StripeState<KIND, R, P> st;
-            {
+            u32 zw[P + 5];
+            const int tg0 = kUni ? __builtin_amdgcn_readfirstlane(LANES * stripe) : 0;
+            auto load_levels = [&](int q) {
+                const int u0 = __builtin_amdgcn_readfirstlane((tg0 + 4 * q) & kmask);
+#pragma unroll
+                for (int k = 0; k < P + 5; k++) zw[k] = p.levels[u0 + k];
+#pragma unroll
+                for (int k = 0; k < P + 5; k++) asm volatile("" : "+s"(zw[k]));
+            };
+            if constexpr (kUni) {
+                load_levels(0);
+#pragma unroll
+                for (int r = 0; r < R; r++) { st.H[r] = zw[r % P]; st.E[r] = zw[r % P + 1]; }
+                st.upH_prev = A::gap(zw[(R - 1) % P], p.gex); st.Hlast = zw[(R - 1) % P]; st.Fout = zw[0];
+#pragma unroll
+                for (int d = 0; d < P + 3; d++) st.maxv[d] = A::add(maxv, zw[d + 1]);
+            } else {
                 u32 zc[P + 5];
                 zc[0] = zbefore; zc[1] = zstart;
 #pragma unroll
@@ -822,7 +849,10 @@
             uint2 nxt = make_uint2(A::kZero, A::kZero);
             const u32* const gIn = MULTI ? gBorder + 2 * (LANES - 1) + 4 * lane : nullptr;
             auto first_stripe_pairs = [&](int j) -> uint4 {
-                if constexpr (OFFS) {
+                if constexpr (kUni) {
+                    constexpr int kLastClass = (R - 1) % P;
+                    return make_uint4(A::zero_at(p.gex_mag, (j & kmask) + kLastClass), A::kZero, A::zero_at(p.gex_mag, ((j + 1) & kmask) + kLastClass), A::kZero);
+                } else if constexpr (OFFS) {
                     constexpr int kLastClass = (R - 1) % P;
                     const int K = 4 * rq;
                     const int j0 = K > 0 ? (j & (K - 1)) : j, j1 = K > 0 ? ((j + 1) & (K - 1)) : j + 1;
@@ -872,24 +902,26 @@
                 nxt = *reinterpret_cast<const uint2*>(inPtr);
             };
 
-            auto quad = [&](int q, auto lower_tag) {
-                constexpr bool LOWER = decltype(lower_tag)::value;
+            auto lower_frame = [&]() {
+                if constexpr (kUni) {
+                    const u32 w = p.renorm_word;
+#pragma unroll
+                    for (int r = 0; r < R; r++) { st.H[r] = A::lower(st.H[r], w); st.E[r] = A::lower(st.E[r], w); }
+                    st.upH_prev = A::lower(st.upH_prev, w);
+                    if constexpr (KIND == I16X2) st.upH_prev = A::true_max(st.upH_prev, A::gap(A::kZero, p.gex));
+                    st.Hlast = A::lower(st.Hlast, w);
+                    st.Fout = A::lower(st.Fout, w);
+#pragma unroll
+                    for (int d = 0; d < P + 3; d++) st.maxv[d] = A::lower(st.maxv[d], w);
+                }
+            };
+            auto quad = [&](int q) {
                 if ((q & (kQuadsPerLetterBlock - 1)) == 0) {
                     lettersA = nextA; lettersB = nextB;
                     nextA = fetch(s0, len0pad, q / kQuadsPerLetterBlock + 1);
                     if constexpr (A::kPacked) nextB = fetch(s1, len1pad, q / kQuadsPerLetterBlock + 1);
                 }
-                const int lower_lane = 4 * (q & (rq - 1));
-                auto lower_frame = [&](int k) {
-                    const u32 gw = lane == k ? p.renorm_word : 0u;
-#pragma unroll
-                    for (int r = 0; r < R; r++) { st.H[r] = A::gap(st.H[r], gw); st.E[r] = A::gap(st.E[r], gw); }
-                    st.upH_prev = A::gap(st.upH_prev, gw);
-#pragma unroll
-                    for (int k = 0; k < P + 4; k++) st.Zc[k] = A::gap(st.Zc[k], gw);
-#pragma unroll
-                    for (int d = 0; d < P + 3; d++) st.maxv[d] = A::gap(st.maxv[d], gw);
-                };
+                const bool lower = kUni && ((tg0 + 4 * q + 4) & kmask) == 0;
                 auto border_step = [&](auto byte_tag) {
                     constexpr int BYTE = decltype(byte_tag)::value;
                     const uint2 in = nxt;
@@ -901,52 +933,36 @@
                             nxt = *reinterpret_cast<const uint2*>(inPtr + 8 * (BYTE + 1));
                         }
                     }
-                    dp_step<KIND, R, LANES, BYTE, MULTI, OFFS, P>(st, lds, lettersA, lettersB, p.gop, p.gex, in.x, in.y, apos, first, p.wrap_class, p.wrap_last, head, laneStep);
+                    dp_step<KIND, R, LANES, BYTE, MULTI, OFFS, P, true, kUni>(st, lds, lettersA, lettersB, p.gop, p.gex, in.x, in.y, apos, first,
+                                                                          p.wrap_class, p.wrap_last, head, laneStep, zw);
+                    if constexpr (kUni && BYTE == 3) {
+                        if (lower) lower_frame();
+                    }
                     if constexpr (MULTI) *reinterpret_cast<uint2*>(outPtr + 8 * BYTE) = make_uint2(st.Hlast, st.Fout);
                 };
-                if constexpr (LOWER) lower_frame(lower_lane + 0);
                 border_step(std::integral_constant<int, 0>{});
-                if constexpr (LOWER) lower_frame(lower_lane + 1);
                 border_step(std::integral_constant<int, 1>{});
-                if constexpr (LOWER) lower_frame(lower_lane + 2);
                 border_step(std::integral_constant<int, 2>{});
-                if constexpr (LOWER) lower_frame(lower_lane + 3);
                 border_step(std::integral_constant<int, 3>{});
                 if constexpr (MULTI) outPtr += walkOut;
                 lettersA = dpp<SHL1, true>(0u, lettersA);
                 if constexpr (A::kPacked) lettersB = dpp<SHL1, true>(0u, lettersB);
                 if constexpr (OFFS && A::kWindow) {
-#pragma unroll
-                    for (int k = 0; k < P + 4; k++) st.Zc[k] = A::add(st.Zc[k], apos4);
+                    if constexpr (!kUni) {
+#pragma unroll
+                        for (int k = 0; k < P + 4; k++) st.Zc[k] = A::add(st.Zc[k], apos4);
+                    }
 #pragma unroll
                     for (int d = 0; d < P + 3; d++) st.maxv[d] = A::add(st.maxv[d], apos4);
                 }
+                if constexpr (kUni) load_levels(q + 1);
             };
             if constexpr (!MULTI) {
-                const int seg = (kLowers && rq > 0) ? rq : nquads;
-                for (int q0 = 0; q0 < nquads; q0 += seg) {
-                    const int qend = min(nquads, q0 + seg);
-                    int q = q0;
-                    if constexpr (kLowers) {
-                        if (q0 > 0) {
-                            const int qlow = min(qend, q0 + LANES / 4);
-                            for (; q < qlow; q++) quad(q, std::true_type{});
-                        }
-                    }
-                    for (; q < qend; q++) quad(q, std::false_type{});
-                }
+                for (int q = 0; q < nquads; q++) quad(q);
             } else {
-                static_assert(BD::kQuadsPerBlock >= LANES / 4, "the lowering quads of a period must lie in one block");
                 for (int q0 = 0; q0 < nquads; q0 += BD::kQuadsPerBlock) {
                     const int qend = min(nquads, q0 + BD::kQuadsPerBlock);
-                    int q = q0;
-                    if constexpr (kLowers) {
-                        if (rq > 0 && q0 > 0 && (q0 & (rq - 1)) == 0) {
-                            const int qlow = min(qend, q0 + LANES / 4);
-                            for (; q < qlow; q++) quad(q, std::true_type{});
-                        }
-                    }
-                    for (; q < qend; q++) quad(q, std::false_type{});
+                    for (int q = q0; q < qend; q++) quad(q);
                     if (qend == q0 + BD::kQuadsPerBlock) block_end(q0 / BD::kQuadsPerBlock);
                 }
             }
@@ -962,7 +978,11 @@
                     *reinterpret_cast<uint4*>(g + 4 * lane) = *reinterpret_cast<const uint4*>(ringOut + 16 * lane);
                 }
             }
-            if constexpr (OFFS) {
+            if constexpr (kUni) {
+                maxv = A::true_of(st.maxv[0], zw[1]);
+#pragma unroll
+                for (int d = 1; d < P + 3; d++) maxv = A::true_max(maxv, A::true_of(st.maxv[d], zw[d + 1]));
+            } else if constexpr (OFFS) {
                 if constexpr (A::kWindow) {
                     maxv = A::true_of(st.maxv[0], st.Zc[0]);
 #pragma unroll
@@ -997,7 +1017,14 @@
             }
             sc0 = A::true_lo(maxv);
             sc1 = A::true_hi(maxv);
-            guard = p.gex_mag * ((rq > 0 && 4 * nquads > 4 * rq ? 4 * rq : 4 * nquads) + 2 * LANES + 4 + P);
+            if constexpr (kUni) {
+                const int tgmax = 4 * nquads + LANES * (p.nstripes - 1);
+                constexpr int kColP = frame_classes(true, R, LANES, MULTI);
+                guard = max(p.gex_mag * ((tgmax > 4 * rq ? 4 * rq : tgmax) + P + 8),
+                            p.gex_mag * (min(4 * nquads, p.flag_period) + 2 * LANES + 4 + kColP));
+            } else {
+                guard = p.gex_mag * (4 * nquads + 2 * LANES + 4 + P);
+            }
         } else {
             maxv = group_max<KIND, LANES>(maxv);
             sc0 = A::score_lo(maxv);
@@ -1028,7 +1055,7 @@
 template <int KIND, int R, int LANES>
 __global__ void sw_build_profile_kernel(const int8_t* __restrict__ query, int32_t qlen,
                                         const int8_t* __restrict__ matrix21, int32_t pad_row, int32_t nstripes,
-                                        unsigned char* __restrict__ profile, int32_t shift) {
+                                        unsigned char* __restrict__ profile, int32_t shift, int32_t head_extra) {
     using A = Arith<KIND>;
     using G = Geometry<KIND, R, LANES>;
     constexpr int kWordsPerRow = G::kRowBytes / 4;
@@ -1047,9 +1074,10 @@
                 if (row_in_lane >= R) return 0u;
                 const int64_t row = (int64_t)stripe * G::kStripeRows + lane * R + row_in_lane;
                 const int qc = row < qlen ? (int)query[row] : pad_row;
-                const int P = frame_classes(A::kPacked, R, LANES, nstripes > 1);
+                const int P = frame_classes(A::kPacked, R, LANES, nstripes > 1, head_extra != 0);
                 const int cls = row_in_lane % P, above = (row_in_lane == 0 ? R - 1 : row_in_lane - 1) % P;
-                return A::encode_score((int)matrix21[qc * kLetters + letter] + shift * (1 + cls - above));
+                const int head = row_in_lane == 0 ? head_extra : 0;
+                return A::encode_score((int)matrix21[qc * kLetters + letter] + shift * (1 + head + cls - above));
             };
             if constexpr (G::kWide) v = w < R ? (entry(w) | (A::kOne << 16)) : 0u;
             else if constexpr (A::kPacked) v = entry(2 * w) | (entry(2 * w + 1) << 16);
diff --git a/cudasw4_amd/csrc/sw_kind_f16x2.hip b/cudasw4_amd/csrc/sw_kind_f16x2.hip
--- a/cudasw4_amd/csrc/sw_kind_f16x2.hip
+++ b/cudasw4_amd/csrc/sw_kind_f16x2.hip
@@ -3,15 +3,15 @@
 namespace swk {
 #define SWK_CASE_SCAN16_F16X2(R) case R: return launch_scan_r<F16X2, R, 16>(multi, offs, grid, reserve, stream, p);
 #define SWK_CASE_SCAN64_F16X2(R) case R: return launch_scan_r<F16X2, R, 64>(multi, offs, grid, reserve, stream, p);
-#define SWK_CASE_PROF16_F16X2(R) case R: return launch_profile_r<F16X2, R, 16>(q, qlen, m, pr, ns, out, shift, s);
-#define SWK_CASE_PROF64_F16X2(R) case R: return launch_profile_r<F16X2, R, 64>(q, qlen, m, pr, ns, out, shift, s);
+#define SWK_CASE_PROF16_F16X2(R) case R: return launch_profile_r<F16X2, R, 16>(q, qlen, m, pr, ns, out, shift, hx, s);
+#define SWK_CASE_PROF64_F16X2(R) case R: return launch_profile_r<F16X2, R, 64>(q, qlen, m, pr, ns, out, shift, hx, s);
 #define SWK_CASE_TILE16_F16X2(R) case R: return tile_bytes_r<F16X2, R, 16>();
 #define SWK_CASE_TILE64_F16X2(R) case R: return tile_bytes_r<F16X2, R, 64>();
 #define SWK_CASE_SCAN8_F16X2(R) case R: return launch_scan_r<F16X2, R, 8>(multi, offs, grid, reserve, stream, p);
-#define SWK_CASE_PROF8_F16X2(R) case R: return launch_profile_r<F16X2, R, 8>(q, qlen, m, pr, ns, out, shift, s);
+#define SWK_CASE_PROF8_F16X2(R) case R: return launch_profile_r<F16X2, R, 8>(q, qlen, m, pr, ns, out, shift, hx, s);
 #define SWK_CASE_TILE8_F16X2(R) case R: return tile_bytes_r<F16X2, R, 8>();
 #define SWK_CASE_SCAN4_F16X2(R) case R: return launch_scan_r<F16X2, R, 4>(multi, offs, grid, reserve, stream, p);
-#define SWK_CASE_PROF4_F16X2(R) case R: return launch_profile_r<F16X2, R, 4>(q, qlen, m, pr, ns, out, shift, s);
+#define SWK_CASE_PROF4_F16X2(R) case R: return launch_profile_r<F16X2, R, 4>(q, qlen, m, pr, ns, out, shift, hx, s);
 #define SWK_CASE_TILE4_F16X2(R) case R: return tile_bytes_r<F16X2, R, 4>();
 SWK_DEFINE_KIND(launch_f16x2, F16X2, SWK_FOR_EACH_R_PACKED)
 }
diff --git a/cudasw4_amd/csrc/sw_kind_f32.hip b/cudasw4_amd/csrc/sw_kind_f32.hip
--- a/cudasw4_amd/csrc/sw_kind_f32.hip
+++ b/cudasw4_amd/csrc/sw_kind_f32.hip
@@ -3,15 +3,15 @@
 namespace swk {
 #define SWK_CASE_SCAN16_F32(R) case R: return launch_scan_r<F32, R, 16>(multi, offs, grid, reserve, stream, p);
 #define SWK_CASE_SCAN64_F32(R) case R: return launch_scan_r<F32, R, 64>(multi, offs, grid, reserve, stream, p);
-#define SWK_CASE_PROF16_F32(R) case R: return launch_profile_r<F32, R, 16>(q, qlen, m, pr, ns, out, shift, s);
-#define SWK_CASE_PROF64_F32(R) case R: return launch_profile_r<F32, R, 64>(q, qlen, m, pr, ns, out, shift, s);
+#define SWK_CASE_PROF16_F32(R) case R: return launch_profile_r<F32, R, 16>(q, qlen, m, pr, ns, out, shift, hx, s);
+#define SWK_CASE_PROF64_F32(R) case R: return launch_profile_r<F32, R, 64>(q, qlen, m, pr, ns, out, shift, hx, s);
 #define SWK_CASE_TILE16_F32(R) case R: return tile_bytes_r<F32, R, 16>();
 #define SWK_CASE_TILE64_F32(R) case R: return tile_bytes_r<F32, R, 64>();
 #define SWK_CASE_SCAN8_F32(R) case R: return launch_scan_r<F32, R, 8>(multi, offs, grid, reserve, stream, p);
-#define SWK_CASE_PROF8_F32(R) case R: return launch_profile_r<F32, R, 8>(q, qlen, m, pr, ns, out, shift, s);
+#define SWK_CASE_PROF8_F32(R) case R: return launch_profile_r<F32, R, 8>(q, qlen, m, pr, ns, out, shift, hx, s);
 #define SWK_CASE_TILE8_F32(R) case R: return tile_bytes_r<F32, R, 8>();
 #define SWK_CASE_SCAN4_F32(R) case R: return launch_scan_r<F32, R, 4>(multi, offs, grid, reserve, stream, p);
-#define SWK_CASE_PROF4_F32(R) case R: return launch_profile_r<F32, R, 4>(q, qlen, m, pr, ns, out, shift, s);
+#define SWK_CASE_PROF4_F32(R) case R: return launch_profile_r<F32, R, 4>(q, qlen, m, pr, ns, out, shift, hx, s);
 #define SWK_CASE_TILE4_F32(R) case R: return tile_bytes_r<F32, R, 4>();
 SWK_DEFINE_KIND(launch_f32, F32, SWK_FOR_EACH_R_I32)
 }
diff --git a/cudasw4_amd/csrc/sw_kind_i16x2.hip b/cudasw4_amd/csrc/sw_kind_i16x2.hip
--- a/cudasw4_amd/csrc/sw_kind_i16x2.hip
+++ b/cudasw4_amd/csrc/sw_kind_i16x2.hip
@@ -3,15 +3,15 @@
 namespace swk {
 #define SWK_CASE_SCAN16_I16X2(R) case R: return launch_scan_r<I16X2, R, 16>(multi, offs, grid, reserve, stream, p);
 #define SWK_CASE_SCAN64_I16X2(R) case R: return launch_scan_r<I16X2, R, 64>(multi, offs, grid, reserve, stream, p);
-#define SWK_CASE_PROF16_I16X2(R) case R: return launch_profile_r<I16X2, R, 16>(q, qlen, m, pr, ns, out, shift, s);
-#define SWK_CASE_PROF64_I16X2(R) case R: return launch_profile_r<I16X2, R, 64>(q, qlen, m, pr, ns, out, shift, s);
+#define SWK_CASE_PROF16_I16X2(R) case R: return launch_profile_r<I16X2, R, 16>(q, qlen, m, pr, ns, out, shift, hx, s);
+#define SWK_CASE_PROF64_I16X2(R) case R: return launch_profile_r<I16X2, R, 64>(q, qlen, m, pr, ns, out, shift, hx, s);
 #define SWK_CASE_TILE16_I16X2(R) case R: return tile_bytes_r<I16X2, R, 16>();
 #define SWK_CASE_TILE64_I16X2(R) case R: return tile_bytes_r<I16X2, R, 64>();
 #define SWK_CASE_SCAN8_I16X2(R) case R: return launch_scan_r<I16X2, R, 8>(multi, offs, grid, reserve, stream, p);
-#define SWK_CASE_PROF8_I16X2(R) case R: return launch_profile_r<I16X2, R, 8>(q, qlen, m, pr, ns, out, shift, s);
+#define SWK_CASE_PROF8_I16X2(R) case R: return launch_profile_r<I16X2, R, 8>(q, qlen, m, pr, ns, out, shift, hx, s);
 #define SWK_CASE_TILE8_I16X2(R) case R: return tile_bytes_r<I16X2, R, 8>();
 #define SWK_CASE_SCAN4_I16X2(R) case R: return launch_scan_r<I16X2, R, 4>(multi, offs, grid, reserve, stream, p);
-#define SWK_CASE_PROF4_I16X2(R) case R: return launch_profile_r<I16X2, R, 4>(q, qlen, m, pr, ns, out, shift, s);
+#define SWK_CASE_PROF4_I16X2(R) case R: return launch_profile_r<I16X2, R, 4>(q, qlen, m, pr, ns, out, shift, hx, s);
 #define SWK_CASE_TILE4_I16X2(R) case R: return tile_bytes_r<I16X2, R, 4>();
 SWK_DEFINE_KIND(launch_i16x2, I16X2, SWK_FOR_EACH_R_PACKED)
 }
diff --git a/cudasw4_amd/csrc/sw_kind_i32.hip b/cudasw4_amd/csrc/sw_kind_i32.hip
--- a/cudasw4_amd/csrc/sw_kind_i32.hip
+++ b/cudasw4_amd/csrc/sw_kind_i32.hip
@@ -3,15 +3,15 @@
 namespace swk {
 #define SWK_CASE_SCAN16_I32(R) case R: return launch_scan_r<I32, R, 16>(multi, offs, grid, reserve, stream, p);
 #define SWK_CASE_SCAN64_I32(R) case R: return launch_scan_r<I32, R, 64>(multi, offs, grid, reserve, stream, p);
-#define SWK_CASE_PROF16_I32(R) case R: return launch_profile_r<I32, R, 16>(q, qlen, m, pr, ns, out, shift, s);
-#define SWK_CASE_PROF64_I32(R) case R: return launch_profile_r<I32, R, 64>(q, qlen, m, pr, ns, out, shift, s);
+#define SWK_CASE_PROF16_I32(R) case R: return launch_profile_r<I32, R, 16>(q, qlen, m, pr, ns, out, shift, hx, s);
+#define SWK_CASE_PROF64_I32(R) case R: return launch_profile_r<I32, R, 64>(q, qlen, m, pr, ns, out, shift, hx, s);
 #define SWK_CASE_TILE16_I32(R) case R: return tile_bytes_r<I32, R, 16>();
 #define SWK_CASE_TILE64_I32(R) case R: return tile_bytes_r<I32, R, 64>();
 #define SWK_CASE_SCAN8_I32(R) case R: return launch_scan_r<I32, R, 8>(multi, offs, grid, reserve, stream, p);
-#define SWK_CASE_PROF8_I32(R) case R: return launch_profile_r<I32, R, 8>(q, qlen, m, pr, ns, out, shift, s);
+#define SWK_CASE_PROF8_I32(R) case R: return launch_profile_r<I32, R, 8>(q, qlen, m, pr, ns, out, shift, hx, s);
 #define SWK_CASE_TILE8_I32(R) case R: return tile_bytes_r<I32, R, 8>();
 #define SWK_CASE_SCAN4_I32(R) case R: return launch_scan_r<I32, R, 4>(multi, offs, grid, reserve, stream, p);
-#define SWK_CASE_PROF4_I32(R) case R: return launch_profile_r<I32, R, 4>(q, qlen, m, pr, ns, out, shift, s);
+#define SWK_CASE_PROF4_I32(R) case R: return launch_profile_r<I32, R, 4>(q, qlen, m, pr, ns, out, shift, hx, s);
 #define SWK_CASE_TILE4_I32(R) case R: return tile_bytes_r<I32, R, 4>();
 SWK_DEFINE_KIND(launch_i32, I32, SWK_FOR_EACH_R_I32)
 }
diff --git a/cudasw4_amd/csrc/sw_launch.hpp b/cudasw4_amd/csrc/sw_launch.hpp
--- a/cudasw4_amd/csrc/sw_launch.hpp
+++ b/cudasw4_amd/csrc/sw_launch.hpp
@@ -39,7 +39,7 @@
 struct KindLaunch {
     hipError_t (*scan)(int R, int lanes, bool multi, bool offs, int grid, int reserve, hipStream_t stream, const ScanParams& p);
     hipError_t (*profile)(int R, int lanes, const int8_t* query, int32_t qlen, const int8_t* matrix21, int32_t pad_row,
-                          int32_t nstripes, unsigned char* out, int32_t shift, hipStream_t stream);
+                          int32_t nstripes, unsigned char* out, int32_t shift, int32_t head_extra, hipStream_t stream);
     size_t (*tile_bytes)(int R, int lanes);
     hipError_t (*warm)(hipStream_t stream);
     bool packed;
@@ -86,11 +86,18 @@
     return hipGetLastError();
 }
 
+constexpr bool uniform_frame_launch(bool packed, bool offs, int lanes, bool multi, int stream_slots) {
+    return packed && offs && !(lanes == 16 && (!multi || stream_slots > 1));
+}
+
 template <int KIND, int R, int LANES, bool OFFS>
 hipError_t launch_scan_ro(bool multi, int grid, int reserve, hipStream_t stream, const ScanParams& p) {
     constexpr int kMaxR = max_rows(KIND, LANES);
     constexpr bool kPacked = Arith<KIND>::kPacked;
     if constexpr (R > kMaxR || (kPacked && !OFFS)) {
+        return hipErrorInvalidValue;
+    } else if ((p.uniform_frame != 0) != uniform_frame_launch(kPacked, OFFS, LANES, multi, p.stream_slots) ||
+               (p.uniform_frame && (p.renorm_quads < LANES || 4 * p.renorm_quads > kUniformMaxPeriod))) {
         return hipErrorInvalidValue;
     } else if constexpr (kPacked && LANES == 16) {
         if (p.positions || p.claim || p.service || p.count_ptr || p.stream_slots < 1) return hipErrorInvalidValue;
@@ -125,14 +132,14 @@
 
 template <int KIND, int R, int LANES>
 hipError_t launch_profile_r(const int8_t* query, int32_t qlen, const int8_t* matrix21, int32_t pad_row, int32_t nstripes,
-                            unsigned char* out, int32_t shift, hipStream_t stream) {
+                            unsigned char* out, int32_t shift, int32_t head_extra, hipStream_t stream) {
     if constexpr (R > max_rows(KIND, LANES)) {
         return hipErrorInvalidValue;
     } else {
         const size_t total = (size_t)nstripes * kLetters * (Geometry<KIND, R, LANES>::kRowBytes / 4);
         const int grid = (int)std::min<size_t>((total + 255) / 256, 65536);
         hipLaunchKernelGGL((sw_build_profile_kernel<KIND, R, LANES>), dim3(grid), dim3(256), 0, stream, query, qlen,
-                           matrix21, pad_row, nstripes, out, shift);
+                           matrix21, pad_row, nstripes, out, shift, head_extra);
         return hipGetLastError();
     }
 }
@@ -159,7 +166,7 @@
         return hipErrorInvalidValue;                                                                                \
     }                                                                                                               \
     static hipError_t FN##_profile(int R, int lanes, const int8_t* q, int32_t qlen, const int8_t* m, int32_t pr,    \
-                                   int32_t ns, unsigned char* out, int32_t shift, hipStream_t s) {                  \
+                                   int32_t ns, unsigned char* out, int32_t shift, int32_t hx, hipStream_t s) {      \
         if (lanes == 16) { switch (R) { FOR_EACH_R(SWK_CASE_PROF16_##KIND) } }                                      \
         else if (lanes == 64) { switch (R) { FOR_EACH_R(SWK_CASE_PROF64_##KIND) } }                                 \
         else if (lanes == 8) { switch (R) { FOR_EACH_R(SWK_CASE_PROF8_##KIND) } }                                   \
```
